# aleksandrina-streltsova/lidar-global-registration

Measured on AMD Instinct MI355X. Metric: scan-pair registrations/sec, higher is better.
Workload: dtype f32

## Files before the change

include/lgr.h:

```cpp
#ifndef LGR_H
#define LGR_H
#include <stddef.h>
#include <stdint.h>
#ifdef __cplusplus
extern "C" {
#endif

#define LGR_VERSION 5

enum {
    LGR_OK = 0,
    LGR_ERR_INVALID_ARG = -1,
    LGR_ERR_NO_DEVICE = -2,
    LGR_ERR_OOM = -3,
    LGR_ERR_HIP = -4,
    LGR_ERR_UNSUPPORTED = -5,
    LGR_ERR_VOXEL_TOO_SMALL = -6
};

enum { LGR_MATCH_LR = 0, LGR_MATCH_ONE_SIDED = 1, LGR_MATCH_CLUSTER = 2 };
enum { LGR_METRIC_CORRESPONDENCES = 0, LGR_METRIC_UNIFORMITY = 1, LGR_METRIC_CLOSEST_PLANE = 2, LGR_METRIC_COMBINATION = 3,
       LGR_METRIC_WEIGHTED_CLOSEST_PLANE = 4 };
enum { LGR_SCORE_CONSTANT = 0, LGR_SCORE_MAE = 1, LGR_SCORE_MSE = 2, LGR_SCORE_EXP = 3 };
enum { LGR_ALIGN_RANSAC = 0, LGR_ALIGN_GROR = 1 };
enum { LGR_KEYPOINT_ANY = 0, LGR_KEYPOINT_ISS = 1 };
enum { LGR_ORDER_REFERENCE = 0, LGR_ORDER_CANONICAL = 1 };

typedef struct { int32_t index_query, index_match; float distance, threshold; } lgr_corr;

typedef struct {
    int32_t feature_nr_points;
    int32_t normal_nr_points;
    float   edge_thr_coef;
    float   distance_thr;
    float   feature_radius;
    float   scale_factor;
    float   confidence;
    int32_t bf_block_size;
    int32_t cluster_k;
    int32_t randomness;
    int32_t n_samples;
    int32_t alignment_id, matching_id, metric_id, score_id;
    int32_t max_iterations;
    int32_t normals_available;
    int32_t fix_seed;
    int32_t has_vp_src, has_vp_tgt;
    float   vp_src[3], vp_tgt[3];
    int32_t ransac_batch;
    uint64_t seed;
    int32_t keypoint_id;
    float   iss_radius_src, iss_radius_tgt;
    int32_t use_bfmatcher;
    int32_t has_guess;
    float   match_search_radius;
    float   guess[16];
} lgr_params;

typedef struct {
    float   transformation[16];
    int32_t iterations;
    int32_t converged;
    int32_t n_inliers;
    float   metric;
    float   best_metric_before_refit;
    int32_t best_iteration;
    int32_t num_rejections;
    int32_t estimated_iters;
    int32_t n_correspondences;
    double  time_cs, time_te;
    float   stage_ms[12];
} lgr_result;

typedef struct lgr_ctx lgr_ctx;

typedef struct {
    int32_t helper_contexts;
    int32_t concurrent_contexts;
    int32_t arithmetic;
    int32_t pcl_neighbour_cap;
    int32_t ransac_schedule;
    int32_t reserved[3];
} lgr_ctx_options;
enum { LGR_RANSAC_SCHEDULE_DEFAULT = 0, LGR_RANSAC_SCHEDULE_CHAIN = 1, LGR_RANSAC_SCHEDULE_RESIDENT = 2 };
enum { LGR_ARITH_FAST = 0, LGR_ARITH_PCL = 1 };

typedef struct {
    int32_t prune;
    int32_t leaves;
    int32_t near;
    int32_t operand_format;
    int32_t box_bounds;
    int32_t column_stage;
    int32_t coarse_rejection;
    int32_t rerank_refilter;
    int32_t pair_cap;
    int32_t poison_tables;
    int32_t self_check;
    int32_t shell_bound;
    int32_t split_sweep;
    int32_t kept_cap;
    int32_t auto_dense;
    int32_t irregular_rows;
} lgr_match_options;

int  lgr_version(void);
#define LGR_STREAM_OWN ((void*) (intptr_t) -1)
int  lgr_ctx_create(int device, void* stream, lgr_ctx** out);
int  lgr_ctx_destroy(lgr_ctx* ctx);
int  lgr_ctx_sync(lgr_ctx* ctx);
const char* lgr_last_error(lgr_ctx* ctx);
void lgr_default_params(lgr_params* p);
int  lgr_ctx_stage_ms(lgr_ctx* ctx, float* out12);
void lgr_match_default_options(lgr_match_options* opt);
int  lgr_ctx_set_match_options(lgr_ctx* ctx, const lgr_match_options* opt);
int  lgr_ctx_get_match_options(lgr_ctx* ctx, lgr_match_options* opt);
int  lgr_ctx_workspace_bytes(lgr_ctx* ctx, uint64_t* bytes);
void lgr_ctx_default_options(lgr_ctx_options* opt);
int  lgr_ctx_set_options(lgr_ctx* ctx, const lgr_ctx_options* opt);
int  lgr_ctx_get_options(lgr_ctx* ctx, lgr_ctx_options* opt);
int  lgr_ctx_host_threads(lgr_ctx* ctx, int* n);

int lgr_sort_pairs_u32_dev(lgr_ctx*, const uint32_t* d_keys_in, uint32_t* d_keys_out, const int32_t* d_vals_in, int32_t* d_vals_out,
                           size_t n, int begin_bit, int end_bit);
int lgr_sort_pairs_u64_dev(lgr_ctx*, const uint64_t* d_keys_in, uint64_t* d_keys_out, const int32_t* d_vals_in, int32_t* d_vals_out,
                           size_t n, const int* shifts, const int* widths, int n_ranges);

int lgr_bbox_dev(lgr_ctx*, const float* d_pts, int n, float* d_min3_max3 );

int lgr_preprocess(lgr_ctx*, const float* pts, int n, const float* vp3, int normals_available, int order, float* out, int* n_out, float* voxel_out);
int lgr_preprocess_dev(lgr_ctx*, const float* d_pts, int n, const float* vp3 , int normals_available, float* d_out, int* n_out ,
                       float* voxel_out );
int lgr_dedupe_dev(lgr_ctx*, const float* d_pts, int n, float* d_out, int* n_out );
int lgr_cloud_density_dev(lgr_ctx*, const float* d_pts, int n, float quantile, float* out );

int lgr_iss_keypoints(lgr_ctx*, const float* pts, int n, float radius, float gamma21, float gamma32, int min_neighbors,
                      int32_t* idx, int* n_out);
int lgr_iss_keypoints_dev(lgr_ctx*, const float* d_pts, int n, float radius, float gamma21, float gamma32, int min_neighbors,
                          int32_t* d_idx, int* n_out );

int lgr_downsample(lgr_ctx*, const float* pts, int n, float voxel, int order, float* out, int* n_out);
int lgr_downsample_dev(lgr_ctx*, const float* d_pts, int n, float voxel, float* d_out, int* n_out );

int lgr_normals_knn(lgr_ctx*, float* pts, int n, const float* surf, int ns, int k, const float* vp3, int normals_available);
int lgr_normals_knn_dev(lgr_ctx*, float* d_pts, int n, const float* d_surf, int ns, int k, const float* vp3 , int normals_available);

int lgr_fpfh(lgr_ctx*, const float* kps, int m, const float* surf, int n, float radius, float* out_m_x_33);
int lgr_fpfh_dev(lgr_ctx*, const float* d_kps, int m, const float* d_surf, int n, float radius, float* d_out);
int lgr_shot_lrf(lgr_ctx*, const float* kps, int m, const float* surf, int n, float radius, float* out_m_x_9);
int lgr_shot_lrf_dev(lgr_ctx*, const float* d_kps, int m, const float* d_surf, int n, float radius, float* d_out_m_x_9);
int lgr_shot(lgr_ctx*, const float* kps, int m, const float* surf, int n, float radius, const float* lrf_or_null,
             float* out_m_x_352, float* out_lrf_or_null);
int lgr_shot_dev(lgr_ctx*, const float* d_kps, int m, const float* d_surf, int n, float radius, const float* d_lrf_or_null,
                 float* d_out_m_x_352, float* d_out_lrf_or_null);
int lgr_gravity_lrf(lgr_ctx*, const float* kps, int m, const float* surf, int n, float radius, float* out_m_x_9);
int lgr_gravity_lrf_dev(lgr_ctx*, const float* d_kps, int m, const float* d_surf, int n, float radius, float* d_out_m_x_9);
int lgr_rops(lgr_ctx*, const float* kps, int m, const float* surf, int n, float radius, const float* lrf, float* out_m_x_135);
int lgr_rops_dev(lgr_ctx*, const float* d_kps, int m, const float* d_surf, int n, float radius, const float* d_lrf, float* d_out_m_x_135);
int lgr_selfcheck_rcp(lgr_ctx*, unsigned lo_bits, unsigned hi_bits, unsigned long long* out2);
int lgr_selfcheck_libm(lgr_ctx*, int fn, const float* a, const float* b, long long n, float* out);

int lgr_match_bf(lgr_ctx*, const float* q33, int mq, const float* t33, int mt, int block, int32_t* idx, float* dist);
int lgr_match_bf_dev(lgr_ctx*, const float* d_q33, int mq, const float* d_t33, int mt, int block, int32_t* d_idx, float* d_dist);
int lgr_match_bf2_dev(lgr_ctx*, const float* d_a33, int ma, const float* d_b33, int mb, int block,
                      int32_t* d_ab_idx, float* d_ab_dist, int32_t* d_ba_idx, float* d_ba_dist);
int lgr_match_shot(lgr_ctx*, const float* q352, int mq, const float* t352, int mt, int block, int32_t* idx, float* dist);
int lgr_match_shot_dev(lgr_ctx*, const float* d_q352, int mq, const float* d_t352, int mt, int block, int32_t* d_idx, float* d_dist);
int lgr_match2_shot_dev(lgr_ctx*, const float* d_a352, int ma, const float* d_b352, int mb, int block,
                        int32_t* d_ab_idx, float* d_ab_dist, int32_t* d_ba_idx, float* d_ba_dist);
int lgr_match_rops(lgr_ctx*, const float* q135, int mq, const float* t135, int mt, int block, int32_t* idx, float* dist);
int lgr_match_rops_dev(lgr_ctx*, const float* d_q135, int mq, const float* d_t135, int mt, int block, int32_t* d_idx, float* d_dist);
int lgr_match2_rops_dev(lgr_ctx*, const float* d_a135, int ma, const float* d_b135, int mb, int block,
                        int32_t* d_ab_idx, float* d_ab_dist, int32_t* d_ba_idx, float* d_ba_dist);
int lgr_match_flann(lgr_ctx*, const float* q33, int mq, const float* t33, int mt, int32_t* idx, float* dist);
int lgr_match_flann_dev(lgr_ctx*, const float* d_q33, int mq, const float* d_t33, int mt, int32_t* d_idx, float* d_dist);
int lgr_match_local(lgr_ctx*, const float* query_pts, int mq, const float* train_pts, int mt, const float* q33, const float* t33,
                    const float guess16[16], float match_search_radius, int32_t* idx, float* dist);
int lgr_match_local_dev(lgr_ctx*, const float* d_query_pts, int mq, const float* d_train_pts, int mt, const float* d_q33, const float* d_t33,
                        const float guess16[16] , float match_search_radius, int32_t* d_idx, float* d_dist);

int lgr_match_last_stats(lgr_ctx*, unsigned* out6);
int lgr_match_last_kernel_ms(lgr_ctx*, float* ms);
int lgr_match_last_work(lgr_ctx*, double* executed_fraction);
int lgr_match_last_issued(lgr_ctx*, double* out2 );
int lgr_match_last_coarse(lgr_ctx*, double* out2);
int lgr_match_last_shell(lgr_ctx*, double* tiles_skipped);
int lgr_match_last_pairs(lgr_ctx*, unsigned* out2);
int lgr_match_last_format(lgr_ctx*, int* f16);
int lgr_match_last_lbstats(lgr_ctx*, double* out2);
int lgr_match_last_irregular(lgr_ctx*, unsigned* out3);
int lgr_match_last_check(lgr_ctx*, double* out2);
int lgr_match_last_check_cover(lgr_ctx*, unsigned long long* out8);
int lgr_smoothed_densities(lgr_ctx*, const float* pts, int n, int k, float* out);
int lgr_smoothed_densities_dev(lgr_ctx*, const float* d_pts, int n, int k, float* d_out);
int lgr_knn_dev(lgr_ctx*, const float* d_q, int nq, const float* d_pts, int n, int k, int32_t* d_idx, float* d_d2);

int lgr_filter_dev(lgr_ctx*, int matching_id, const float* d_src, int ns, const float* d_tgt, int nt,
                   const int32_t* d_ij_idx, const float* d_ij_dist, const int32_t* d_ji_idx, const float* d_ji_dist,
                   float distance_thr, int cluster_k, lgr_corr* d_out, int* n_out );

int lgr_correspondences(lgr_ctx*, const float* src, int ns, const float* tgt, int nt, const lgr_params*, lgr_corr* out, int* n_out);
int lgr_correspondences_dev(lgr_ctx*, const float* d_src, int ns, const float* d_tgt, int nt, const lgr_params*, lgr_corr* d_out, int* n_out );

enum { LGR_DESCRIPTOR_FPFH = 0, LGR_DESCRIPTOR_SHOT = 1, LGR_DESCRIPTOR_ROPS = 2 };
enum { LGR_LRF_DEFAULT = 0, LGR_LRF_GRAVITY = 1, LGR_LRF_GT = 2 };
typedef struct {
    int32_t descriptor_id;
    int32_t lrf_id;
    int32_t reserved[6];
} lgr_feature_params;
void lgr_default_feature_params(lgr_feature_params* f);
int lgr_correspondences_ex(lgr_ctx*, const float* src, int ns, const float* tgt, int nt, const lgr_params*, const lgr_feature_params*,
                           lgr_corr* out, int* n_out);
int lgr_correspondences_ex_dev(lgr_ctx*, const float* d_src, int ns, const float* d_tgt, int nt, const lgr_params*, const lgr_feature_params*,
                               lgr_corr* d_out, int* n_out );

int lgr_ransac(lgr_ctx*, const float* src, int ns, const float* tgt, int nt, const lgr_corr* corr, int c,
               const lgr_params*, lgr_result*, uint8_t* final_mask);
int lgr_ransac_dev(lgr_ctx*, const float* d_src, int ns, const float* d_tgt, int nt, const lgr_corr* d_corr, int c,
                   const lgr_params*, lgr_result* , uint8_t* d_final_mask);
int lgr_ransac_replay_dev(lgr_ctx*, const float* d_src, int ns, const float* d_tgt, int nt, const lgr_corr* d_corr, int c,
                          const lgr_params*, const int32_t* d_triples, int n,
                          uint8_t* d_ok, float* d_T16, int32_t* d_n_inliers, float* d_metric);
int lgr_ransac_samples_dev(lgr_ctx*, uint64_t seed, int first, int n, int n_corr, int32_t* d_triples);
int lgr_ransac_samples_n_dev(lgr_ctx*, uint64_t seed, int first, int n, int n_corr, int n_samples, int32_t* d_tuples);
int lgr_selfcheck_philox(lgr_ctx*, uint64_t key, const uint32_t counter4[4], uint32_t out4[4]);
int lgr_evaluate_dev(lgr_ctx*, const float* d_src, int ns, const float* d_tgt, int nt, const lgr_corr* d_corr, int c,
                     const float T16[16] , int metric_id, int score_id,
                     uint8_t* d_mask, int* n_inliers, float* rmse, float* metric );

int lgr_evaluate_plane_dev(lgr_ctx*, const float* d_src, int ns, const float* d_tgt, int nt, const float T16[16] , int score_id,
                           uint64_t seed, uint32_t counter, int* n_inliers, float* rmse, float* metric, float* threshold ,
                           int32_t* pairs , int* n_pairs);

enum { LGR_WEIGHT_CONSTANT = 0, LGR_WEIGHT_EXP_CURVATURE = 1, LGR_WEIGHT_CURVEDNESS = 2, LGR_WEIGHT_HARRIS = 3, LGR_WEIGHT_TOMASI = 4,
       LGR_WEIGHT_CURVATURE = 5, LGR_WEIGHT_NSS = 6 };
typedef struct {
    int32_t weight_id;
    int32_t reserved[5];
    const float* weights;
} lgr_metric_params;
void lgr_default_metric_params(lgr_metric_params* m);
int lgr_ransac_ex(lgr_ctx*, const float* src, int ns, const float* tgt, int nt, const lgr_corr* corr, int c,
                  const lgr_params*, const lgr_metric_params*, lgr_result*, uint8_t* final_mask);
int lgr_ransac_ex_dev(lgr_ctx*, const float* d_src, int ns, const float* d_tgt, int nt, const lgr_corr* d_corr, int c,
                      const lgr_params*, const lgr_metric_params*, lgr_result* , uint8_t* d_final_mask);
int lgr_weights(lgr_ctx*, const float* pts, int n, int weight_id, int nr_points, float* out, float* weights_sum );
int lgr_weights_dev(lgr_ctx*, const float* d_pts, int n, int weight_id, int nr_points, float* d_out, float* weights_sum );
int lgr_principal_curvatures(lgr_ctx*, const float* pts, int n, int k, float* pc1, float* pc2);
int lgr_principal_curvatures_dev(lgr_ctx*, const float* d_pts, int n, int k, float* d_pc1, float* d_pc2);
int lgr_evaluate_plane_weighted_dev(lgr_ctx*, const float* d_src, int ns, const float* d_tgt, int nt, const float T16[16] , int score_id,
                                    uint64_t seed, uint32_t counter, const float* d_weights, float weights_sum,
                                    int* n_inliers, float* rmse, float* metric, float* threshold ,
                                    int32_t* pairs , int* n_pairs);

int lgr_refit_svd(lgr_ctx*, const float* src, const float* tgt, int ns, int nt, const lgr_corr* inliers, int n, float T16[16]);
int lgr_refit_svd_dev(lgr_ctx*, const float* d_src, const float* d_tgt, const lgr_corr* d_corr, int c,
                      const uint8_t* d_mask , float T16[16] );

int lgr_align(lgr_ctx*, const float* src, int ns, const float* tgt, int nt, const lgr_params*, lgr_result*);
int lgr_align_dev(lgr_ctx*, const float* d_src, int ns, const float* d_tgt, int nt, const lgr_params*, lgr_result* );

int lgr_align_ex(lgr_ctx*, const float* src, int ns, const float* tgt, int nt, const lgr_params*, const lgr_feature_params*, lgr_result*);
int lgr_align_ex_dev(lgr_ctx*, const float* d_src, int ns, const float* d_tgt, int nt, const lgr_params*, const lgr_feature_params*,
                     lgr_result* );

int lgr_align_ex2(lgr_ctx*, const float* src, int ns, const float* tgt, int nt, const lgr_params*, const lgr_feature_params*,
                  const lgr_metric_params*, lgr_result*);
int lgr_align_ex2_dev(lgr_ctx*, const float* d_src, int ns, const float* d_tgt, int nt, const lgr_params*, const lgr_feature_params*,
                      const lgr_metric_params*, lgr_result* );

int lgr_gror(lgr_ctx*, const float* src, int ns, const float* tgt, int nt, const lgr_corr* corr, int c,
             float resolution, int k_optimal, lgr_result* res, uint8_t* inlier_mask );
int lgr_gror_dev(lgr_ctx*, const float* d_src, int ns, const float* d_tgt, int nt, const lgr_corr* d_corr, int c,
                 float resolution, int k_optimal, lgr_result* res , uint8_t* d_inlier_mask );
int lgr_gror_node_degree_dev(lgr_ctx*, const float* d_src, const float* d_tgt, const lgr_corr* d_corr, int c,
                             float resolution, int32_t* d_degree);

int lgr_choose_best_hypothesis_dev(lgr_ctx*, const float* d_src, int ns, const float* d_tgt, int nt, const lgr_corr* d_corr, int c,
                                   const float* tns16 , int n, float T_out16[16], int* best_index, float* uniformities );
int lgr_update_hypotheses(float* tns16, float* metrics, int n, int cap, const float* new_T16, float new_metric, float distance_thr);

#ifdef __cplusplus
}
#endif
#endif
```

lidar-global-registration_amd/csrc/lgr_features.hip:

```cpp
#include <rocprim/device/device_radix_sort.hpp>
#include <rocprim/device/device_scan.hpp>

#include <algorithm>
#include <cmath>
#include <type_traits>
#include <unordered_map>
#include <vector>

#include "lgr_grid.cuh"
#include "lgr_knn_wave.cuh"
#include "lgr_seqsum.h"
#include "lgr_math.cuh"
#include "lgr_libm.cuh"

namespace {

__global__ void voxel_keys(const float* __restrict__ pts, int n, float bx, float by, float bz, float voxel,
                           unsigned long long* __restrict__ keys, int* __restrict__ vals, int* __restrict__ bad) {
    int i = blockIdx.x * blockDim.x + threadIdx.x;
    if (i >= n) return;
    float x = pts[(size_t) i * 12], y = pts[(size_t) i * 12 + 1], z = pts[(size_t) i * 12 + 2];
    unsigned long long k = ~0ull;
    if (lgr_finite3(x, y, z)) {
        int ix = (int) floorf((x - bx) / voxel), iy = (int) floorf((y - by) / voxel), iz = (int) floorf((z - bz) / voxel);
        if (ix < 0 || iy < 0 || iz < 0 || ix >= (1 << 21) || iy >= (1 << 21) || iz >= (1 << 21)) { atomicExch(bad, 1); ix = iy = iz = 0; }
        k = ((unsigned long long) iz << 42) | ((unsigned long long) iy << 21) | (unsigned long long) ix;
    }
    keys[i] = k; vals[i] = i;
}

__global__ void head_flags(const unsigned long long* __restrict__ keys, int n, int* __restrict__ flags) {
    int i = blockIdx.x * blockDim.x + threadIdx.x;
    if (i >= n) return;
    unsigned long long k = keys[i];
    flags[i] = (k != ~0ull && (i == 0 || keys[i - 1] != k)) ? 1 : 0;
}

__global__ void voxel_accumulate(const float* __restrict__ pts, const unsigned long long* __restrict__ keys,
                                 const int* __restrict__ vals, const int* __restrict__ flags,
                                 const int* __restrict__ rank , int n,
                                 float* __restrict__ out, unsigned long long* __restrict__ out_keys, int* __restrict__ out_first) {
    int i = blockIdx.x * blockDim.x + threadIdx.x;
    if (i >= n || !flags[i]) return;
    unsigned long long k = keys[i];
    float sx = 0.f, sy = 0.f, sz = 0.f, sw = 0.f, snx = 0.f, sny = 0.f, snz = 0.f;
    for (int j = i; j < n && keys[j] == k; ++j) {
        const float4* p = reinterpret_cast<const float4*>(pts + (size_t) vals[j] * 12);
        float4 a = p[0], b = p[1], c = p[2];
        float w = c.x;
        sx += w * a.x; sy += w * a.y; sz += w * a.z;
        sw += w;
        snx += w * b.x; sny += w * b.y; snz += w * b.z;
    }
    float ax = snx / sw, ay = sny / sw, az = snz / sw;
    float norm = __builtin_sqrtf(ax * ax + ay * ay + az * az);
    norm = ((double) norm < 1e-5) ? 1.f : norm;
    int r = rank[i];
    float4* o = reinterpret_cast<float4*>(out + (size_t) r * 12);
    o[0] = make_float4(sx / sw, sy / sw, sz / sw, 1.f);
    o[1] = make_float4(ax / norm, ay / norm, az / norm, 0.f);
    o[2] = make_float4(sw, 0.f, 0.f, 0.f);
    if (out_keys) { out_keys[r] = k; out_first[r] = vals[i]; }
}

constexpr int NB = 128;

template <class IndexOf>
__device__ __forceinline__ void normals_finish(float* __restrict__ p, float px, float py, float pz, int count, IndexOf&& index_of,
                                               const float* __restrict__ surf, float vpx, float vpy, float vpz) {
    const float nanv = __uint_as_float(0x7fc00000u);
    if (count < 3) { p[4] = nanv; p[5] = nanv; p[6] = nanv; p[9] = nanv; return; }
    const float* K = surf + (size_t) index_of(0) * 12;
    float Kx = K[0], Ky = K[1], Kz = K[2];
    float a0 = 0.f, a1 = 0.f, a2 = 0.f, a3 = 0.f, a4 = 0.f, a5 = 0.f, a6 = 0.f, a7 = 0.f, a8 = 0.f;
    for (int j = 0; j < count; ++j) {
        const float* q = surf + (size_t) index_of(j) * 12;
        float x = q[0] - Kx, y = q[1] - Ky, z = q[2] - Kz;
        a0 += x * x; a1 += x * y; a2 += x * z; a3 += y * y; a4 += y * z; a5 += z * z;
        a6 += x; a7 += y; a8 += z;
    }
    float fn = (float) count;
    a0 /= fn; a1 /= fn; a2 /= fn; a3 /= fn; a4 /= fn; a5 /= fn; a6 /= fn; a7 /= fn; a8 /= fn;
    float C[9];
    C[0] = a0 - a6 * a6; C[1] = a1 - a6 * a7; C[2] = a2 - a6 * a8;
    C[4] = a3 - a7 * a7; C[5] = a4 - a7 * a8; C[8] = a5 - a8 * a8;
    C[3] = C[1]; C[6] = C[2]; C[7] = C[5];
    float lambda_min, nx, ny, nz;
    lgr_pcl_eigen33(C, lambda_min, nx, ny, nz);
    float eig_sum = C[0] + C[4] + C[8];
    float curv = (eig_sum != 0.f) ? fabsf(lambda_min / eig_sum) : 0.f;
    float dx = vpx - px, dy = vpy - py, dz = vpz - pz;
    float cos_theta = (dx * nx + dy * ny + dz * nz);
    if (cos_theta < 0.f) { nx = -nx; ny = -ny; nz = -nz; }
    if (lgr_finite3(nx, ny, nz)) {
        float norm = __builtin_sqrtf(nx * nx + ny * ny + nz * nz);
        nx /= norm; ny /= norm; nz /= norm;
    }
    p[4] = nx; p[5] = ny; p[6] = nz; p[9] = curv;
}

__global__ __launch_bounds__(NB) void normals_kernel(GridDev g, const float* __restrict__ surf, float* __restrict__ pts, int n,
                                                      int k, float vpx, float vpy, float vpz, int by_grid) {
    extern __shared__ float smem[];
    float* sd = smem;
    int* si = (int*) (smem + (size_t) k * NB);
    int i = blockIdx.x * NB + threadIdx.x;
    if (by_grid == 1) {
        i = lgr_xcd_tile(blockIdx.x, cdiv_dev(g.n, NB)) * NB + threadIdx.x;
        if (i >= g.n) return;
        i = __float_as_int(g.pxyz[i].w);
    } else if (i >= n) return;
    float* p = pts + (size_t) i * 12;
    float px = p[0], py = p[1], pz = p[2];
    if (by_grid == 2 && lgr_finite3(px, py, pz)) return;
    KnnList<NB> L;
    L.init(sd, si, k, threadIdx.x);
    if (lgr_finite3(px, py, pz) && g.n > 0) lgr_knn_query(g, px, py, pz, L);
    normals_finish(p, px, py, pz, L.count, [&](int j) { return L.index(j); }, surf, vpx, vpy, vpz);
}

constexpr int NW_WAVES = 4;
template <int KPL>
__global__ __launch_bounds__(64 * NW_WAVES) void normals_wave_kernel(GridDev g, const float* __restrict__ surf, float* __restrict__ pts, int k,
                                                                      float vpx, float vpy, float vpz, float r2_init) {
    extern __shared__ int slist[];
    __shared__ unsigned long long sbuf[NW_WAVES][WaveKnn<KPL>::BUF];
    __shared__ int srow[NW_WAVES][128];
    const int lane = threadIdx.x & 63, wv = threadIdx.x >> 6;
    const int n_tiles = cdiv_dev(g.n, 64 * NW_WAVES);
    const int tile = lgr_xcd_tile(blockIdx.x, n_tiles);
    if (tile >= n_tiles) return;
    const int t = (tile * NW_WAVES + wv) * 64 + lane;
    int* list = slist + (size_t) wv * k * 64;
    int qi = -1;
    float px = 0.f, py = 0.f, pz = 0.f;
    if (t < g.n) {
        const float4 q = g.pxyz[t];
        qi = __float_as_int(q.w); px = q.x; py = q.y; pz = q.z;
    }
    float guess = r2_init;
    int count = 0;
    lgr_wave_knn_tile<KPL>(g, qi >= 0, px, py, pz, k, guess, sbuf[wv], srow[wv], [&](int l, const WaveKnn<KPL>& W) {
        const int mk = min(W.m, k);
#pragma unroll
        for (int j = 0; j < KPL; ++j)
            if (W.rank[j] < mk) list[W.rank[j] * 64 + l] = (int) (unsigned) W.key[j];
        if (lane == l) count = mk;
    });
    __builtin_amdgcn_fence(__ATOMIC_RELEASE, "wavefront");
    __builtin_amdgcn_wave_barrier();
    if (qi < 0) return;
    normals_finish(pts + (size_t) qi * 12, px, py, pz, count, [&](int j) { return list[j * 64 + lane]; }, surf, vpx, vpy, vpz);
}

__device__ __forceinline__ float dot3e(float ax, float ay, float az, float bx, float by, float bz) {
    return (ax * bx + az * bz) + ay * by;
}

__device__ __forceinline__ bool pair_features(float p1x, float p1y, float p1z, float n1x, float n1y, float n1z,
                                              float p2x, float p2y, float p2z, float n2x, float n2y, float n2z,
                                              float& f1, float& f2, float& f3) {
    float dx = p2x - p1x, dy = p2y - p1y, dz = p2z - p1z;
    float f4 = __builtin_sqrtf(dot3e(dx, dy, dz, dx, dy, dz));
    if (f4 == 0.0f) return false;
    float angle1 = dot3e(n1x, n1y, n1z, dx, dy, dz) / f4;
    float angle2 = dot3e(n2x, n2y, n2z, dx, dy, dz) / f4;
    float ux = n1x, uy = n1y, uz = n1z, mx = n2x, my = n2y, mz = n2z;
    float a1 = fabsf(angle1), a2 = fabsf(angle2);
    if (lgr_glibc::acosf_(a1) > lgr_glibc::acosf_(a2)) {
        ux = n2x; uy = n2y; uz = n2z; mx = n1x; my = n1y; mz = n1z;
        dx = -dx; dy = -dy; dz = -dz;
        f3 = -angle2;
    } else {
        f3 = angle1;
    }
    float vx = dy * uz - dz * uy, vy = dz * ux - dx * uz, vz = dx * uy - dy * ux;
    float v_norm = __builtin_sqrtf(dot3e(vx, vy, vz, vx, vy, vz));
    if (v_norm == 0.0f) return false;
    vx /= v_norm; vy /= v_norm; vz /= v_norm;
    float wx = uy * vz - uz * vy, wy = uz * vx - ux * vz, wz = ux * vy - uy * vx;
    f2 = dot3e(vx, vy, vz, mx, my, mz);
    float yy = dot3e(wx, wy, wz, mx, my, mz), xx = dot3e(ux, uy, uz, mx, my, mz);
    f1 = lgr_glibc::atan2f_(yy, xx);
    return true;
}

typedef float v2f __attribute__((ext_vector_type(2)));

__device__ __forceinline__ float lgr_atan2f_fast(float y, float x) {
    const float ax = fabsf(x), ay = fabsf(y);
    const float mx = (ax > ay) ? ax : ay;
    const float mn = (ax > ay) ? ay : ax;
    const float a = mn * __builtin_amdgcn_rcpf(mx);
    const bool hi = a > 0.41421356237f;
    const float z = hi ? (a - 1.0f) * __builtin_amdgcn_rcpf(a + 1.0f) : a;
    const float z2 = z * z;
    float p = 8.05374449538e-2f * z2 - 1.38776856032e-1f;
    p = p * z2 + 1.99777106478e-1f;
    p = p * z2 - 3.33329491539e-1f;
    p = p * z2 * z + z;
    float r = (hi ? 0.78539816339f : 0.0f) + p;
    if (ay > ax) r = 1.57079632679f - r;
    if (x < 0.0f) r = 3.14159265359f - r;
    if (y < 0.0f) r = -r;
    return r;
}
__device__ __forceinline__ bool bin_decided(float t, float margin, int& b) {
    const float fl = floorf(t);
    const float fr = t - fl;
    b = (int) fminf(fmaxf(fl, 0.0f), 10.0f);
    return fr > margin && fr < 1.0f - margin;
}
__device__ __forceinline__ void pair_bins_fast(float p1x, float p1y, float p1z, float n1x, float n1y, float n1z, float p2x, float p2y, float p2z, float n2x, float n2y, float n2z,
                                               int (&b0)[3], bool& dec0) {
    constexpr float DA = 1e-6f;
    float dx = p2x - p1x, dy = p2y - p1y, dz = p2z - p1z;
    const float f4s = dot3e(dx, dy, dz, dx, dy, dz);
    const float rs = __builtin_amdgcn_rsqf(f4s);
    const float angle1 = dot3e(n1x, n1y, n1z, dx, dy, dz) * rs;
    const float angle2 = dot3e(n2x, n2y, n2z, dx, dy, dz) * rs;
    const float a1 = fabsf(angle1), a2 = fabsf(angle2);
    const bool s0 = a1 < a2;
    bool c0 = f4s > 1e-30f && (s0 ? (a2 - a1 > 2.0f * DA && a2 < 1.0f - DA) : (a1 - a2 > 2.0f * DA));
    const float ux = s0 ? n2x : n1x, uy = s0 ? n2y : n1y, uz = s0 ? n2z : n1z;
    const float mx = s0 ? n1x : n2x, my = s0 ? n1y : n2y, mz = s0 ? n1z : n2z;
    dx = s0 ? -dx : dx; dy = s0 ? -dy : dy; dz = s0 ? -dz : dz;
    const float f3 = s0 ? -angle2 : angle1;
    float vx = dy * uz - dz * uy, vy = dz * ux - dx * uz, vz = dx * uy - dy * ux;
    const float vn2 = dot3e(vx, vy, vz, vx, vy, vz);
    const float rv = __builtin_amdgcn_rsqf(vn2);
    c0 = c0 && vn2 > 1e-30f;
    vx = vx * rv; vy = vy * rv; vz = vz * rv;
    const float wx = uy * vz - uz * vy, wy = uz * vx - ux * vz, wz = ux * vy - uy * vx;
    const float f2 = dot3e(vx, vy, vz, mx, my, mz);
    const float yy = dot3e(wx, wy, wz, mx, my, mz), xx = dot3e(ux, uy, uz, mx, my, mz);
    const float rho2 = xx * xx + yy * yy;
    const float f1 = lgr_atan2f_fast(yy, xx);
    const float irho = __builtin_amdgcn_rsqf(rho2);
    c0 = c0 && rho2 > 1e-4f;
    constexpr float S1 = (float) (11.0 * (double) (1.0f / (2.0f * 3.14159274101257324f)));
    constexpr float O1 = (float) (11.0 * 3.14159265358979323846 * (double) (1.0f / (2.0f * 3.14159274101257324f)));
    const float t1 = __builtin_fmaf(f1, S1, O1), t2 = __builtin_fmaf(f2, 5.5f, 5.5f), t3 = __builtin_fmaf(f3, 5.5f, 5.5f);
    const float m1 = __builtin_fmaf(irho, 1.751f * 5e-6f, 1.751f * 3e-6f + 2e-6f);
    constexpr float M2 = 5.5f * 3e-6f + 1e-6f, M3 = 5.5f * DA + 1e-6f;
    const bool d01 = bin_decided(t1, m1, b0[0]), d02 = bin_decided(t2, M2, b0[1]), d03 = bin_decided(t3, M3, b0[2]);
    dec0 = d01 && d02 && d03 && c0;
}

__device__ __forceinline__ int bin11(double t) {
    double v = floor(11 * t);
    if (!(v == v)) return 0;
    if (v < 0) return 0;
    if (v >= 11) return 10;
    return (int) v;
}

constexpr int HP = 48;
__host__ __device__ constexpr int spfh_slot(int b) { return (b & 15) * 3 + (b >> 4); }
#ifdef LGR_SPFH_CHECK
__device__ unsigned long long g_spfh_check[4];
#endif
constexpr int ST = 16;
constexpr int SQ = 256;
constexpr int SHP = 33;

#ifndef LGR_SPFH_WAVES
#define LGR_SPFH_WAVES 5
#endif
__global__ __launch_bounds__(64) __attribute__((amdgpu_waves_per_eu(LGR_SPFH_WAVES, LGR_SPFH_WAVES))) void spfh_tile_kernel(GridDev g, float r2, const int* __restrict__ order, float* __restrict__ spfh ) {
    __shared__ float4 tp[ST], tn[ST];
    __shared__ float4 cp[64], cn[64];
    __shared__ unsigned short queue[SQ];
    __shared__ int hist[2][ST][SHP];
    __shared__ int kcnt[ST];
    const int l = threadIdx.x;
    int pos = -1, cell = -1;
    float x = 0.f, y = 0.f, z = 0.f;
    const int tile = lgr_xcd_tile(blockIdx.x, cdiv_dev(g.n, ST));
    if (tile * ST >= g.n) return;
    if (l < ST) {
        const int rnk = tile * ST + l;
        if (rnk < g.n) {
            pos = order ? order[rnk] : rnk;
            const float4 P = g.pxyz[pos];
            x = P.x; y = P.y; z = P.z;
            tp[l] = make_float4(P.x, P.y, P.z, __int_as_float(pos));
            tn[l] = g.pnrm[pos];
            const int cx = min(max(lgr_cellc(x, g.ox, g.h), 0), g.dx - 1), cy = min(max(lgr_cellc(y, g.oy, g.h), 0), g.dy - 1), cz = min(max(lgr_cellc(z, g.oz, g.h), 0), g.dz - 1);
            cell = (cz * g.dy + cy) * g.dx + cx;
        }
        kcnt[l] = 0;
    }
    for (int q = l; q < 2 * ST * SHP; q += 64) (&hist[0][0][0])[q] = 0;
    __syncthreads();
    const float r2box = r2 * 1.0001f + 1e-30f;
    const float d_pi = 1.0f / (2.0f * 3.14159274101257324f);
    const double MPI = 3.14159265358979323846;
    int qh = 0, qt = 0;
    auto process = [&](int nb) __attribute__((always_inline)) {
        if (l < nb) {
            const unsigned e0 = queue[(qh + l) & (SQ - 1)];
            const int i0 = (int) (e0 >> 8);
            const float4 P0 = tp[i0], N0 = tn[i0], Q0 = cp[e0 & 255u], M0 = cn[e0 & 255u];
            int ba[3];
            bool dec0, ok0 = true;
            pair_bins_fast(P0.x, P0.y, P0.z, N0.x, N0.y, N0.z, Q0.x, Q0.y, Q0.z, M0.x, M0.y, M0.z, ba, dec0);
#ifdef LGR_SPFH_CHECK
            const bool fdec0 = dec0;
            const int fa0 = ba[0], fa1 = ba[1], fa2 = ba[2];
            dec0 = false;
#endif
            if (!dec0) {
                const int cc = (int) (e0 & 255u);
                const float Px = tp[i0].x, Py = tp[i0].y, Pz = tp[i0].z, Nx = tn[i0].x, Ny = tn[i0].y, Nz = tn[i0].z;
                const float Qx = cp[cc].x, Qy = cp[cc].y, Qz = cp[cc].z, Mx = cn[cc].x, My = cn[cc].y, Mz = cn[cc].z;
                float f1, f2, f3;
                ok0 = pair_features(Px, Py, Pz, Nx, Ny, Nz, Qx, Qy, Qz, Mx, My, Mz, f1, f2, f3);
                ba[0] = bin11(((double) f1 + MPI) * (double) d_pi); ba[1] = bin11(((double) f2 + 1.0) * 0.5); ba[2] = bin11(((double) f3 + 1.0) * 0.5);
            }
#ifdef LGR_SPFH_CHECK
            {
                const bool bad0 = fdec0 && (!ok0 || fa0 != ba[0] || fa1 != ba[1] || fa2 != ba[2]);
                const unsigned long long n_pairs = __popcll(__ballot(true));
                const unsigned long long n_und = __popcll(__ballot(!fdec0));
                const unsigned long long n_bad = __popcll(__ballot(bad0));
                if (l == 0) { atomicAdd(&g_spfh_check[0], n_pairs); atomicAdd(&g_spfh_check[1], n_und); if (n_bad) atomicAdd(&g_spfh_check[2], n_bad); }
            }
#endif
            if (ok0) {
                int* h = &hist[l & 1][i0][0];
                atomicAdd(h + ba[0], 1); atomicAdd(h + 11 + ba[1], 1); atomicAdd(h + 22 + ba[2], 1);
            }
        }
        qh += nb;
    };
    for (int p = 0; p < ST;) {
        const int c = __builtin_amdgcn_readlane(cell, p);
        const bool active = l < ST && cell == c;
        const int n_run = __popcll(__ballot(active));
        const int p0 = p;
        p += n_run;
        if (c < 0) break;
        float bx0 = active ? x : 3.4e38f, bx1 = active ? x : -3.4e38f, by0 = active ? y : 3.4e38f, by1 = active ? y : -3.4e38f;
        float bz0 = active ? z : 3.4e38f, bz1 = active ? z : -3.4e38f;
#pragma unroll
        for (int o = 1; o < 64; o <<= 1) {
            bx0 = fminf(bx0, __shfl_xor(bx0, o)); bx1 = fmaxf(bx1, __shfl_xor(bx1, o));
            by0 = fminf(by0, __shfl_xor(by0, o)); by1 = fmaxf(by1, __shfl_xor(by1, o));
            bz0 = fminf(bz0, __shfl_xor(bz0, o)); bz1 = fmaxf(bz1, __shfl_xor(bz1, o));
        }
        const int cz = c / (g.dx * g.dy), cy = (c / g.dx) % g.dy, cx = c % g.dx;
        int n_buf = 0;
        auto test_block = [&](int n_c) __attribute__((always_inline)) {
            float4 Q = make_float4(0.f, 0.f, 0.f, 0.f);
            if (l < n_c) Q = cp[l];
            for (int i = p0; i < p0 + n_run; ++i) {
                const float4 P_i = tp[i];
                const float d2 = lgr_dist2(P_i.x, P_i.y, P_i.z, Q.x, Q.y, Q.z);
                const bool acc = l < n_c && d2 < r2;
                const unsigned long long am = __ballot(acc);
                if (am == 0ull) continue;
                if (l == 0) kcnt[i] += __popcll(am);
                const bool enq = acc && __float_as_int(Q.w) != __float_as_int(P_i.w);
                const unsigned long long em = __ballot(enq);
                if (enq) {
                    const int rank = __builtin_amdgcn_mbcnt_hi((unsigned) (em >> 32), __builtin_amdgcn_mbcnt_lo((unsigned) em, 0u));
                    queue[(qt + rank) & (SQ - 1)] = (unsigned short) ((i << 8) | l);
                }
                qt += __popcll(em);
                if (qt - qh >= 64) {
                    __syncthreads();
                    process(64);
                }
            }
            __syncthreads();
            while (qt - qh > 0) process(min(qt - qh, 64));
            __syncthreads();
        };
        for (int zz = max(cz - 1, 0); zz <= min(cz + 1, g.dz - 1); ++zz)
            for (int yy = max(cy - 1, 0); yy <= min(cy + 1, g.dy - 1); ++yy) {
                const int x0 = max(cx - 1, 0), x1 = min(cx + 1, g.dx - 1);
                const size_t c0 = ((size_t) zz * g.dy + yy) * g.dx;
                const int b = g.cell_start[c0 + x0], e = g.cell_start[c0 + x1 + 1];
                for (int t0 = b; t0 < e; t0 += 64) {
                    const int t = t0 + l;
                    bool live = false;
                    float4 P = make_float4(0.f, 0.f, 0.f, 0.f);
                    if (t < e) {
                        P = g.pxyz[t];
                        const float ddx = fmaxf(fmaxf(bx0 - P.x, P.x - bx1), 0.f), ddy = fmaxf(fmaxf(by0 - P.y, P.y - by1), 0.f), ddz = fmaxf(fmaxf(bz0 - P.z, P.z - bz1), 0.f);
                        live = (ddx * ddx + ddy * ddy) + ddz * ddz <= r2box;
                    }
                    const unsigned long long lm = __ballot(live);
                    if (lm == 0ull) continue;
                    const int rank = __builtin_amdgcn_mbcnt_hi((unsigned) (lm >> 32), __builtin_amdgcn_mbcnt_lo((unsigned) lm, 0u));
                    const int fit = min(__popcll(lm), 64 - n_buf);
                    float4 Nq = make_float4(0.f, 0.f, 0.f, 0.f);
                    if (live) {
                        Nq = g.pnrm[t];
                        if (rank < fit) { cp[n_buf + rank] = make_float4(P.x, P.y, P.z, __int_as_float(t)); cn[n_buf + rank] = Nq; }
                    }
                    n_buf += fit;
                    __syncthreads();
                    if (n_buf == 64) {
                        test_block(64);
                        if (live && rank >= fit) { cp[rank - fit] = make_float4(P.x, P.y, P.z, __int_as_float(t)); cn[rank - fit] = Nq; }
                        n_buf = __popcll(lm) - fit;
                        __syncthreads();
                    }
                }
            }
        if (n_buf > 0) test_block(n_buf);
    }
    __syncthreads();
    for (int q = l; q < ST * 33; q += 64) {
        const int i = q / 33, b = q % 33;
        if (tile * ST + i >= g.n) continue;
        const int ps = __float_as_int(tp[i].w);
        const float incr = 100.0f / (float) (kcnt[i] - 1);
        spfh[(size_t) ps * HP + spfh_slot(b)] = lgr_seqsum(incr, hist[0][i][b] + hist[1][i][b]);
    }
    for (int q = l; q < ST * (HP - 33); q += 64) {
        const int i = q / (HP - 33), b = 33 + q % (HP - 33);
        if (tile * ST + i >= g.n) continue;
        spfh[(size_t) __float_as_int(tp[i].w) * HP + spfh_slot(b)] = 0.f;
    }
}

typedef float f32x4 __attribute__((ext_vector_type(4)));
typedef float f32x3 __attribute__((ext_vector_type(3)));
#ifndef LGR_RCP_STEPS
#define LGR_RCP_STEPS 1
#endif
constexpr float LGR_RCP_LO = 1e-36f;
__device__ __forceinline__ v2f lgr_rcp2(v2f x) {
    v2f y{__builtin_amdgcn_rcpf(x.x), __builtin_amdgcn_rcpf(x.y)};
    const v2f one{1.f, 1.f};
#pragma unroll
    for (int s = 0; s < LGR_RCP_STEPS; ++s) {
        const v2f e = __builtin_elementwise_fma(-x, y, one);
        y = __builtin_elementwise_fma(e, y, y);
    }
    return y;
}
__device__ __forceinline__ float lgr_rcp1(float x) {
    float y = __builtin_amdgcn_rcpf(x);
#pragma unroll
    for (int s = 0; s < LGR_RCP_STEPS; ++s) {
        const float e = fmaf(-x, y, 1.f);
        y = fmaf(e, y, y);
    }
    return y;
}
__global__ void rcp_check_kernel(unsigned lo_bits, unsigned hi_bits, unsigned long long* __restrict__ out) {
    unsigned long long bad = 0, cnt = 0;
    const unsigned long long span = (unsigned long long) hi_bits - lo_bits + 1ull;
    for (unsigned long long o = (unsigned long long) blockIdx.x * blockDim.x + threadIdx.x; o < span; o += (unsigned long long) gridDim.x * blockDim.x) {
        const float x = __uint_as_float(lo_bits + (unsigned) o);
        const float q = 1.0f / x;
        const v2f r2 = lgr_rcp2(v2f{x, x});
        bad += (__float_as_uint(lgr_rcp1(x)) != __float_as_uint(q)) || (__float_as_uint(r2.x) != __float_as_uint(q)) || (__float_as_uint(r2.y) != __float_as_uint(q));
        ++cnt;
    }
    for (int o = 32; o > 0; o >>= 1) { bad += __shfl_xor(bad, o); cnt += __shfl_xor(cnt, o); }
    if ((threadIdx.x & 63) == 0) { if (bad) atomicAdd(&out[0], bad); atomicAdd(&out[1], cnt); }
}
constexpr int FT = 16;
constexpr int FRING = 128;
constexpr int FP_PITCH = 36;

__global__ __launch_bounds__(64) void fpfh_mfma_kernel(GridDev g, const float* __restrict__ kps, const int* __restrict__ order, int m, float r2,
                                                       const float* __restrict__ Hs , float* __restrict__ out) {
    __shared__ float4 ring[FRING];
    __shared__ float fpl[FT * FP_PITCH];
    const int l = threadIdx.x, i = l & 15, k = l >> 4;
    const int tile = lgr_xcd_tile(blockIdx.x, cdiv_dev(m, FT));
    if (tile * FT >= m) return;
    const int r = tile * FT + i;
    const float nanv = __uint_as_float(0x7fc00000u);
    int kp = -1;
    float x = nanv, y = nanv, z = nanv;
    if (r < m) {
        kp = order[r];
        x = kps[(size_t) kp * 12]; y = kps[(size_t) kp * 12 + 1]; z = kps[(size_t) kp * 12 + 2];
    }
    const bool fin = lgr_finite3(x, y, z);
    int cell = -1;
    if (fin && g.n > 0) {
        int cx = min(max(lgr_cellc(x, g.ox, g.h), 0), g.dx - 1), cy = min(max(lgr_cellc(y, g.oy, g.h), 0), g.dy - 1), cz = min(max(lgr_cellc(z, g.oz, g.h), 0), g.dz - 1);
        cell = (cz * g.dy + cy) * g.dx + cx;
    }
    f32x4 acc0 = {0.f, 0.f, 0.f, 0.f}, acc1 = acc0, acc2 = acc0;
    bool found = false;
    const float r2box = r2 * 1.0001f + 1e-30f;
    const float* hload = Hs + 3 * i;
    for (int p = 0; p < FT;) {
        const int c = __builtin_amdgcn_readlane(cell, p);
        const bool active = cell == c;
        const unsigned long long am = __ballot(active) & 0xffffull;
        p += __popcll(am);
        if (c < 0) continue;
        float bx0 = active ? x : 3.4e38f, bx1 = active ? x : -3.4e38f, by0 = active ? y : 3.4e38f, by1 = active ? y : -3.4e38f;
        float bz0 = active ? z : 3.4e38f, bz1 = active ? z : -3.4e38f;
#pragma unroll
        for (int o = 1; o < 16; o <<= 1) {
            bx0 = fminf(bx0, __shfl_xor(bx0, o)); bx1 = fmaxf(bx1, __shfl_xor(bx1, o));
            by0 = fminf(by0, __shfl_xor(by0, o)); by1 = fmaxf(by1, __shfl_xor(by1, o));
            bz0 = fminf(bz0, __shfl_xor(bz0, o)); bz1 = fmaxf(bz1, __shfl_xor(bz1, o));
        }
        auto uni = [](float v) { return __int_as_float(__builtin_amdgcn_readfirstlane(__float_as_int(v))); };
        bx0 = uni(bx0); bx1 = uni(bx1); by0 = uni(by0); by1 = uni(by1); bz0 = uni(bz0); bz1 = uni(bz1);
        const int cz = c / (g.dx * g.dy), cy = (c / g.dx) % g.dy, cx = c % g.dx;
        int head = 0, tail = 0;
        auto round = [&](auto GC) {
            constexpr int G = decltype(GC)::value;
            float4 e[G];
            f32x3 hv[G];
#pragma unroll
            for (int u = 0; u < G; ++u) e[u] = ring[(head + 4 * u + k) & (FRING - 1)];
#pragma unroll
            for (int u = 0; u < G; ++u) hv[u] = *reinterpret_cast<const f32x3*>(hload + (unsigned) __float_as_int(e[u].w));
            const v2f X{x, x}, Y{y, y}, Z{z, z};
            float d2[G], w[G];
#pragma unroll
            for (int h2 = 0; h2 < G / 2; ++h2) {
                const v2f dx = X - v2f{e[2 * h2].x, e[2 * h2 + 1].x}, dy = Y - v2f{e[2 * h2].y, e[2 * h2 + 1].y}, dz = Z - v2f{e[2 * h2].z, e[2 * h2 + 1].z};
                const v2f dd = (dx * dx + dy * dy) + dz * dz;
                const v2f ww = lgr_rcp2(dd);
                d2[2 * h2] = dd.x; d2[2 * h2 + 1] = dd.y; w[2 * h2] = ww.x; w[2 * h2 + 1] = ww.y;
            }
            bool odd = false;
#pragma unroll
            for (int u = 0; u < G; ++u) {
                const bool in = active & (d2[u] < r2);
                found = found | in;
                const bool use = in & (d2[u] != 0.f);
                odd = odd | (use & !(d2[u] >= LGR_RCP_LO));
                w[u] = use ? w[u] : 0.f;
            }
            if (__ballot(odd) != 0ull) {
#pragma unroll
                for (int u = 0; u < G; ++u) w[u] = (active & (d2[u] < r2) & (d2[u] != 0.f)) ? 1.0f / d2[u] : 0.f;
            }
#pragma unroll
            for (int u = 0; u < G; ++u) {
                acc0 = __builtin_amdgcn_mfma_f32_16x16x4f32(w[u], hv[u].x, acc0, 0, 0, 0);
                acc1 = __builtin_amdgcn_mfma_f32_16x16x4f32(w[u], hv[u].y, acc1, 0, 0, 0);
                acc2 = __builtin_amdgcn_mfma_f32_16x16x4f32(w[u], hv[u].z, acc2, 0, 0, 0);
            }
            head += 4 * G;
        };
        auto consume = [&](int n_groups) {
            int gq = 0;
            for (; gq + 4 <= n_groups; gq += 4) round(std::integral_constant<int, 4>{});
            for (; gq < n_groups; ++gq, head += 4) {
                const float4 e = ring[(head + k) & (FRING - 1)];
                const float d2 = lgr_dist2(x, y, z, e.x, e.y, e.z);
                const bool in = active & (d2 < r2);
                found = found | in;
                const bool use = in & (d2 != 0.f);
                if (__ballot(use) == 0ull) continue;
                float w = lgr_rcp1(d2);
                if (__ballot(use & !(d2 >= LGR_RCP_LO)) != 0ull) w = 1.0f / d2;
                w = use ? w : 0.f;
                const f32x3 hv = *reinterpret_cast<const f32x3*>(hload + (unsigned) __float_as_int(e.w));
                const float b0 = hv.x, b1 = hv.y, b2 = hv.z;
                acc0 = __builtin_amdgcn_mfma_f32_16x16x4f32(w, b0, acc0, 0, 0, 0);
                acc1 = __builtin_amdgcn_mfma_f32_16x16x4f32(w, b1, acc1, 0, 0, 0);
                acc2 = __builtin_amdgcn_mfma_f32_16x16x4f32(w, b2, acc2, 0, 0, 0);
            }
        };
        for (int zz = max(cz - 1, 0); zz <= min(cz + 1, g.dz - 1); ++zz)
            for (int yy = max(cy - 1, 0); yy <= min(cy + 1, g.dy - 1); ++yy) {
                const int x0 = max(cx - 1, 0), x1 = min(cx + 1, g.dx - 1);
                const size_t c0 = ((size_t) zz * g.dy + yy) * g.dx;
                const int b = g.cell_start[c0 + x0], e = g.cell_start[c0 + x1 + 1];
                for (int t0 = b; t0 < e; t0 += 64) {
                    const int t = t0 + l;
                    bool live = false;
                    float4 P = make_float4(0.f, 0.f, 0.f, 0.f);
                    if (t < e) {
                        P = g.pxyz[t];
                        const float ddx = fmaxf(fmaxf(bx0 - P.x, P.x - bx1), 0.f), ddy = fmaxf(fmaxf(by0 - P.y, P.y - by1), 0.f), ddz = fmaxf(fmaxf(bz0 - P.z, P.z - bz1), 0.f);
                        live = (ddx * ddx + ddy * ddy) + ddz * ddz <= r2box;
                    }
                    const unsigned long long lm = __ballot(live);
                    if (lm == 0ull) continue;
                    if (live) {
                        const int rank = __builtin_amdgcn_mbcnt_hi((unsigned) (lm >> 32), __builtin_amdgcn_mbcnt_lo((unsigned) lm, 0u));
                        ring[(tail + rank) & (FRING - 1)] = make_float4(P.x, P.y, P.z, __uint_as_float((unsigned) t * (unsigned) HP));
                    }
                    tail += __popcll(lm);
                    __syncthreads();
                    consume((tail - head) >> 2);
                    __syncthreads();
                }
            }
        if (tail > head) {
            if (l < 4 - (tail - head)) ring[(tail + l) & (FRING - 1)] = make_float4(3.0e38f, 3.0e38f, 3.0e38f, __uint_as_float((unsigned) g.n * (unsigned) HP));
            __syncthreads();
            consume(1);
            __syncthreads();
        }
    }
    asm volatile("s_nop 15\n\ts_nop 7" ::: "memory");
    const unsigned long long fm = __ballot(found);
#pragma unroll
    for (int q = 0; q < 4; ++q) {
        const int row = 4 * k + q;
        fpl[row * FP_PITCH + i] = acc0[q];
        fpl[row * FP_PITCH + 16 + i] = acc1[q];
        if (i == 0) fpl[row * FP_PITCH + 32] = acc2[q];
    }
    __syncthreads();
    if (l < 3 * FT) {
        const int kq = l / 3, blk = l % 3;
        const int rr = tile * FT + kq;
        if (rr < m) {
            const bool any = ((fm >> kq) | (fm >> (kq + 16)) | (fm >> (kq + 32)) | (fm >> (kq + 48))) & 1ull;
            float* o = out + (size_t) order[rr] * 33 + 11 * blk;
            const float* f = fpl + kq * FP_PITCH + 11 * blk;
            if (!any) {
#pragma unroll
                for (int q = 0; q < 11; ++q) o[q] = nanv;
            } else {
                double sum = 0.0;
#pragma unroll
                for (int q = 0; q < 11; ++q) sum += (double) f[q];
                if (sum != 0) sum = 100.0 / sum;
#pragma unroll
                for (int q = 0; q < 11; ++q) o[q] = (float) ((double) f[q] * sum);
            }
        }
    }
}

template <int PW_CAP>
__global__ __launch_bounds__(64) void fpfh_pcl_kernel(GridDev g, const float* __restrict__ kps, const int* __restrict__ order, int m, float r2,
                                                      const float* __restrict__ Hs , float* __restrict__ out) {
    __shared__ unsigned long long skey[PW_CAP];
    __shared__ unsigned spos[PW_CAP];
    __shared__ float sval[64];
    const int l = threadIdx.x;
    const int tile = lgr_xcd_tile(blockIdx.x, m);
    if (tile >= m) return;
    const int kp = order[tile];
    const float x = kps[(size_t) kp * 12], y = kps[(size_t) kp * 12 + 1], z = kps[(size_t) kp * 12 + 2];
    const float nanv = __uint_as_float(0x7fc00000u);
    float* o = out + (size_t) kp * 33;
    if (!lgr_finite3(x, y, z) || g.n == 0) {
        if (l < 33) o[l] = nanv;
        return;
    }
    const int cx = min(max(lgr_cellc(x, g.ox, g.h), 0), g.dx - 1), cy = min(max(lgr_cellc(y, g.oy, g.h), 0), g.dy - 1), cz = min(max(lgr_cellc(z, g.oz, g.h), 0), g.dz - 1);
    const unsigned long long key_end = (unsigned long long) __float_as_uint(r2) << 32;
    auto scan = [&](unsigned long long lo, unsigned long long hi, bool store) -> int {
        int cnt = 0;
        for (int zz = max(cz - 1, 0); zz <= min(cz + 1, g.dz - 1); ++zz)
            for (int yy = max(cy - 1, 0); yy <= min(cy + 1, g.dy - 1); ++yy) {
                const int x0 = max(cx - 1, 0), x1 = min(cx + 1, g.dx - 1);
                const size_t c0 = ((size_t) zz * g.dy + yy) * g.dx;
                const int b = g.cell_start[c0 + x0], e = g.cell_start[c0 + x1 + 1];
                for (int t0 = b; t0 < e; t0 += 64) {
                    const int t = t0 + l;
                    bool in = false;
                    unsigned long long key = 0ull;
                    if (t < e) {
                        const float4 P = g.pxyz[t];
                        const float d2 = lgr_dist2(x, y, z, P.x, P.y, P.z);
                        key = ((unsigned long long) __float_as_uint(d2) << 32) | (unsigned) __float_as_int(P.w);
                        in = d2 < r2 && key >= lo && key < hi;
                    }
                    const unsigned long long bm = __ballot(in);
                    if (bm == 0ull) continue;
                    if (store && in) {
                        const int slot = cnt + __builtin_amdgcn_mbcnt_hi((unsigned) (bm >> 32), __builtin_amdgcn_mbcnt_lo((unsigned) bm, 0u));
                        if (slot < PW_CAP) { skey[slot] = key; spos[slot] = (unsigned) t; }
                    }
                    cnt += __popcll(bm);
                }
            }
        return cnt;
    };
    const int bin = min(l, 32);
    const float* hcol = Hs + spfh_slot(bin);
    for (int strict = 0; strict < 2; ++strict) {
        float fp = 0.f;
        double dsum = 0.0;
        int emin = 255;
        bool bad = false;
        int total = 0;
        unsigned long long lo = 0ull;
        while (lo < key_end) {
            unsigned long long hi = key_end;
            __syncthreads();
            int cnt = scan(lo, hi, true);
            if (cnt > PW_CAP) {
                unsigned long long a = lo, bnd = hi;
                for (;;) {
                    const unsigned long long mid = a + ((bnd - a) >> 1);
                    const int c = scan(lo, mid, false);
                    if (c > PW_CAP) bnd = mid;
                    else { a = mid; if (c >= PW_CAP / 4 || bnd - a <= 1ull) break; }
                }
                hi = a;
                __syncthreads();
                cnt = scan(lo, hi, true);
            }
            total += cnt;
            int n_pad = 64;
            while (n_pad < cnt) n_pad <<= 1;
            for (int q = cnt + l; q < n_pad; q += 64) { skey[q] = ~0ull; spos[q] = 0u; }
            __syncthreads();
            for (int k2 = 2; k2 <= n_pad; k2 <<= 1)
                for (int j = k2 >> 1; j > 0; j >>= 1) {
                    for (int q = l; q < (n_pad >> 1); q += 64) {
                        const int i0 = ((q & ~(j - 1)) << 1) | (q & (j - 1)), i1 = i0 | j;
                        const unsigned long long ka = skey[i0], kb = skey[i1];
                        const bool up = (i0 & k2) == 0;
                        if ((ka > kb) == up) {
                            skey[i0] = kb; skey[i1] = ka;
                            const unsigned pa = spos[i0]; spos[i0] = spos[i1]; spos[i1] = pa;
                        }
                    }
                    __syncthreads();
                }
            for (int q = l; q < cnt; q += 64) {
                const float d2 = __uint_as_float((unsigned) (skey[q] >> 32));
                const float w = d2 == 0.f ? 0.f : 1.0f / d2;
                skey[q] = ((unsigned long long) __float_as_uint(w) << 32) | (spos[q] * (unsigned) HP);
            }
            __syncthreads();
            if (!strict) {
                int q = 0;
                for (; q + 4 <= cnt; q += 4) {
                    const unsigned long long e0 = skey[q], e1 = skey[q + 1], e2 = skey[q + 2], e3 = skey[q + 3];
                    const float h0 = hcol[(unsigned) e0], h1 = hcol[(unsigned) e1], h2 = hcol[(unsigned) e2], h3 = hcol[(unsigned) e3];
                    const float w0 = __uint_as_float((unsigned) (e0 >> 32)), w1 = __uint_as_float((unsigned) (e1 >> 32)), w2 = __uint_as_float((unsigned) (e2 >> 32)), w3 = __uint_as_float((unsigned) (e3 >> 32));
                    const float v[4] = {h0 * w0, h1 * w1, h2 * w2, h3 * w3};
                    const float ws[4] = {w0, w1, w2, w3};
#pragma unroll
                    for (int u = 0; u < 4; ++u) {
                        if (ws[u] == 0.f) continue;
                        fp += v[u];
                        dsum += (double) v[u];
                        const int eb = (int) ((__float_as_uint(v[u]) >> 23) & 0xffu);
                        bad = bad || !(v[u] >= 0.f) || eb == 255;
                        if (v[u] != 0.f) emin = min(emin, max(eb, 1));
                    }
                }
                for (; q < cnt; ++q) {
                    const unsigned long long e0 = skey[q];
                    const float w0 = __uint_as_float((unsigned) (e0 >> 32));
                    if (w0 == 0.f) continue;
                    const float v0 = hcol[(unsigned) e0] * w0;
                    fp += v0;
                    dsum += (double) v0;
                    const int eb = (int) ((__float_as_uint(v0) >> 23) & 0xffu);
                    bad = bad || !(v0 >= 0.f) || eb == 255;
                    if (v0 != 0.f) emin = min(emin, max(eb, 1));
                }
            } else {
                for (int q = 0; q < cnt; ++q) {
                    const unsigned long long e0 = skey[q];
                    const float w0 = __uint_as_float((unsigned) (e0 >> 32));
                    if (w0 == 0.f) continue;
                    const float v0 = hcol[(unsigned) e0] * w0;
                    fp += v0;
                    sval[l] = v0;
                    __syncthreads();
                    if (l < 3) {
#pragma unroll
                        for (int u = 0; u < 11; ++u) dsum += (double) sval[11 * l + u];
                    }
                    __syncthreads();
                }
            }
            lo = hi;
        }
        if (total == 0) {
            if (l < 33) o[l] = nanv;
            return;
        }
        double bsum;
        if (!strict) {
            double t_all = l < 33 ? dsum : 0.0;
            int e_all = l < 33 ? emin : 255;
            bool b_all = l < 33 && bad;
#pragma unroll
            for (int s2 = 1; s2 < 64; s2 <<= 1) {
                t_all += __shfl_xor(t_all, s2);
                e_all = min(e_all, __shfl_xor(e_all, s2));
            }
            b_all = __ballot(b_all) != 0ull;
            const bool exact_here = !b_all && (e_all == 255 || t_all * 1.000001 < ldexp(1.0, 53 + e_all - 150));
            if (__ballot(!exact_here) != 0ull) continue;
            const int blk = bin / 11;
            bsum = 0.0;
#pragma unroll
            for (int u = 0; u < 11; ++u) bsum += __shfl(dsum, 11 * blk + u);
        } else {
            bsum = __shfl(dsum, bin / 11);
        }
        if (bsum != 0) bsum = 100.0 / bsum;
        if (l < 33) o[l] = (float) ((double) fp * bsum);
        return;
    }
}

__global__ void fine_keys(GridDev g, const float* __restrict__ pts, int stride, int m, int sb, unsigned* __restrict__ keys, int* __restrict__ vals) {
    int i = blockIdx.x * blockDim.x + threadIdx.x;
    if (i >= m) return;
    float x = pts[(size_t) i * stride], y = pts[(size_t) i * stride + 1], z = pts[(size_t) i * stride + 2];
    unsigned k = 0xffffffffu;
    if (lgr_finite3(x, y, z)) {
        int cx = min(max(lgr_cellc(x, g.ox, g.h), 0), g.dx - 1), cy = min(max(lgr_cellc(y, g.oy, g.h), 0), g.dy - 1), cz = min(max(lgr_cellc(z, g.oz, g.h), 0), g.dz - 1);
        k = (unsigned) ((cz * g.dy + cy) * g.dx + cx);
        if (sb > 0) {
            const float q = (float) (1 << sb);
            int sx = min(max((int) (((x - g.ox) / g.h - (float) cx) * q), 0), (1 << sb) - 1);
            int sy = min(max((int) (((y - g.oy) / g.h - (float) cy) * q), 0), (1 << sb) - 1);
            int sz = min(max((int) (((z - g.oz) / g.h - (float) cz) * q), 0), (1 << sb) - 1);
            unsigned mort = 0;
            for (int b = 0; b < sb; ++b) mort |= (((unsigned) sx >> b) & 1u) << (3 * b) | (((unsigned) sy >> b) & 1u) << (3 * b + 1) | (((unsigned) sz >> b) & 1u) << (3 * b + 2);
            k = (k << (3 * sb)) | mort;
        }
    }
    keys[i] = k; vals[i] = i;
}

struct Key3 { int x, y, z; bool operator==(const Key3& o) const { return x == o.x && y == o.y && z == o.z; } };
struct HashKey3 {
    std::size_t operator()(const Key3& k) const {
        std::size_t seed = 0;
        const int e[3] = {k.x, k.y, k.z};
        for (int i = 0; i < 3; ++i) seed ^= std::hash<int>()(e[i]) + 0x9e3779b9 + (seed << 6) + (seed >> 2);
        return seed;
    }
};

}

static int downsample_core(lgr_ctx* ctx, const float* d_pts, int n, float voxel, float* d_out, int* n_out,
                           std::vector<unsigned long long>* h_keys, std::vector<int>* h_first) {
    LGR_CHECK(ctx, voxel > 0.f, LGR_ERR_INVALID_ARG);
    *n_out = 0;
    if (n == 0) return LGR_OK;
    float bb[12];
    LGR_TRY(lgr_bbox_host(ctx, d_pts, n, bb));
    float bx = bb[6] - voxel * 0.5f, by = bb[7] - voxel * 0.5f, bz = bb[8] - voxel * 0.5f;
    unsigned long long *keys, *keys2;
    int *vals, *vals2, *flags, *rank, *bad;
    LGR_TRY(lgr_ws_t(ctx, WS_DS_KEYS, (size_t) n, &keys));
    LGR_TRY(lgr_ws_t(ctx, WS_DS_KEYS2, (size_t) n, &keys2));
    LGR_TRY(lgr_ws_t(ctx, WS_DS_VALS, (size_t) n, &vals));
    LGR_TRY(lgr_ws_t(ctx, WS_DS_VALS2, (size_t) n, &vals2));
    LGR_TRY(lgr_ws_t(ctx, WS_DS_FLAGS, (size_t) 2 * n + 16, &flags));
    rank = flags + n;
    bad = rank + n;
    LGR_HIP(ctx, hipMemsetAsync(bad, 0, 4, ctx->stream));
    voxel_keys<<<cdiv(n, 256), 256, 0, ctx->stream>>>(d_pts, n, bx, by, bz, voxel, keys, vals, bad);
    size_t tb2 = 0;
    LGR_HIP(ctx, rocprim::exclusive_scan(nullptr, tb2, flags, rank, 0, (size_t) n, rocprim::plus<int>(), ctx->stream));
    void* tmp;
    LGR_TRY(lgr_ws(ctx, WS_GRID_TMP, tb2, &tmp));
    {
        const float bnd[3] = {bx, by, bz};
        int shifts[3] = {0, 21, 42}, widths[3];
        for (int a = 0; a < 3; ++a) {
            const float q = std::floor((bb[9 + a] - bnd[a]) / voxel);
            long long imax = (q >= 0.f && q < 2097152.f) ? (long long) q : 2097151;
            int b = 1;
            while ((1ll << b) <= imax) ++b;
            widths[a] = std::min(21, b);
        }
        widths[2] = std::min(22, widths[2] + 1);
        LGR_TRY(lgr_sort_pairs_u64(ctx, keys, keys2, vals, vals2, (size_t) n, shifts, widths, 3));
    }
    head_flags<<<cdiv(n, 256), 256, 0, ctx->stream>>>(keys2, n, flags);
    LGR_HIP(ctx, rocprim::exclusive_scan(tmp, tb2, flags, rank, 0, (size_t) n, rocprim::plus<int>(), ctx->stream));
    int* h;
    LGR_TRY(lgr_pinned(ctx, 64, (void**) &h));
    LGR_HIP(ctx, hipMemcpyAsync(h, rank + (n - 1), 4, hipMemcpyDeviceToHost, ctx->stream));
    LGR_HIP(ctx, hipMemcpyAsync(h + 1, flags + (n - 1), 4, hipMemcpyDeviceToHost, ctx->stream));
    LGR_HIP(ctx, hipMemcpyAsync(h + 2, bad, 4, hipMemcpyDeviceToHost, ctx->stream));
    LGR_HIP(ctx, hipStreamSynchronize(ctx->stream));
    int nv = h[0] + h[1];
    if (h[2]) return lgr_fail(ctx, LGR_ERR_VOXEL_TOO_SMALL, "voxel index exceeds 21 bits per axis", __FILE__, __LINE__);
    unsigned long long* okeys = nullptr;
    int* ofirst = nullptr;
    if (h_keys) {
        LGR_TRY(lgr_ws_t(ctx, WS_DS_MISC, (size_t) nv * 3 + 4, (int**) &ofirst));
        okeys = (unsigned long long*) (ofirst + ((nv + 1) & ~1));
    }
    float* stage = d_out;
    bool alias = d_out == d_pts;
    if (alias) LGR_TRY(lgr_ws_t(ctx, WS_HOST_F, (size_t) nv * 12 + 4, &stage));
    voxel_accumulate<<<cdiv(n, 256), 256, 0, ctx->stream>>>(d_pts, keys2, vals2, flags, rank, n, stage, okeys, ofirst);
    if (alias) LGR_HIP(ctx, hipMemcpyAsync(d_out, stage, (size_t) nv * 48, hipMemcpyDeviceToDevice, ctx->stream));
    if (h_keys) {
        h_keys->resize(nv); h_first->resize(nv);
        LGR_HIP(ctx, hipMemcpyAsync(h_keys->data(), okeys, (size_t) nv * 8, hipMemcpyDeviceToHost, ctx->stream));
        LGR_HIP(ctx, hipMemcpyAsync(h_first->data(), ofirst, (size_t) nv * 4, hipMemcpyDeviceToHost, ctx->stream));
        LGR_HIP(ctx, hipStreamSynchronize(ctx->stream));
    }
    LGR_HIP(ctx, hipGetLastError());
    *n_out = nv;
    return LGR_OK;
}

extern "C" int lgr_downsample_dev(lgr_ctx* ctx, const float* d_pts, int n, float voxel, float* d_out, int* n_out) {
    lgr_turn turn__(ctx);
    if (!ctx) return LGR_ERR_INVALID_ARG;
    LGR_CHECK(ctx, (d_pts || n == 0) && (d_out || n == 0) && n_out && n >= 0, LGR_ERR_INVALID_ARG);
    LGR_HIP(ctx, hipSetDevice(ctx->device));
    return downsample_core(ctx, d_pts, n, voxel, d_out, n_out, nullptr, nullptr);
}

extern "C" int lgr_downsample(lgr_ctx* ctx, const float* pts, int n, float voxel, int order, float* out, int* n_out) {
    lgr_turn turn__(ctx);
    if (!ctx) return LGR_ERR_INVALID_ARG;
    LGR_CHECK(ctx, (pts || n == 0) && out && n_out && n >= 0, LGR_ERR_INVALID_ARG);
    LGR_CHECK(ctx, order == LGR_ORDER_REFERENCE || order == LGR_ORDER_CANONICAL, LGR_ERR_INVALID_ARG);
    LGR_HIP(ctx, hipSetDevice(ctx->device));
    *n_out = 0;
    if (n == 0) return LGR_OK;
    float *dp, *dout;
    LGR_TRY(lgr_ws_t(ctx, WS_HOST_A, (size_t) n * 12, &dp));
    LGR_TRY(lgr_ws_t(ctx, WS_HOST_B, (size_t) n * 12, &dout));
    LGR_HIP(ctx, hipMemcpyAsync(dp, pts, (size_t) n * 48, hipMemcpyHostToDevice, ctx->stream));
    std::vector<unsigned long long> keys;
    std::vector<int> first;
    int nv = 0;
    LGR_TRY(downsample_core(ctx, dp, n, voxel, dout, &nv, order == LGR_ORDER_REFERENCE ? &keys : nullptr, &first));
    if (order == LGR_ORDER_CANONICAL) {
        LGR_HIP(ctx, hipMemcpyAsync(out, dout, (size_t) nv * 48, hipMemcpyDeviceToHost, ctx->stream));
        LGR_HIP(ctx, hipStreamSynchronize(ctx->stream));
    } else {
        std::vector<float> tmp((size_t) nv * 12);
        LGR_HIP(ctx, hipMemcpyAsync(tmp.data(), dout, (size_t) nv * 48, hipMemcpyDeviceToHost, ctx->stream));
        LGR_HIP(ctx, hipStreamSynchronize(ctx->stream));
        std::vector<int> by_first(nv);
        for (int i = 0; i < nv; ++i) by_first[i] = i;
        std::sort(by_first.begin(), by_first.end(), [&](int a, int b) { return first[a] < first[b]; });
        std::unordered_map<Key3, int, HashKey3> m;
        for (int v : by_first) {
            unsigned long long k = keys[v];
            Key3 k3{(int) (k & 0x1fffff), (int) ((k >> 21) & 0x1fffff), (int) ((k >> 42) & 0x1fffff)};
            m[k3] = v;
        }
        size_t o = 0;
        for (const auto& kv : m) { memcpy(out + 12 * o, tmp.data() + 12 * (size_t) kv.second, 48); ++o; }
    }
    *n_out = nv;
    return LGR_OK;
}

extern "C" int lgr_selfcheck_rcp(lgr_ctx* ctx, unsigned lo_bits, unsigned hi_bits, unsigned long long* out2) {
    lgr_turn turn__(ctx);
    if (!ctx) return LGR_ERR_INVALID_ARG;
    LGR_CHECK(ctx, out2 && lo_bits <= hi_bits, LGR_ERR_INVALID_ARG);
    LGR_HIP(ctx, hipSetDevice(ctx->device));
    unsigned long long* d;
    LGR_TRY(lgr_ws_t(ctx, WS_HOST_A, (size_t) 2, &d));
    LGR_HIP(ctx, hipMemsetAsync(d, 0, 16, ctx->stream));
    rcp_check_kernel<<<8 * ctx->n_cu, 256, 0, ctx->stream>>>(lo_bits, hi_bits, d);
    LGR_HIP(ctx, hipGetLastError());
    LGR_HIP(ctx, hipMemcpyAsync(out2, d, 16, hipMemcpyDeviceToHost, ctx->stream));
    LGR_HIP(ctx, hipStreamSynchronize(ctx->stream));
    return LGR_OK;
}

__global__ void libm_eval_kernel(int fn, const float* __restrict__ a, const float* __restrict__ b, long long n, float* __restrict__ out) {
    for (long long i = (long long) blockIdx.x * blockDim.x + threadIdx.x; i < n; i += (long long) gridDim.x * blockDim.x) {
        const float x = a[i];
        float r;
        switch (fn) {
            case 0: r = lgr_glibc::acosf_(x); break;
            case 1: r = lgr_glibc::atanf_(x); break;
            case 2: r = lgr_glibc::atan2f_(x, b[i]); break;
            case 3: r = lgr_glibc::sinf_(x); break;
            default: r = lgr_glibc::cosf_(x); break;
        }
        out[i] = r;
    }
}
extern "C" int lgr_selfcheck_libm(lgr_ctx* ctx, int fn, const float* a, const float* b, long long n, float* out) {
    lgr_turn turn__(ctx);
    if (!ctx) return LGR_ERR_INVALID_ARG;
    LGR_CHECK(ctx, fn >= 0 && fn <= 6 && a && out && n >= 0 && (fn != 2 || b), LGR_ERR_INVALID_ARG);
    if (n == 0) return LGR_OK;
    LGR_HIP(ctx, hipSetDevice(ctx->device));
    float *da, *db, *dout;
    LGR_TRY(lgr_ws_t(ctx, WS_HOST_A, (size_t) n, &da));
    LGR_TRY(lgr_ws_t(ctx, WS_HOST_B, (size_t) n, &db));
    LGR_TRY(lgr_ws_t(ctx, WS_HOST_C, (size_t) n, &dout));
    LGR_HIP(ctx, hipMemcpyAsync(da, a, (size_t) n * 4, hipMemcpyHostToDevice, ctx->stream));
    if (fn == 2) LGR_HIP(ctx, hipMemcpyAsync(db, b, (size_t) n * 4, hipMemcpyHostToDevice, ctx->stream));
    if (fn >= 5) LGR_TRY(lgr_weights_libm_launch(ctx, fn, da, n, dout));
    else libm_eval_kernel<<<8 * ctx->n_cu, 256, 0, ctx->stream>>>(fn, da, db, n, dout);
    LGR_HIP(ctx, hipGetLastError());
    LGR_HIP(ctx, hipMemcpyAsync(out, dout, (size_t) n * 4, hipMemcpyDeviceToHost, ctx->stream));
    LGR_HIP(ctx, hipStreamSynchronize(ctx->stream));
    return LGR_OK;
}

#ifdef LGR_SPFH_CHECK
extern "C" int lgr_debug_spfh_check(unsigned long long* out3, int reset) {
    unsigned long long z[4] = {0, 0, 0, 0};
    if (hipMemcpyFromSymbol(out3, HIP_SYMBOL(g_spfh_check), 24) != hipSuccess) return LGR_ERR_HIP;
    if (reset && hipMemcpyToSymbol(HIP_SYMBOL(g_spfh_check), z, 32) != hipSuccess) return LGR_ERR_HIP;
    return LGR_OK;
}
#endif

extern "C" int lgr_normals_knn_dev(lgr_ctx* ctx, float* d_pts, int n, const float* d_surf, int ns, int k, const float* vp3, int normals_available) {
    lgr_turn turn__(ctx);
    if (!ctx) return LGR_ERR_INVALID_ARG;
    LGR_CHECK(ctx, (d_pts || n == 0) && n >= 0 && k >= 1 && k <= 64, LGR_ERR_INVALID_ARG);
    (void) normals_available;
    if (n == 0) return LGR_OK;
    LGR_HIP(ctx, hipSetDevice(ctx->device));
    const float* S = d_surf;
    if (!S) {
        float* snap;
        LGR_TRY(lgr_ws_t(ctx, WS_HOST_F, (size_t) n * 12, &snap));
        LGR_HIP(ctx, hipMemcpyAsync(snap, d_pts, (size_t) n * 48, hipMemcpyDeviceToDevice, ctx->stream));
        S = snap; ns = n;
    }
    GridDev g;
    const bool wave = !d_surf && k >= 16;
    const float ppc = wave ? 10.f : 6.f;
    LGR_TRY(lgr_grid_build(ctx, WS_GRID_A, S, ns, 0.f, ppc, &g));
    size_t sm = (size_t) k * NB * 8;
    const float vx = vp3 ? vp3[0] : 0.f, vy = vp3 ? vp3[1] : 0.f, vz = vp3 ? vp3[2] : 0.f;
    if (wave) {
        const float r2i = g.h * g.h * 1.25f * (float) k / (3.14159265f * ppc);
        const int grid = lgr_xcd_grid(cdiv(g.n, 64 * NW_WAVES));
        const size_t sml = (size_t) NW_WAVES * k * 64 * sizeof(int);
        if (g.n > 0) {
            if (k <= 40) normals_wave_kernel<1><<<grid, 64 * NW_WAVES, sml, ctx->stream>>>(g, S, d_pts, k, vx, vy, vz, r2i);
            else {
                if (sml + 8192 > 65536) LGR_HIP(ctx, hipFuncSetAttribute((const void*) normals_wave_kernel<2>, hipFuncAttributeMaxDynamicSharedMemorySize, (int) sml));
                normals_wave_kernel<2><<<grid, 64 * NW_WAVES, sml, ctx->stream>>>(g, S, d_pts, k, vx, vy, vz, r2i);
            }
        }
        if (g.n < n) normals_kernel<<<cdiv(n, NB), NB, sm, ctx->stream>>>(g, S, d_pts, n, k, vx, vy, vz, 2);
    } else if (!d_surf) {
        if (g.n > 0) normals_kernel<<<lgr_xcd_grid(cdiv(g.n, NB)), NB, sm, ctx->stream>>>(g, S, d_pts, n, k, vx, vy, vz, 1);
        if (g.n < n) normals_kernel<<<cdiv(n, NB), NB, sm, ctx->stream>>>(g, S, d_pts, n, k, vx, vy, vz, 2);
    } else {
        normals_kernel<<<cdiv(n, NB), NB, sm, ctx->stream>>>(g, S, d_pts, n, k, vx, vy, vz, 0);
    }
    LGR_HIP(ctx, hipGetLastError());
    return LGR_OK;
}

extern "C" int lgr_normals_knn(lgr_ctx* ctx, float* pts, int n, const float* surf, int ns, int k, const float* vp3, int normals_available) {
    lgr_turn turn__(ctx);
    if (!ctx) return LGR_ERR_INVALID_ARG;
    LGR_CHECK(ctx, (pts || n == 0) && n >= 0, LGR_ERR_INVALID_ARG);
    if (n == 0) return LGR_OK;
    LGR_HIP(ctx, hipSetDevice(ctx->device));
    float *dp, *ds = nullptr;
    LGR_TRY(lgr_ws_t(ctx, WS_HOST_A, (size_t) n * 12, &dp));
    LGR_HIP(ctx, hipMemcpyAsync(dp, pts, (size_t) n * 48, hipMemcpyHostToDevice, ctx->stream));
    if (surf) {
        LGR_TRY(lgr_ws_t(ctx, WS_HOST_B, (size_t) ns * 12 + 4, &ds));
        LGR_HIP(ctx, hipMemcpyAsync(ds, surf, (size_t) ns * 48, hipMemcpyHostToDevice, ctx->stream));
    }
    LGR_TRY(lgr_normals_knn_dev(ctx, dp, n, ds, ns, k, vp3, normals_available));
    LGR_HIP(ctx, hipMemcpyAsync(pts, dp, (size_t) n * 48, hipMemcpyDeviceToHost, ctx->stream));
    LGR_HIP(ctx, hipStreamSynchronize(ctx->stream));
    return LGR_OK;
}

extern "C" int lgr_fpfh_dev(lgr_ctx* ctx, const float* d_kps, int m, const float* d_surf, int n, float radius, float* d_out) {
    lgr_turn turn__(ctx);
    if (!ctx) return LGR_ERR_INVALID_ARG;
    LGR_CHECK(ctx, (d_kps || m == 0) && (d_surf || n == 0) && (d_out || m == 0) && m >= 0 && n >= 0 && radius > 0.f, LGR_ERR_INVALID_ARG);
    LGR_CHECK(ctx, radius <= 1e18f && (size_t) n + 1 <= ((size_t) 1 << 32) / HP - 1, LGR_ERR_UNSUPPORTED);
    if (m == 0) return LGR_OK;
    LGR_HIP(ctx, hipSetDevice(ctx->device));
    GridDev g;
    LGR_TRY(lgr_grid_build(ctx, WS_GRID_B, d_surf, n, radius * 1.001f, 0.f, &g));
    float r2 = radius * radius;
    float* spfh;
    LGR_TRY(lgr_ws_t(ctx, WS_SPFH, ((size_t) n + 1) * HP + 64, &spfh));
    LGR_HIP(ctx, hipMemsetAsync(spfh + (size_t) g.n * HP, 0, HP * sizeof(float), ctx->stream));
    const long long n_cells = (long long) g.dx * g.dy * g.dz;
    int cell_bits = 1;
    while ((1ll << cell_bits) < n_cells) ++cell_bits;
    const int sb = std::max(0, std::min(2, (32 - cell_bits) / 3));
    const int key_bits = std::min(32, cell_bits + 3 * sb);
    const int mx = std::max(m, g.n);
    unsigned *keys, *keys2, *kkeys, *kkeys2;
    int *vals, *vals2, *kvals, *kvals2;
    LGR_TRY(lgr_ws_t(ctx, WS_KP_ORDER, (size_t) mx * 8 + 16, &keys));
    keys2 = keys + mx; vals = (int*) (keys2 + mx); vals2 = vals + mx;
    kkeys = (unsigned*) (vals2 + mx); kkeys2 = kkeys + mx; kvals = (int*) (kkeys2 + mx); kvals2 = kvals + mx;
    fine_keys<<<cdiv(m, 256), 256, 0, ctx->stream>>>(g, d_kps, 12, m, sb, kkeys, kvals);
    LGR_TRY(lgr_sort_pairs_u32(ctx, kkeys, kkeys2, kvals, kvals2, (size_t) m, 0, key_bits));
    if (g.n > 0) {
        fine_keys<<<cdiv(g.n, 256), 256, 0, ctx->stream>>>(g, reinterpret_cast<const float*>(g.pxyz), 4, g.n, sb, keys, vals);
        LGR_TRY(lgr_sort_pairs_u32(ctx, keys, keys2, vals, vals2, (size_t) g.n, 0, key_bits));
        spfh_tile_kernel<<<lgr_xcd_grid(cdiv(g.n, ST)), 64, 0, ctx->stream>>>(g, r2, vals2, spfh);
    }
    if (ctx->opt.arithmetic == LGR_ARITH_PCL) {
        if (ctx->opt.pcl_neighbour_cap == 64) fpfh_pcl_kernel<64><<<lgr_xcd_grid(m), 64, 0, ctx->stream>>>(g, d_kps, kvals2, m, r2, spfh, d_out);
        else if (ctx->opt.pcl_neighbour_cap == 1024) fpfh_pcl_kernel<1024><<<lgr_xcd_grid(m), 64, 0, ctx->stream>>>(g, d_kps, kvals2, m, r2, spfh, d_out);
        else fpfh_pcl_kernel<512><<<lgr_xcd_grid(m), 64, 0, ctx->stream>>>(g, d_kps, kvals2, m, r2, spfh, d_out);
    } else {
        fpfh_mfma_kernel<<<lgr_xcd_grid(cdiv(m, FT)), 64, 0, ctx->stream>>>(g, d_kps, kvals2, m, r2, spfh, d_out);
    }
    LGR_HIP(ctx, hipGetLastError());
    return LGR_OK;
}

extern "C" int lgr_fpfh(lgr_ctx* ctx, const float* kps, int m, const float* surf, int n, float radius, float* out) {
    lgr_turn turn__(ctx);
    if (!ctx) return LGR_ERR_INVALID_ARG;
    LGR_CHECK(ctx, (kps || m == 0) && (surf || n == 0) && (out || m == 0) && m >= 0 && n >= 0, LGR_ERR_INVALID_ARG);
    if (m == 0) return LGR_OK;
    LGR_HIP(ctx, hipSetDevice(ctx->device));
    float *dk, *ds, *dout;
    LGR_TRY(lgr_ws_t(ctx, WS_HOST_A, (size_t) m * 12, &dk));
    LGR_TRY(lgr_ws_t(ctx, WS_HOST_B, (size_t) n * 12 + 4, &ds));
    LGR_TRY(lgr_ws_t(ctx, WS_HOST_C, (size_t) m * 33, &dout));
    LGR_HIP(ctx, hipMemcpyAsync(dk, kps, (size_t) m * 48, hipMemcpyHostToDevice, ctx->stream));
    if (n) LGR_HIP(ctx, hipMemcpyAsync(ds, surf, (size_t) n * 48, hipMemcpyHostToDevice, ctx->stream));
    LGR_TRY(lgr_fpfh_dev(ctx, dk, m, ds, n, radius, dout));
    LGR_HIP(ctx, hipMemcpyAsync(out, dout, (size_t) m * 132, hipMemcpyDeviceToHost, ctx->stream));
    LGR_HIP(ctx, hipStreamSynchronize(ctx->stream));
    return LGR_OK;
}
```

lidar-global-registration_amd/csrc/lgr_grid.hip:

```cpp
#include <rocprim/device/device_radix_sort.hpp>
#include <rocprim/device/device_scan.hpp>

#include <algorithm>
#include <cmath>

#include "lgr_grid.cuh"
#include "lgr_knn_wave.cuh"

namespace {

__device__ __forceinline__ unsigned fkey(float f) {
    unsigned b = __float_as_uint(f);
    return (b & 0x80000000u) ? ~b : (b | 0x80000000u);
}
__host__ __device__ inline float fkey_inv(unsigned k) {
    unsigned b = (k & 0x80000000u) ? (k & 0x7fffffffu) : ~k;
    float f;
    memcpy(&f, &b, 4);
    return f;
}

__global__ void bbox_kernel(const float* __restrict__ pts, int n, unsigned* __restrict__ out) {
    float tmn[3] = {INFINITY, INFINITY, INFINITY}, tmx[3] = {-INFINITY, -INFINITY, -INFINITY};
    float qmn[3] = {3.4028234663852886e38f, 3.4028234663852886e38f, 3.4028234663852886e38f};
    float qmx[3] = {1.17549435e-38f, 1.17549435e-38f, 1.17549435e-38f};
    for (int i = blockIdx.x * blockDim.x + threadIdx.x; i < n; i += gridDim.x * blockDim.x) {
        float p[3] = {pts[(size_t) i * 12], pts[(size_t) i * 12 + 1], pts[(size_t) i * 12 + 2]};
        bool fin = lgr_finite3(p[0], p[1], p[2]);
#pragma unroll
        for (int a = 0; a < 3; ++a) {
            if (fin) { tmn[a] = fminf(tmn[a], p[a]); tmx[a] = fmaxf(tmx[a], p[a]); }
            qmn[a] = (p[a] < qmn[a]) ? p[a] : qmn[a];
            qmx[a] = (qmx[a] < p[a]) ? p[a] : qmx[a];
        }
    }
    __shared__ float sh[4][12];
#pragma unroll
    for (int a = 0; a < 3; ++a) {
        for (int o = 32; o > 0; o >>= 1) {
            tmn[a] = fminf(tmn[a], __shfl_xor(tmn[a], o)); tmx[a] = fmaxf(tmx[a], __shfl_xor(tmx[a], o));
            qmn[a] = fminf(qmn[a], __shfl_xor(qmn[a], o)); qmx[a] = fmaxf(qmx[a], __shfl_xor(qmx[a], o));
        }
        if ((threadIdx.x & 63) == 0) {
            int w = threadIdx.x >> 6;
            sh[w][a] = tmn[a]; sh[w][3 + a] = tmx[a]; sh[w][6 + a] = qmn[a]; sh[w][9 + a] = qmx[a];
        }
    }
    __syncthreads();
    if (threadIdx.x < 12) {
        int k = threadIdx.x;
        bool is_min = (k < 3) || (k >= 6 && k < 9);
        float v = sh[0][k];
        for (int w = 1; w < (int) (blockDim.x >> 6); ++w) v = is_min ? fminf(v, sh[w][k]) : fmaxf(v, sh[w][k]);
        if (is_min) atomicMin(&out[k], fkey(v)); else atomicMax(&out[k], fkey(v));
    }
}

__global__ void cell_keys(const float* __restrict__ pts, int n, float ox, float oy, float oz, float h, int dx, int dy, int dz,
                          unsigned invalid_key, unsigned* __restrict__ keys, int* __restrict__ vals) {
    int i = blockIdx.x * blockDim.x + threadIdx.x;
    if (i >= n) return;
    float x = pts[(size_t) i * 12], y = pts[(size_t) i * 12 + 1], z = pts[(size_t) i * 12 + 2];
    unsigned k = invalid_key;
    if (lgr_finite3(x, y, z)) {
        int cx = min(max(lgr_cellc(x, ox, h), 0), dx - 1), cy = min(max(lgr_cellc(y, oy, h), 0), dy - 1), cz = min(max(lgr_cellc(z, oz, h), 0), dz - 1);
        k = (unsigned) ((cz * dy + cy) * dx + cx);
    }
    keys[i] = k; vals[i] = i;
}

constexpr int CSF_T = 256, CSF_SHIFT = 10, CSF_CELLS = 1 << CSF_SHIFT;
static_assert(CSF_CELLS == 4 * CSF_T, "one int4 store per thread");
__global__ __launch_bounds__(256) void coarse_start_fill(const unsigned* __restrict__ keys, int n, int nblk, int* __restrict__ coarse) {
    const int lane = threadIdx.x & 63;
    const int base = (blockIdx.x * 4 + (threadIdx.x >> 6)) * 64;
    const int i = base + lane;
    int lo = 1, hi = 0;
    if (i <= n) {
        lo = i == 0 ? 0 : (int) (keys[i - 1] >> CSF_SHIFT) + 1;
        hi = i == n ? nblk : (int) (keys[i] >> CSF_SHIFT);
    }
    unsigned long long todo = __ballot(lo <= hi);
    while (todo) {
        const int j = __builtin_ctzll(todo);
        todo &= todo - 1ull;
        const int lo_j = __builtin_amdgcn_readlane(lo, j), hi_j = __builtin_amdgcn_readlane(hi, j);
        for (int c = lo_j + lane; c <= hi_j; c += 64) coarse[c] = base + j;
    }
}
__global__ __launch_bounds__(CSF_T) void cell_start_fill(const unsigned* __restrict__ keys, const int* __restrict__ coarse, unsigned ncell, int* __restrict__ start) {
    const int k0 = coarse[blockIdx.x], k1 = coarse[blockIdx.x + 1];
    const unsigned c = (unsigned) blockIdx.x * CSF_CELLS + 4u * threadIdx.x;
    if (c > ncell) return;
    int lo = k0, hi = k1;
    while (lo < hi) { const int mid = (lo + hi) >> 1; if (keys[mid] < c) lo = mid + 1; else hi = mid; }
    int4 v;
    v.x = lo;
    while (lo < k1 && keys[lo] < c + 1u) ++lo;
    v.y = lo;
    while (lo < k1 && keys[lo] < c + 2u) ++lo;
    v.z = lo;
    while (lo < k1 && keys[lo] < c + 3u) ++lo;
    v.w = lo;
    if (c + 3u <= ncell) {
        *reinterpret_cast<int4*>(start + c) = v;
    } else {
        start[c] = v.x;
        if (c + 1u <= ncell) start[c + 1] = v.y;
        if (c + 2u <= ncell) start[c + 2] = v.z;
    }
}

__global__ void gather_points(const float* __restrict__ pts, const int* __restrict__ vals, int nvalid,
                              float4* __restrict__ pxyz, float4* __restrict__ pnrm) {
    int i = blockIdx.x * blockDim.x + threadIdx.x;
    if (i >= nvalid) return;
    int o = vals[i];
    const float4* p = reinterpret_cast<const float4*>(pts + (size_t) o * 12);
    float4 a = p[0], b = p[1], c = p[2];
    pxyz[i] = make_float4(a.x, a.y, a.z, __int_as_float(o));
    pnrm[i] = make_float4(b.x, b.y, b.z, c.y);
}

constexpr int KNN_BLOCK = 128;

template <int MODE>
__global__ __launch_bounds__(KNN_BLOCK) void knn_kernel(GridDev g, const float* __restrict__ q, int nq, int k,
                                                        int32_t* __restrict__ idx, float* __restrict__ d2, int by_grid) {
    extern __shared__ float smem[];
    float* sd = smem;
    int* si = (int*) (smem + (size_t) k * KNN_BLOCK);
    int i = blockIdx.x * KNN_BLOCK + threadIdx.x;
    bool active = true;
    if (by_grid == 1) {
        i = lgr_xcd_tile(blockIdx.x, cdiv_dev(g.n, KNN_BLOCK)) * KNN_BLOCK + threadIdx.x;
        active = i < g.n;
        i = active ? __float_as_int(g.pxyz[i].w) : 0;
    } else if (i >= nq) { active = false; i = 0; }
    float x = 0.f, y = 0.f, z = 0.f;
    if (active) { x = q[(size_t) i * 12]; y = q[(size_t) i * 12 + 1]; z = q[(size_t) i * 12 + 2]; }
    if (by_grid == 2 && lgr_finite3(x, y, z)) active = false;
    KnnList<KNN_BLOCK> L;
    L.init(sd, si, k, threadIdx.x);
    if (active && lgr_finite3(x, y, z) && g.n > 0) lgr_knn_query(g, x, y, z, L);
    if (MODE == 0) {
        const int lane = threadIdx.x & 63, wbase = threadIdx.x & ~63;
        const int my_row = active ? i : -1, my_cnt = L.count;
        for (int r = 0; r < 64; ++r) {
            const int row = __builtin_amdgcn_readlane(my_row, r);
            if (row < 0) continue;
            const int cnt = __builtin_amdgcn_readlane(my_cnt, r);
            for (int j = lane; j < k; j += 64) {
                idx[(size_t) row * k + j] = j < cnt ? si[j * KNN_BLOCK + wbase + r] : -1;
                if (d2) d2[(size_t) row * k + j] = j < cnt ? sd[j * KNN_BLOCK + wbase + r] : INFINITY;
            }
        }
    } else if (active) {
        d2[i] = L.count >= k ? __builtin_sqrtf(L.dist(k - 1)) : __uint_as_float(0x7fc00000u);
        idx[i] = L.count >= 2 ? L.index(1) : i;
    }
}

constexpr int WK_WAVES = 4, WK_Q = 32;
template <int MODE, int KPL>
__device__ __forceinline__ void knn_wave_emit(const WaveKnn<KPL>& W, int m, int i, int k, int32_t* __restrict__ idx, float* __restrict__ d2) {
    const int lane = threadIdx.x & 63;
    if (MODE == 0) {
        const int mk = min(m, k);
#pragma unroll
        for (int j = 0; j < KPL; ++j)
            if (m > 0 && W.rank[j] < mk) {
                idx[(size_t) i * k + W.rank[j]] = (int) (unsigned) W.key[j];
                if (d2) d2[(size_t) i * k + W.rank[j]] = wk_key_d2(W.key[j]);
            }
        for (int j = mk + lane; j < k; j += 64) {
            idx[(size_t) i * k + j] = -1;
            if (d2) d2[(size_t) i * k + j] = INFINITY;
        }
    } else {
        if (m >= k) {
#pragma unroll
            for (int j = 0; j < KPL; ++j) if (W.rank[j] == k - 1) d2[i] = __builtin_sqrtf(wk_key_d2(W.key[j]));
        } else if (lane == 0) d2[i] = __uint_as_float(0x7fc00000u);
        if (m >= 2) {
#pragma unroll
            for (int j = 0; j < KPL; ++j) if (W.rank[j] == 1) idx[i] = (int) (unsigned) W.key[j];
        } else if (lane == 0) idx[i] = i;
    }
}

template <int MODE, int KPL>
__global__ __launch_bounds__(64 * WK_WAVES) void knn_wave_kernel(GridDev g, const float* __restrict__ q, int nq, int k,
                                                                  int32_t* __restrict__ idx, float* __restrict__ d2, int by_grid, float r2_init) {
    __shared__ unsigned long long sbuf[WK_WAVES][WaveKnn<KPL>::BUF];
    const int lane = threadIdx.x & 63, wv = threadIdx.x >> 6;
    const int t0 = (blockIdx.x * WK_WAVES + wv) * WK_Q;
    int qi = -1;
    float qx = 0.f, qy = 0.f, qz = 0.f;
    if (lane < WK_Q && t0 + lane < nq) {
        qi = t0 + lane;
        qx = q[(size_t) qi * 12]; qy = q[(size_t) qi * 12 + 1]; qz = q[(size_t) qi * 12 + 2];
        if (by_grid == 2 && lgr_finite3(qx, qy, qz)) qi = -1;
    }
    float guess = r2_init;
    WaveKnn<KPL> W;
    const int nloc = min(WK_Q, nq - t0);
    for (int l = 0; l < nloc; ++l) {
        const int i = __builtin_amdgcn_readlane(qi, l);
        if (i < 0) continue;
        const float x = __uint_as_float(__builtin_amdgcn_readlane(__float_as_uint(qx), l));
        const float y = __uint_as_float(__builtin_amdgcn_readlane(__float_as_uint(qy), l));
        const float z = __uint_as_float(__builtin_amdgcn_readlane(__float_as_uint(qz), l));
        W.m = 0;
        if (lgr_finite3(x, y, z) && g.n > 0) lgr_wave_knn<KPL>(g, x, y, z, k, guess, sbuf[wv], W);
        knn_wave_emit<MODE, KPL>(W, W.m, i, k, idx, d2);
    }
}

template <int MODE, int KPL>
__global__ __launch_bounds__(64 * WK_WAVES) void knn_tile_kernel(GridDev g, int k, int32_t* __restrict__ idx, float* __restrict__ d2, float r2_init) {
    __shared__ unsigned long long sbuf[WK_WAVES][WaveKnn<KPL>::BUF];
    __shared__ int srow[WK_WAVES][128];
    const int lane = threadIdx.x & 63, wv = threadIdx.x >> 6;
    const int n_tiles = cdiv_dev(g.n, WK_WAVES * 64);
    const int tile = lgr_xcd_tile(blockIdx.x, n_tiles);
    if (tile >= n_tiles) return;
    const int t = (tile * WK_WAVES + wv) * 64 + lane;
    int qi = -1;
    float px = 0.f, py = 0.f, pz = 0.f;
    if (t < g.n) {
        const float4 p = g.pxyz[t];
        qi = __float_as_int(p.w); px = p.x; py = p.y; pz = p.z;
    }
    float guess = r2_init;
    lgr_wave_knn_tile<KPL>(g, qi >= 0, px, py, pz, k, guess, sbuf[wv], srow[wv], [&](int l, const WaveKnn<KPL>& W) {
        knn_wave_emit<MODE, KPL>(W, W.m, __builtin_amdgcn_readlane(qi, l), k, idx, d2);
    });
}

static float wk_r2_init(const GridDev& g, int k, float ppc) { return g.h * g.h * 1.25f * (float) k / (3.14159265f * ppc); }

template <int MODE>
static void knn_wave_launch(lgr_ctx* ctx, const GridDev& g, const float* d_q, int nq, int k, int32_t* d_idx, float* d_d2, int by_grid, float ppc) {
    const float r2i = wk_r2_init(g, k, ppc);
    const int T = 64 * WK_WAVES;
    if (by_grid == 1) {
        if (g.n <= 0) return;
        const int grid = lgr_xcd_grid(cdiv(g.n, WK_WAVES * 64));
        if (k <= 40) knn_tile_kernel<MODE, 1><<<grid, T, 0, ctx->stream>>>(g, k, d_idx, d_d2, r2i);
        else if (k <= 96) knn_tile_kernel<MODE, 2><<<grid, T, 0, ctx->stream>>>(g, k, d_idx, d_d2, r2i);
        else knn_tile_kernel<MODE, 4><<<grid, T, 0, ctx->stream>>>(g, k, d_idx, d_d2, r2i);
        return;
    }
    if (nq <= 0) return;
    const int grid = cdiv(nq, WK_WAVES * WK_Q);
    if (k <= 40) knn_wave_kernel<MODE, 1><<<grid, T, 0, ctx->stream>>>(g, d_q, nq, k, d_idx, d_d2, by_grid, r2i);
    else if (k <= 96) knn_wave_kernel<MODE, 2><<<grid, T, 0, ctx->stream>>>(g, d_q, nq, k, d_idx, d_d2, by_grid, r2i);
    else knn_wave_kernel<MODE, 4><<<grid, T, 0, ctx->stream>>>(g, d_q, nq, k, d_idx, d_d2, by_grid, r2i);
}

__global__ void density_min(const float* __restrict__ dk, const int32_t* __restrict__ nn1, int n, float* __restrict__ out) {
    int i = blockIdx.x * blockDim.x + threadIdx.x;
    if (i >= n) return;
    float a = dk[i], b = dk[nn1[i]];
    out[i] = (b < a) ? b : a;
}

}

int lgr_bbox_launch(lgr_ctx* ctx, const float* d_pts, int n, const unsigned** d_keys12) {
    unsigned* d;
    LGR_TRY(lgr_ws_t(ctx, WS_GRID_MISC, 16, &d));
    unsigned init[12];
    unsigned pinf = 0x7f800000u | 0x80000000u;
    unsigned ninf = ~0xff800000u;
    float fmx = 3.4028234663852886e38f, fmn = 1.17549435e-38f;
    unsigned kfmx, kfmn;
    memcpy(&kfmx, &fmx, 4); kfmx |= 0x80000000u;
    memcpy(&kfmn, &fmn, 4); kfmn |= 0x80000000u;
    for (int a = 0; a < 3; ++a) { init[a] = pinf; init[3 + a] = ninf; init[6 + a] = kfmx; init[9 + a] = kfmn; }
    LGR_HIP(ctx, hipMemcpyAsync(d, init, sizeof init, hipMemcpyHostToDevice, ctx->stream));
    if (n > 0) bbox_kernel<<<std::min(cdiv(n, 256), ctx->n_cu), 256, 0, ctx->stream>>>(d_pts, n, d);
    LGR_HIP(ctx, hipGetLastError());
    *d_keys12 = d;
    return LGR_OK;
}

int lgr_bbox_host(lgr_ctx* ctx, const float* d_pts, int n, float* out12) {
    const unsigned* d;
    LGR_TRY(lgr_bbox_launch(ctx, d_pts, n, &d));
    unsigned* h;
    LGR_TRY(lgr_pinned(ctx, 64, (void**) &h));
    LGR_HIP(ctx, hipMemcpyAsync(h, d, 48, hipMemcpyDeviceToHost, ctx->stream));
    LGR_HIP(ctx, hipStreamSynchronize(ctx->stream));
    for (int i = 0; i < 12; ++i) out12[i] = fkey_inv(h[i]);
    return LGR_OK;
}

extern "C" int lgr_bbox_dev(lgr_ctx* ctx, const float* d_pts, int n, float* d_min3_max3) {
    lgr_turn turn__(ctx);
    if (!ctx) return LGR_ERR_INVALID_ARG;
    LGR_CHECK(ctx, (d_pts || n == 0) && d_min3_max3 && n >= 0, LGR_ERR_INVALID_ARG);
    float bb[12];
    LGR_TRY(lgr_bbox_host(ctx, d_pts, n, bb));
    LGR_HIP(ctx, hipMemcpyAsync(d_min3_max3, bb + 6, 24, hipMemcpyHostToDevice, ctx->stream));
    LGR_HIP(ctx, hipStreamSynchronize(ctx->stream));
    return LGR_OK;
}

int lgr_grid_build(lgr_ctx* ctx, int sb, const float* d_pts, int n, float h, float target, GridDev* out) {
    float bb[12];
    LGR_TRY(lgr_bbox_host(ctx, d_pts, n, bb));
    float mn[3] = {bb[0], bb[1], bb[2]}, mx[3] = {bb[3], bb[4], bb[5]};
    if (!(mn[0] <= mx[0])) { for (int a = 0; a < 3; ++a) { mn[a] = 0.f; mx[a] = 0.f; } }
    if (!(h > 0.f)) {
        float e[3] = {mx[0] - mn[0], mx[1] - mn[1], mx[2] - mn[2]};
        std::sort(e, e + 3);
        float area = std::max(e[2] * e[1], 1e-12f);
        h = std::sqrt(area * target / (float) std::max(n, 1));
        h = std::max(h, std::max(e[2] / 1024.f, 1e-6f));
    }
    int dim[3];
    for (;;) {
        double cells = 1;
        for (int a = 0; a < 3; ++a) {
            dim[a] = (int) std::floor((mx[a] - mn[a]) / h) + 1;
            if (dim[a] < 1) dim[a] = 1;
            cells *= dim[a];
        }
        if (cells <= 256e6) break;
        h *= 2.f;
    }
    int ncell = dim[0] * dim[1] * dim[2];
    unsigned *keys, *keys2;
    int *vals, *vals2, *start;
    float4 *pxyz, *pnrm;
    LGR_TRY(lgr_ws_t(ctx, sb + 0, (size_t) n + 1, &keys));
    LGR_TRY(lgr_ws_t(ctx, sb + 1, (size_t) n + 1, &vals));
    LGR_TRY(lgr_ws_t(ctx, sb + 2, (size_t) n + 1, &keys2));
    LGR_TRY(lgr_ws_t(ctx, sb + 3, (size_t) n + 1, &vals2));
    LGR_TRY(lgr_ws_t(ctx, sb + 4, (size_t) ncell + 2, &start));
    LGR_TRY(lgr_ws_t(ctx, sb + 5, (size_t) n + 1, &pxyz));
    LGR_TRY(lgr_ws_t(ctx, sb + 6, (size_t) n + 1, &pnrm));
    int nvalid = 0;
    if (n > 0) {
        cell_keys<<<cdiv(n, 256), 256, 0, ctx->stream>>>(d_pts, n, mn[0], mn[1], mn[2], h, dim[0], dim[1], dim[2], (unsigned) ncell, keys, vals);
        int bits = 1;
        while (((unsigned long long) 1 << bits) <= (unsigned long long) ncell) ++bits;
        LGR_TRY(lgr_sort_pairs_u32(ctx, keys, keys2, vals, vals2, (size_t) n, 0, bits));
        const int nblk = (int) (((size_t) ncell + 1 + CSF_CELLS - 1) >> CSF_SHIFT);
        int* coarse;
        LGR_TRY(lgr_ws_t(ctx, WS_GRID_MISC, (size_t) nblk + 1 + 64, &coarse));
        coarse += 64;
        coarse_start_fill<<<cdiv(n + 1, 256), 256, 0, ctx->stream>>>(keys2, n, nblk, coarse);
        cell_start_fill<<<nblk, CSF_T, 0, ctx->stream>>>(keys2, coarse, (unsigned) ncell, start);
        int* h_n;
        LGR_TRY(lgr_pinned(ctx, 64, (void**) &h_n));
        LGR_HIP(ctx, hipMemcpyAsync(h_n, start + ncell, 4, hipMemcpyDeviceToHost, ctx->stream));
        LGR_HIP(ctx, hipStreamSynchronize(ctx->stream));
        nvalid = *h_n;
        if (nvalid > 0) gather_points<<<cdiv(nvalid, 256), 256, 0, ctx->stream>>>(d_pts, vals2, nvalid, pxyz, pnrm);
    } else {
        LGR_HIP(ctx, hipMemsetAsync(start, 0, ((size_t) ncell + 2) * 4, ctx->stream));
    }
    LGR_HIP(ctx, hipGetLastError());
    out->ox = mn[0]; out->oy = mn[1]; out->oz = mn[2]; out->h = h;
    out->dx = dim[0]; out->dy = dim[1]; out->dz = dim[2];
    out->n = nvalid; out->cell_start = start; out->pxyz = pxyz; out->pnrm = pnrm;
    return LGR_OK;
}

extern "C" int lgr_knn_dev(lgr_ctx* ctx, const float* d_q, int nq, const float* d_pts, int n, int k, int32_t* d_idx, float* d_d2) {
    lgr_turn turn__(ctx);
    if (!ctx) return LGR_ERR_INVALID_ARG;
    LGR_CHECK(ctx, d_d2 != nullptr, LGR_ERR_INVALID_ARG);
    return lgr_knn_lists(ctx, d_q, nq, d_pts, n, k, d_idx, d_d2);
}

int lgr_knn_lists(lgr_ctx* ctx, const float* d_q, int nq, const float* d_pts, int n, int k, int32_t* d_idx, float* d_d2) {
    LGR_CHECK(ctx, nq >= 0 && n >= 0 && k >= 1 && k <= 128 && (d_q || nq == 0) && (d_pts || n == 0) && d_idx, LGR_ERR_INVALID_ARG);
    if (nq == 0) return LGR_OK;
    LGR_HIP(ctx, hipSetDevice(ctx->device));
    GridDev g;
    const float ppc = std::max(4.f, 0.35f * (float) k);
    LGR_TRY(lgr_grid_build(ctx, WS_GRID_A, d_pts, n, 0.f, ppc, &g));
    size_t sm = (size_t) k * KNN_BLOCK * 8;
    const bool heap = k < 16;
    if (!heap) {
        if (d_q == d_pts && nq == n) {
            knn_wave_launch<0>(ctx, g, d_q, nq, k, d_idx, d_d2, 1, ppc);
            if (g.n < nq) knn_wave_launch<0>(ctx, g, d_q, nq, k, d_idx, d_d2, 2, ppc);
        } else {
            knn_wave_launch<0>(ctx, g, d_q, nq, k, d_idx, d_d2, 0, ppc);
        }
    } else if (d_q == d_pts && nq == n) {
        if (g.n > 0) knn_kernel<0><<<lgr_xcd_grid(cdiv(g.n, KNN_BLOCK)), KNN_BLOCK, sm, ctx->stream>>>(g, d_q, nq, k, d_idx, d_d2, 1);
        if (g.n < nq) knn_kernel<0><<<cdiv(nq, KNN_BLOCK), KNN_BLOCK, sm, ctx->stream>>>(g, d_q, nq, k, d_idx, d_d2, 2);
    } else {
        knn_kernel<0><<<cdiv(nq, KNN_BLOCK), KNN_BLOCK, sm, ctx->stream>>>(g, d_q, nq, k, d_idx, d_d2, 0);
    }
    LGR_HIP(ctx, hipGetLastError());
    return LGR_OK;
}

extern "C" int lgr_smoothed_densities_dev(lgr_ctx* ctx, const float* d_pts, int n, int k, float* d_out) {
    lgr_turn turn__(ctx);
    if (!ctx) return LGR_ERR_INVALID_ARG;
    LGR_CHECK(ctx, d_pts && d_out && n > 1 && k >= 2 && k <= 128, LGR_ERR_INVALID_ARG);
    LGR_HIP(ctx, hipSetDevice(ctx->device));
    GridDev g;
    LGR_TRY(lgr_grid_build(ctx, WS_GRID_A, d_pts, n, 0.f, 4.f, &g));
    float* dk; int32_t* nn1;
    LGR_TRY(lgr_ws_t(ctx, WS_DENS_A, (size_t) n, &dk));
    LGR_TRY(lgr_ws_t(ctx, WS_DENS_B, (size_t) n, &nn1));
    size_t sm = (size_t) k * KNN_BLOCK * 8;
    const bool heap = k < 16;
    if (!heap) {
        knn_wave_launch<1>(ctx, g, d_pts, n, k, nn1, dk, 1, 4.f);
        if (g.n < n) knn_wave_launch<1>(ctx, g, d_pts, n, k, nn1, dk, 2, 4.f);
    } else {
    if (g.n > 0) knn_kernel<1><<<lgr_xcd_grid(cdiv(g.n, KNN_BLOCK)), KNN_BLOCK, sm, ctx->stream>>>(g, d_pts, n, k, nn1, dk, 1);
    if (g.n < n) knn_kernel<1><<<cdiv(n, KNN_BLOCK), KNN_BLOCK, sm, ctx->stream>>>(g, d_pts, n, k, nn1, dk, 2);
    }
    density_min<<<cdiv(n, 256), 256, 0, ctx->stream>>>(dk, nn1, n, d_out);
    LGR_HIP(ctx, hipGetLastError());
    return LGR_OK;
}

extern "C" int lgr_smoothed_densities(lgr_ctx* ctx, const float* pts, int n, int k, float* out) {
    lgr_turn turn__(ctx);
    if (!ctx) return LGR_ERR_INVALID_ARG;
    LGR_CHECK(ctx, pts && out && n > 1, LGR_ERR_INVALID_ARG);
    LGR_HIP(ctx, hipSetDevice(ctx->device));
    float *dp, *dout;
    LGR_TRY(lgr_ws_t(ctx, WS_HOST_A, (size_t) n * 12, &dp));
    LGR_TRY(lgr_ws_t(ctx, WS_HOST_C, (size_t) n, &dout));
    LGR_HIP(ctx, hipMemcpyAsync(dp, pts, (size_t) n * 48, hipMemcpyHostToDevice, ctx->stream));
    LGR_TRY(lgr_smoothed_densities_dev(ctx, dp, n, k, dout));
    LGR_HIP(ctx, hipMemcpyAsync(out, dout, (size_t) n * 4, hipMemcpyDeviceToHost, ctx->stream));
    LGR_HIP(ctx, hipStreamSynchronize(ctx->stream));
    return LGR_OK;
}
```

lidar-global-registration_amd/csrc/lgr_internal.h:

```cpp
#pragma once
#include <hip/hip_runtime.h>
#include <stdint.h>
#include <stdio.h>
#include <string.h>

#include <condition_variable>
#include <functional>
#include <mutex>
#include <string>
#include <thread>
#include <vector>

#include "../../include/lgr.h"

#define LGR_WAVE 64
#define LGR_STREAM_OWN_LOW ((void*) (intptr_t) -2)

struct lgr_buf {
    void* p = nullptr;
    size_t cap = 0;
};

struct lgr_match_stats { unsigned items_ab, dense_ab, items_ba, dense_ba; int sub_cols, rg_rows; double stages_done, stages_all, stages_unique; int f16; double coarse_tested, coarse_rejected; unsigned pairs_ab, pairs_ba; double shell_skipped; double lb_zero, lb_finite; unsigned irr_a, irr_b, irr_gave_up; };

struct lgr_helper {
    std::thread th;
    std::mutex mu;
    std::condition_variable cv;
    std::function<int()> job;
    bool has_job = false, busy = false, quit = false, started = false;
    int rc = 0;
};

struct lgr_ctx {
    int device = 0;
    hipStream_t stream = nullptr;
    bool own_stream = false;
    std::string err;
    lgr_buf ws[112];
    void* pinned = nullptr;
    size_t pinned_cap = 0;
    hipEvent_t ev[32];
    float stage_ms[12];
    int n_cu = 256;
    int mfma_timed = 0;
    lgr_match_options mopt{-1, 0, 0, -1, 1, 1, 1, 1, -1, 0, 0, 1, 1, 0, 1, 1};
    bool corr_trusted = false;
    void* match_prep = nullptr;
    void (*match_prep_free)(void*) = nullptr;
    lgr_ctx* aux = nullptr;
    hipEvent_t aux_ev = nullptr;
    lgr_ctx* aux2 = nullptr;
    hipEvent_t aux2_ev = nullptr;
    hipStream_t stream3 = nullptr;
    hipEvent_t ev3 = nullptr;
    lgr_ctx_options opt{1, 0, LGR_ARITH_FAST, 0, 0, {0, 0, 0}};
    lgr_helper* helper = nullptr;
    lgr_match_stats mstats{};
    double mcheck[2] = {-1, -1};
    unsigned long long mcover[8] = {~0ull, ~0ull, ~0ull, ~0ull, ~0ull, ~0ull, ~0ull, ~0ull};
    bool internal = false;
    int turn_depth = 0;
    unsigned long long turn_id = 0;
};

struct lgr_turn {
    lgr_ctx* c = nullptr;
    bool held = false;
    explicit lgr_turn(lgr_ctx* ctx);
    ~lgr_turn();
    lgr_turn(const lgr_turn&) = delete;
    lgr_turn& operator=(const lgr_turn&) = delete;
};

int lgr_fail(lgr_ctx* ctx, int code, const char* what, const char* file, int line);

#define LGR_HIP(ctx, call)                                                                 \
    do {                                                                                   \
        hipError_t e__ = (call);                                                           \
        if (e__ != hipSuccess) {                                                           \
            char b__[512];                                                                 \
            snprintf(b__, sizeof b__, "%s -> %s", #call, hipGetErrorString(e__));          \
            return lgr_fail(ctx, e__ == hipErrorOutOfMemory ? LGR_ERR_OOM : LGR_ERR_HIP, b__, __FILE__, __LINE__); \
        }                                                                                  \
    } while (0)

#define LGR_CHECK(ctx, cond, code)                                                         \
    do {                                                                                   \
        if (!(cond)) return lgr_fail(ctx, code, #cond, __FILE__, __LINE__);                \
    } while (0)

#define LGR_TRY(expr)                 \
    do {                              \
        int rc__ = (expr);            \
        if (rc__ != LGR_OK) return rc__; \
    } while (0)

enum {
    WS_MATCH_AP = 0, WS_MATCH_BP, WS_MATCH_NA, WS_MATCH_NB, WS_MATCH_ROWMIN, WS_MATCH_COLMIN, WS_MATCH_ITEMS,
    WS_MATCH_BEST_A, WS_MATCH_BEST_B, WS_MATCH_MISC, WS_MATCH_DENSE, WS_MATCH_SORTED_A, WS_MATCH_SORTED_B, WS_MATCH_PRUNE, WS_MATCH_ITEMS2, WS_MATCH_NORMS, WS_MATCH_PAIRS, WS_MATCH_KEPT,
    WS_GRID_A, WS_GRID_B = WS_GRID_A + 7, WS_GRID_C = WS_GRID_B + 7, WS_GRID_TMP = WS_GRID_C + 7, WS_GRID_MISC,
    WS_DS_KEYS, WS_DS_VALS, WS_DS_KEYS2, WS_DS_VALS2, WS_DS_FLAGS, WS_DS_MISC,
    WS_SPFH, WS_KP_ORDER, WS_DENS_A, WS_DENS_B, WS_DENS_C,
    WS_RANSAC_T, WS_RANSAC_STATS, WS_RANSAC_PACK, WS_RANSAC_LIST, WS_RANSAC_HIST, WS_RANSAC_MISC, WS_RANSAC_MASK, WS_RANSAC_MASKT,
    WS_PIPE_SURF_S, WS_PIPE_SURF_T, WS_PIPE_FEAT_S, WS_PIPE_FEAT_T, WS_PIPE_IJ, WS_PIPE_JI, WS_PIPE_DIJ, WS_PIPE_DJI,
    WS_PIPE_CORR, WS_PIPE_KNN_S, WS_PIPE_KNN_T, WS_PIPE_FLAGS, WS_PIPE_MISC, WS_PIPE_KIDX_S, WS_PIPE_KIDX_T, WS_PIPE_KPS_S, WS_PIPE_KPS_T,
    WS_MS_KNN_I, WS_MS_KNN_D, WS_MS_LIST_S, WS_MS_LIST_T, WS_MS_SUB, WS_MS_FEAT_S, WS_MS_FEAT_T, WS_MS_SURF2, WS_MS_RES, WS_PLANE_VISITED, WS_PLANE_CLAIMED, WS_PLANE_OUT, WS_LOCAL_G, WS_SORT_TMP, WS_MATCH_BOX, WS_RANSAC_GHIST,
    WS_HOST_A, WS_HOST_B, WS_HOST_C, WS_HOST_D, WS_HOST_E, WS_HOST_F,
    WS_SHOT_PACK_A, WS_SHOT_PACK_B, WS_SHOT_KEYS,
    WS_ROPS_MASKED, WS_ROPS_LRF, WS_ROPS_KPS,
    WS_WEIGHTS, WS_WEIGHTS_KNN, WS_WEIGHTS_TMP, WS_WEIGHTS_VALS, WS_WEIGHTS_SUM, WS_WEIGHTS_HOST,
    WS_COUNT
};
static_assert(WS_COUNT <= 112, "grow lgr_ctx::ws");

int lgr_ws(lgr_ctx* ctx, int slot, size_t bytes, void** out);
int lgr_pinned(lgr_ctx* ctx, size_t bytes, void** out);

template <class T>
static inline int lgr_ws_t(lgr_ctx* ctx, int slot, size_t count, T** out) {
    void* p = nullptr;
    int rc = lgr_ws(ctx, slot, count * sizeof(T), &p);
    *out = (T*) p;
    return rc;
}

static inline int cdiv(long long a, long long b) { return (int) ((a + b - 1) / b); }
static inline size_t cdivz(size_t a, size_t b) { return (a + b - 1) / b; }

struct GridDev {
    float ox, oy, oz, h;
    int dx, dy, dz;
    int n;
    const int* cell_start;
    const float4* pxyz;
    const float4* pnrm;
};
int lgr_grid_build(lgr_ctx* ctx, int slot_base, const float* d_pts, int n, float h, float target, GridDev* out);
int lgr_rops_gravity_dev(lgr_ctx* ctx, const float* d_kps, int m, const float* d_surf, int n, float radius, float* d_out135);
int lgr_bbox_host(lgr_ctx* ctx, const float* d_pts, int n, float* out12);
int lgr_bbox_launch(lgr_ctx* ctx, const float* d_pts, int n, const unsigned** d_keys12);
__host__ __device__ inline float lgr_bbox_key_inv(unsigned k) {
    const unsigned b = (k & 0x80000000u) ? (k & 0x7fffffffu) : ~k;
    float f;
    memcpy(&f, &b, 4);
    return f;
}
int lgr_knn_lists(lgr_ctx* ctx, const float* d_q, int nq, const float* d_pts, int n, int k, int32_t* d_idx, float* d_d2);

int lgr_ctx_aux(lgr_ctx* ctx);
int lgr_ctx_aux2(lgr_ctx* ctx);
int lgr_ctx_stream3(lgr_ctx* ctx, hipStream_t* out);
int lgr_helper_post(lgr_ctx* owner, lgr_ctx* aux, std::function<int()> job);
int lgr_helper_wait(lgr_ctx* aux);
struct lgr_helper_guard {
    lgr_ctx* aux = nullptr;
    bool armed = false;
    int wait() { armed = false; return lgr_helper_wait(aux); }
    ~lgr_helper_guard() { if (armed) (void) lgr_helper_wait(aux); }
};
template <class F>
static inline std::function<int()> lgr_aux_job(lgr_ctx* aux, F&& f) {
    return [aux, &f]() -> int {
        int rc = hipSetDevice(aux->device) == hipSuccess ? f(aux) : (int) LGR_ERR_HIP;
        const hipError_t e = hipStreamSynchronize(aux->stream);
        if (rc == LGR_OK && e != hipSuccess) rc = lgr_fail(aux, LGR_ERR_HIP, hipGetErrorString(e), __FILE__, __LINE__);
        return rc;
    };
}
template <class FA, class FB>
static inline int lgr_run_pair(lgr_ctx* ctx, FA&& fa, FB&& fb) {
    LGR_TRY(lgr_ctx_aux(ctx));
    lgr_ctx* ax = ctx->aux;
    if (!ctx->opt.helper_contexts) {
        LGR_TRY(fa(ctx));
        const int rc = fb(ax);
        if (rc != LGR_OK) ctx->err = ax->err;
        return rc;
    }
    LGR_HIP(ctx, hipEventRecord(ctx->aux_ev, ctx->stream));
    LGR_HIP(ctx, hipStreamWaitEvent(ax->stream, ctx->aux_ev, 0));
    lgr_helper_guard g{ax, false};
    LGR_TRY(lgr_helper_post(ctx, ax, lgr_aux_job(ax, fb)));
    g.armed = true;
    const int rc_a = fa(ctx);
    const int rc_b = g.wait();
    (void) hipSetDevice(ctx->device);
    if (rc_b != LGR_OK) { ctx->err = ax->err; return rc_b; }
    return rc_a;
}

int lgr_check_corr(lgr_ctx* ctx, const lgr_corr* d_corr, int c, int ns, int nt);
int lgr_sort_pairs_u32(lgr_ctx* ctx, const unsigned* kin, unsigned* kout, const int* vin, int* vout, size_t n, int begin_bit, int end_bit);
int lgr_sort_pairs_u64(lgr_ctx* ctx, const unsigned long long* kin, unsigned long long* kout, const int* vin, int* vout, size_t n,
                       const int* shifts, const int* widths, int n_ranges);
int lgr_match_prepare(lgr_ctx* ctx, const float* d_a33, int ma, int mb, bool both);
void lgr_match_prepare_cancel(lgr_ctx* ctx);

struct lgr_plane_dev {
    GridDev g;
    float thr, r2;
    int n_sp, ns;
    const float* d_src;
    uint64_t seed;
    unsigned* visited;
    int* claimed;
    int n_wg;
    const float* w = nullptr;
    float w_sum = 0.f, w_gate = 0.f;
};
int lgr_plane_setup(lgr_ctx* ctx, const float* d_src, int ns, const float* d_tgt, int nt, uint64_t seed, lgr_plane_dev* out);
int lgr_weights_map(lgr_ctx* ctx, const float* d_pts, int n, int weight_id, int nr_points, float* d_w);
int lgr_weights_sum(lgr_ctx* ctx, const float* d_w, int n, float* sum, float* w_max, int* n_bad);
int lgr_weights_prepare(lgr_ctx* ctx, const float* d_src, int ns, const lgr_metric_params* mp, const float** d_w, float* w_sum, float* w_gate);
int lgr_weights_libm_launch(lgr_ctx* ctx, int fn, const float* d_a, long long n, float* d_out);
struct lgr_plane_dyn { const int* nh; const int* counter_base; const float* best_prev; const int* record_prev; };
int lgr_plane_eval(lgr_ctx* ctx, const lgr_plane_dev& pd, const float* d_Ts, const int* d_list, int nh, unsigned counter_base, int score_id,
                   int* d_cnt, float* d_metric, float* d_rmse, int2* d_pairs, int* d_n_pairs, float best_prev = 0.f, int record_prev = 0x7fffffff,
                   const float* d_factor = nullptr, const lgr_plane_dyn* dyn = nullptr);
```

lidar-global-registration_amd/csrc/lgr_sort.hip:

```cpp
#include <algorithm>

#include "lgr_internal.h"

namespace {

constexpr int RS_THREADS = 256, RS_ITEMS = 8, RS_TILE = RS_THREADS * RS_ITEMS, RS_SLOTS = RS_ITEMS * (RS_THREADS / 64);

template <class K>
__global__ __launch_bounds__(RS_THREADS) void rs_count(const K* __restrict__ keys, size_t n, int shift, unsigned mask, int nblk, unsigned* __restrict__ counts ) {
    __shared__ unsigned h[256];
    h[threadIdx.x] = 0u;
    __syncthreads();
    const size_t base = (size_t) blockIdx.x * RS_TILE;
#pragma unroll
    for (int r = 0; r < RS_ITEMS; ++r) {
        const size_t i = base + (size_t) r * RS_THREADS + threadIdx.x;
        if (i < n) atomicAdd(&h[(unsigned) (keys[i] >> shift) & mask], 1u);
    }
    __syncthreads();
    counts[(size_t) threadIdx.x * nblk + blockIdx.x] = h[threadIdx.x];
}

__global__ __launch_bounds__(256) void rs_scan(unsigned* __restrict__ counts, int nblk, unsigned* __restrict__ tot) {
    __shared__ unsigned wsum[4];
    __shared__ unsigned carry_s;
    unsigned* row = counts + (size_t) blockIdx.x * nblk;
    const int tid = threadIdx.x, lane = tid & 63, wave = tid >> 6;
    if (tid == 0) carry_s = 0u;
    __syncthreads();
    for (int b0 = 0; b0 < nblk; b0 += 256) {
        const int b = b0 + tid;
        const unsigned c = b < nblk ? row[b] : 0u;
        unsigned incl = c;
        for (int o = 1; o < 64; o <<= 1) { const unsigned t = __shfl_up(incl, o); if (lane >= o) incl += t; }
        if (lane == 63) wsum[wave] = incl;
        __syncthreads();
        unsigned before = carry_s;
        for (int w = 0; w < wave; ++w) before += wsum[w];
        if (b < nblk) row[b] = before + incl - c;
        __syncthreads();
        if (tid == 255) carry_s = before + incl;
        __syncthreads();
    }
    if (tid == 0) tot[blockIdx.x] = carry_s;
}

template <class K>
__global__ __launch_bounds__(RS_THREADS) void rs_scatter(const K* __restrict__ kin, const int* __restrict__ vin, K* __restrict__ kout, int* __restrict__ vout,
                                                         size_t n, int shift, unsigned mask, int nblk, const unsigned* __restrict__ offs ,
                                                         const unsigned* __restrict__ tot ) {
    __shared__ unsigned short hist[RS_SLOTS][256];
    __shared__ unsigned goff[256];
    __shared__ unsigned short tstart[257];
    __shared__ unsigned wsum[4];
    __shared__ K sk[RS_TILE];
    __shared__ int sv[RS_TILE];
    const int tid = threadIdx.x, lane = tid & 63, wave = tid >> 6;
    for (int e = tid; e < RS_SLOTS * 256; e += RS_THREADS) (&hist[0][0])[e] = 0;
    {
        const unsigned c = tot[tid];
        unsigned incl = c;
        for (int o = 1; o < 64; o <<= 1) { const unsigned t = __shfl_up(incl, o); if (lane >= o) incl += t; }
        if (lane == 63) wsum[wave] = incl;
        __syncthreads();
        unsigned before = 0u;
        for (int w = 0; w < wave; ++w) before += wsum[w];
        goff[tid] = before + incl - c + offs[(size_t) tid * nblk + blockIdx.x];
    }
    __syncthreads();
    const size_t base = (size_t) blockIdx.x * RS_TILE;
    const int n_tile = (int) min((size_t) RS_TILE, n - base);
    const unsigned long long lt = (1ull << lane) - 1ull;
    K key[RS_ITEMS];
    int val[RS_ITEMS];
    unsigned short wrank[RS_ITEMS];
#pragma unroll
    for (int r = 0; r < RS_ITEMS; ++r) {
        const int e = r * RS_THREADS + tid;
        const bool valid = e < n_tile;
        key[r] = valid ? kin[base + e] : (K) 0;
        val[r] = valid ? vin[base + e] : 0;
        const unsigned d = (unsigned) (key[r] >> shift) & mask;
        unsigned long long peers = __ballot(valid);
#pragma unroll
        for (int b = 0; b < 8; ++b) {
            const bool bit = (d >> b) & 1u;
            const unsigned long long bal = __ballot(bit);
            peers &= bit ? bal : ~bal;
        }
        wrank[r] = (unsigned short) __popcll(peers & lt);
        if (valid && (peers & lt) == 0ull) hist[r * (RS_THREADS / 64) + wave][d] = (unsigned short) __popcll(peers);
    }
    __syncthreads();
    {
        unsigned run = 0u;
#pragma unroll 4
        for (int s = 0; s < RS_SLOTS; ++s) { const unsigned c = hist[s][tid]; hist[s][tid] = (unsigned short) run; run += c; }
        unsigned incl = run;
        for (int o = 1; o < 64; o <<= 1) { const unsigned t = __shfl_up(incl, o); if (lane >= o) incl += t; }
        __syncthreads();
        if (lane == 63) wsum[wave] = incl;
        __syncthreads();
        unsigned before = 0u;
        for (int w = 0; w < wave; ++w) before += wsum[w];
        tstart[tid] = (unsigned short) (before + incl - run);
        if (tid == 255) tstart[256] = (unsigned short) (before + incl);
    }
    __syncthreads();
#pragma unroll
    for (int r = 0; r < RS_ITEMS; ++r) {
        const int e = r * RS_THREADS + tid;
        if (e >= n_tile) continue;
        const unsigned d = (unsigned) (key[r] >> shift) & mask;
        const int tp = tstart[d] + hist[r * (RS_THREADS / 64) + wave][d] + wrank[r];
        sk[tp] = key[r];
        sv[tp] = val[r];
    }
    __syncthreads();
#pragma unroll
    for (int r = 0; r < RS_ITEMS; ++r) {
        const int e = r * RS_THREADS + tid;
        if (e >= n_tile) continue;
        const K k = sk[e];
        const unsigned d = (unsigned) (k >> shift) & mask;
        const size_t pos = (size_t) goff[d] + (unsigned) (e - tstart[d]);
        kout[pos] = k;
        vout[pos] = sv[e];
    }
}

__global__ void rs_copy(const unsigned* __restrict__ a, unsigned* __restrict__ b, size_t nwords) {
    size_t i = (size_t) blockIdx.x * blockDim.x + threadIdx.x;
    if (i < nwords) b[i] = a[i];
}

template <class K>
int sort_impl(lgr_ctx* ctx, const K* kin, K* kout, const int* vin, int* vout, size_t n, const int* shifts, const int* widths, int np) {
    if (n == 0) return LGR_OK;
    LGR_CHECK(ctx, kin && kout && vin && vout && (const void*) kin != (const void*) kout && vin != vout && n < ((size_t) 1 << 31), LGR_ERR_INVALID_ARG);
    int dsh[16], dw[16], nd = 0;
    for (int p = 0; p < np; ++p)
        for (int b = 0; b < widths[p]; b += 8) {
            LGR_CHECK(ctx, nd < 16, LGR_ERR_INVALID_ARG);
            dsh[nd] = shifts[p] + b; dw[nd] = std::min(8, widths[p] - b); ++nd;
        }
    if (nd == 0) {
        rs_copy<<<cdiv((long long) (n * sizeof(K) / 4), 256), 256, 0, ctx->stream>>>((const unsigned*) kin, (unsigned*) kout, n * sizeof(K) / 4);
        rs_copy<<<cdiv((long long) n, 256), 256, 0, ctx->stream>>>((const unsigned*) vin, (unsigned*) vout, n);
        LGR_HIP(ctx, hipGetLastError());
        return LGR_OK;
    }
    const int nblk = (int) ((n + RS_TILE - 1) / RS_TILE);
    char* tmp;
    const size_t kb = (n * sizeof(K) + 255) & ~(size_t) 255, vb = (n * 4 + 255) & ~(size_t) 255;
    LGR_TRY(lgr_ws_t(ctx, WS_SORT_TMP, kb + vb + (size_t) nblk * 256 * 4 + 1024, &tmp));
    K* tk = (K*) tmp;
    int* tv = (int*) (tmp + kb);
    unsigned* tot = (unsigned*) (tmp + kb + vb);
    unsigned* counts = tot + 256;
    const K* sk = kin;
    const int* sv = vin;
    for (int p = 0; p < nd; ++p) {
        const bool to_out = ((nd - 1 - p) & 1) == 0;
        K* dk = to_out ? kout : tk;
        int* dv = to_out ? vout : tv;
        const unsigned mask = (1u << dw[p]) - 1u;
        rs_count<K><<<nblk, RS_THREADS, 0, ctx->stream>>>(sk, n, dsh[p], mask, nblk, counts);
        rs_scan<<<256, 256, 0, ctx->stream>>>(counts, nblk, tot);
        rs_scatter<K><<<nblk, RS_THREADS, 0, ctx->stream>>>(sk, sv, dk, dv, n, dsh[p], mask, nblk, counts, tot);
        sk = dk; sv = dv;
    }
    LGR_HIP(ctx, hipGetLastError());
    return LGR_OK;
}

}

int lgr_sort_pairs_u32(lgr_ctx* ctx, const unsigned* kin, unsigned* kout, const int* vin, int* vout, size_t n, int begin_bit, int end_bit) {
    const int sh = begin_bit, w = std::max(0, end_bit - begin_bit);
    return sort_impl<unsigned>(ctx, kin, kout, vin, vout, n, &sh, &w, 1);
}
int lgr_sort_pairs_u64(lgr_ctx* ctx, const unsigned long long* kin, unsigned long long* kout, const int* vin, int* vout, size_t n,
                       const int* shifts, const int* widths, int n_ranges) {
    return sort_impl<unsigned long long>(ctx, kin, kout, vin, vout, n, shifts, widths, n_ranges);
}

extern "C" int lgr_sort_pairs_u32_dev(lgr_ctx* ctx, const uint32_t* kin, uint32_t* kout, const int32_t* vin, int32_t* vout, size_t n, int begin_bit, int end_bit) {
    lgr_turn turn__(ctx);
    if (!ctx) return LGR_ERR_INVALID_ARG;
    LGR_CHECK(ctx, begin_bit >= 0 && end_bit <= 32 && begin_bit <= end_bit, LGR_ERR_INVALID_ARG);
    LGR_HIP(ctx, hipSetDevice(ctx->device));
    return lgr_sort_pairs_u32(ctx, kin, kout, vin, vout, n, begin_bit, end_bit);
}
extern "C" int lgr_sort_pairs_u64_dev(lgr_ctx* ctx, const uint64_t* kin, uint64_t* kout, const int32_t* vin, int32_t* vout, size_t n,
                                      const int* shifts, const int* widths, int n_ranges) {
    lgr_turn turn__(ctx);
    if (!ctx) return LGR_ERR_INVALID_ARG;
    LGR_CHECK(ctx, n_ranges >= 0 && n_ranges <= 8 && (n_ranges == 0 || (shifts && widths)), LGR_ERR_INVALID_ARG);
    for (int i = 0; i < n_ranges; ++i) LGR_CHECK(ctx, shifts[i] >= 0 && widths[i] >= 0 && shifts[i] + widths[i] <= 64, LGR_ERR_INVALID_ARG);
    LGR_HIP(ctx, hipSetDevice(ctx->device));
    return lgr_sort_pairs_u64(ctx, (const unsigned long long*) kin, (unsigned long long*) kout, vin, vout, n, shifts, widths, n_ranges);
}
```

lidar-global-registration_amd/lgr_amd/capi.py:

```python
import ctypes as C
import os

import numpy as np

try:
    import torch as _torch
except ImportError:
    _torch = None

_CSRC = os.path.join(os.path.dirname(os.path.dirname(os.path.abspath(__file__))), "csrc")
LIB_PATH = os.environ.get("LGR_HIP_LIB") or os.path.join(_CSRC, "liblgr_hip.so")

MATCH_LR, MATCH_ONE_SIDED, MATCH_CLUSTER = 0, 1, 2
METRIC_CORRESPONDENCES, METRIC_UNIFORMITY, METRIC_CLOSEST_PLANE, METRIC_COMBINATION, METRIC_WEIGHTED_CLOSEST_PLANE = 0, 1, 2, 3, 4
WEIGHT_CONSTANT, WEIGHT_EXP_CURVATURE, WEIGHT_CURVEDNESS, WEIGHT_HARRIS, WEIGHT_TOMASI, WEIGHT_CURVATURE, WEIGHT_NSS = 0, 1, 2, 3, 4, 5, 6
WEIGHT_IDS = {"constant": 0, "exp_curvature": 1, "curvedness": 2, "harris": 3, "tomasi": 4, "curvature": 5, "nss": 6}
KEYPOINT_ANY, KEYPOINT_ISS = 0, 1
SCORE_CONSTANT, SCORE_MAE, SCORE_MSE, SCORE_EXP = 0, 1, 2, 3
ALIGN_RANSAC, ALIGN_GROR = 0, 1
ORDER_REFERENCE, ORDER_CANONICAL = 0, 1
DESCRIPTOR_FPFH, DESCRIPTOR_SHOT, DESCRIPTOR_ROPS = 0, 1, 2
LRF_DEFAULT, LRF_GRAVITY, LRF_GT = 0, 1, 2
ERR_UNSUPPORTED = -5
ERR_INVALID_ARG = -1

CORR_DTYPE = np.dtype([("index_query", "<i4"), ("index_match", "<i4"), ("distance", "<f4"), ("threshold", "<f4")])


class Params(C.Structure):
    _fields_ = [
        ("feature_nr_points", C.c_int32), ("normal_nr_points", C.c_int32), ("edge_thr_coef", C.c_float),
        ("distance_thr", C.c_float), ("feature_radius", C.c_float), ("scale_factor", C.c_float),
        ("confidence", C.c_float), ("bf_block_size", C.c_int32), ("cluster_k", C.c_int32),
        ("randomness", C.c_int32), ("n_samples", C.c_int32),
        ("alignment_id", C.c_int32), ("matching_id", C.c_int32), ("metric_id", C.c_int32), ("score_id", C.c_int32),
        ("max_iterations", C.c_int32), ("normals_available", C.c_int32), ("fix_seed", C.c_int32),
        ("has_vp_src", C.c_int32), ("has_vp_tgt", C.c_int32), ("vp_src", C.c_float * 3), ("vp_tgt", C.c_float * 3),
        ("ransac_batch", C.c_int32), ("seed", C.c_uint64),
        ("keypoint_id", C.c_int32), ("iss_radius_src", C.c_float), ("iss_radius_tgt", C.c_float), ("use_bfmatcher", C.c_int32),
        ("has_guess", C.c_int32), ("match_search_radius", C.c_float), ("guess", C.c_float * 16),
    ]


class Result(C.Structure):
    _fields_ = [
        ("transformation", C.c_float * 16), ("iterations", C.c_int32), ("converged", C.c_int32),
        ("n_inliers", C.c_int32), ("metric", C.c_float), ("best_metric_before_refit", C.c_float),
        ("best_iteration", C.c_int32), ("num_rejections", C.c_int32), ("estimated_iters", C.c_int32),
        ("n_correspondences", C.c_int32), ("time_cs", C.c_double), ("time_te", C.c_double),
        ("stage_ms", C.c_float * 12),
    ]

    def matrix(self):
        return np.array(self.transformation, dtype=np.float32).reshape(4, 4).T.copy()


class MatchOptions(C.Structure):
    _fields_ = [("prune", C.c_int32), ("leaves", C.c_int32), ("near", C.c_int32), ("operand_format", C.c_int32), ("box_bounds", C.c_int32),
                ("column_stage", C.c_int32), ("coarse_rejection", C.c_int32), ("rerank_refilter", C.c_int32), ("pair_cap", C.c_int32),
                ("poison_tables", C.c_int32), ("self_check", C.c_int32), ("shell_bound", C.c_int32), ("split_sweep", C.c_int32), ("kept_cap", C.c_int32), ("auto_dense", C.c_int32),
                ("irregular_rows", C.c_int32)]


class CtxOptions(C.Structure):
    _fields_ = [("helper_contexts", C.c_int32), ("concurrent_contexts", C.c_int32), ("arithmetic", C.c_int32), ("pcl_neighbour_cap", C.c_int32),
                ("ransac_schedule", C.c_int32), ("reserved", C.c_int32 * 3)]


RANSAC_SCHEDULE_DEFAULT, RANSAC_SCHEDULE_CHAIN, RANSAC_SCHEDULE_RESIDENT = 0, 1, 2
ARITH_FAST, ARITH_PCL = 0, 1
LIBM_ACOSF, LIBM_ATANF, LIBM_ATAN2F, LIBM_SINF, LIBM_COSF = 0, 1, 2, 3, 4


FORMAT_AUTO, FORMAT_F32, FORMAT_F16, FORMAT_F16R = -1, 0, 1, 2


class FeatureParams(C.Structure):
    _fields_ = [("descriptor_id", C.c_int32), ("lrf_id", C.c_int32), ("reserved", C.c_int32 * 6)]


def feature_params(descriptor="fpfh", lrf_id=None):
    f = FeatureParams()
    _lib.lgr_default_feature_params(C.byref(f))
    f.descriptor_id = {"fpfh": DESCRIPTOR_FPFH, "shot": DESCRIPTOR_SHOT, "rops": DESCRIPTOR_ROPS}.get(descriptor, descriptor)
    if lrf_id is None:
        lrf_id = LRF_GRAVITY if f.descriptor_id == DESCRIPTOR_ROPS else LRF_DEFAULT
    f.lrf_id = int(lrf_id)
    return f


class MetricParams(C.Structure):
    _fields_ = [("weight_id", C.c_int32), ("reserved", C.c_int32 * 5), ("weights", C.c_void_p)]


def metric_params(weight="constant", weights=None):
    m = MetricParams()
    _lib.lgr_default_metric_params(C.byref(m))
    m.weight_id = WEIGHT_IDS.get(weight, weight) if isinstance(weight, str) else int(weight)
    if weights is not None:
        m.weights = _ptr(weights).value
    return m


class LgrError(RuntimeError):
    pass


def load():
    if not os.path.exists(LIB_PATH):
        raise ImportError(
            f"{LIB_PATH} is missing: build it with `make -C {_CSRC}` (or __graft_entry__.build()). "
            "The MI355X HIP extension is mandatory; there is no CPU fallback.")
    return C.CDLL(LIB_PATH)


ABI_VERSION = 5

_lib = load()
_lib.lgr_last_error.restype = C.c_char_p
_lib.lgr_last_error.argtypes = [C.c_void_p]
if _lib.lgr_version() != ABI_VERSION:
    raise ImportError(f"{LIB_PATH} has ABI revision {_lib.lgr_version()}, this binding needs {ABI_VERSION}: rebuild it (make -C {_CSRC})")


def lib():
    return _lib


def default_params(**kw):
    p = Params()
    _lib.lgr_default_params(C.byref(p))
    for k, v in kw.items():
        if k in ("vp_src", "vp_tgt"):
            setattr(p, k, (C.c_float * 3)(*[float(x) for x in v]))
            setattr(p, "has_" + k, 1)
        elif k == "guess":
            p.guess = (C.c_float * 16)(*np.asarray(v, np.float32).T.reshape(16).tolist())
            p.has_guess = 1
        else:
            assert hasattr(p, k), k
            setattr(p, k, v)
    return p


def _ptr(t):
    if t is None:
        return None
    if isinstance(t, np.ndarray):
        return t.ctypes.data_as(C.c_void_p)
    return C.c_void_p(t.data_ptr())


class Context:

    def __init__(self, device=0, stream=None):
        import torch
        self.torch = torch
        self.device = int(device)
        self.foreign_stream = stream is not None and stream != torch.cuda.current_stream(self.device).cuda_stream
        if stream is None:
            stream = torch.cuda.current_stream(self.device).cuda_stream
        h = C.c_void_p()
        rc = _lib.lgr_ctx_create(self.device, C.c_void_p(stream), C.byref(h))
        if rc != 0:
            raise LgrError(f"lgr_ctx_create failed: {rc}")
        self.h = h

    def close(self):
        if self.h:
            _lib.lgr_ctx_destroy(self.h)
            self.h = None

    def __del__(self):
        try:
            self.close()
        except Exception:
            pass

    def check(self, rc):
        if rc != 0:
            raise LgrError(f"rc={rc}: {_lib.lgr_last_error(self.h).decode()}")

    def sync(self):
        self.check(_lib.lgr_ctx_sync(self.h))

    def _join(self):
        if self.foreign_stream:
            self.sync()

    def set_match_options(self, **kw):
        o = MatchOptions()
        _lib.lgr_match_default_options(C.byref(o))
        for k, v in kw.items():
            assert hasattr(o, k), k
            setattr(o, k, int(v))
        self.check(_lib.lgr_ctx_set_match_options(self.h, C.byref(o)))
        return o

    def match_options(self):
        o = MatchOptions()
        self.check(_lib.lgr_ctx_get_match_options(self.h, C.byref(o)))
        return o

    def set_options(self, **kw):
        o = CtxOptions()
        _lib.lgr_ctx_default_options(C.byref(o))
        for k, v in kw.items():
            assert hasattr(o, k), k
            setattr(o, k, int(v))
        self.check(_lib.lgr_ctx_set_options(self.h, C.byref(o)))
        return o

    def host_threads(self):
        n = C.c_int(0)
        self.check(_lib.lgr_ctx_host_threads(self.h, C.byref(n)))
        return n.value

    def workspace_bytes(self):
        out = C.c_uint64(0)
        self.check(_lib.lgr_ctx_workspace_bytes(self.h, C.byref(out)))
        return int(out.value)

    def _dev(self):
        return self.torch.device("cuda", self.device)

    def empty(self, shape, dtype):
        return self.torch.empty(shape, dtype=dtype, device=self._dev())

    def match_bf(self, q, t, block=10000):
        torch = self.torch
        q = q.contiguous(); t = t.contiguous()
        idx = self.empty((q.shape[0],), torch.int32)
        dist = self.empty((q.shape[0],), torch.float32)
        self.check(_lib.lgr_match_bf_dev(self.h, _ptr(q), q.shape[0], _ptr(t), t.shape[0], int(block), _ptr(idx), _ptr(dist)))
        return idx, dist

    def match_bf2(self, a, b, block=10000):
        torch = self.torch
        a = a.contiguous(); b = b.contiguous()
        ab_i = self.empty((a.shape[0],), torch.int32); ab_d = self.empty((a.shape[0],), torch.float32)
        ba_i = self.empty((b.shape[0],), torch.int32); ba_d = self.empty((b.shape[0],), torch.float32)
        self.check(_lib.lgr_match_bf2_dev(self.h, _ptr(a), a.shape[0], _ptr(b), b.shape[0], int(block),
                                          _ptr(ab_i), _ptr(ab_d), _ptr(ba_i), _ptr(ba_d)))
        return ab_i, ab_d, ba_i, ba_d

    def sort_pairs_u32(self, keys, vals, begin_bit=0, end_bit=32):
        torch = self.torch
        keys = keys.contiguous(); vals = vals.contiguous()
        ko = self.empty((keys.shape[0],), torch.int32); vo = self.empty((keys.shape[0],), torch.int32)
        self.check(_lib.lgr_sort_pairs_u32_dev(self.h, _ptr(keys), _ptr(ko), _ptr(vals), _ptr(vo), C.c_size_t(keys.shape[0]), int(begin_bit), int(end_bit)))
        return ko, vo

    def sort_pairs_u64(self, keys, vals, ranges):
        torch = self.torch
        keys = keys.contiguous(); vals = vals.contiguous()
        ko = self.empty((keys.shape[0],), torch.int64); vo = self.empty((keys.shape[0],), torch.int32)
        sh = (C.c_int * max(1, len(ranges)))(*[r[0] for r in ranges]); wd = (C.c_int * max(1, len(ranges)))(*[r[1] for r in ranges])
        self.check(_lib.lgr_sort_pairs_u64_dev(self.h, _ptr(keys), _ptr(ko), _ptr(vals), _ptr(vo), C.c_size_t(keys.shape[0]), sh, wd, len(ranges)))
        return ko, vo

    def match_flann(self, q, t):
        torch = self.torch
        q = q.contiguous(); t = t.contiguous()
        idx = self.empty((q.shape[0],), torch.int32)
        dist = self.empty((q.shape[0],), torch.float32)
        self.check(_lib.lgr_match_flann_dev(self.h, _ptr(q), q.shape[0], _ptr(t), t.shape[0], _ptr(idx), _ptr(dist)))
        return idx, dist

    def match_local(self, qpts, tpts, qf, tf, guess, radius):
        torch = self.torch
        g = (C.c_float * 16)(*np.asarray(guess, np.float32).T.reshape(16).tolist())
        idx = self.empty((qpts.shape[0],), torch.int32)
        dist = self.empty((qpts.shape[0],), torch.float32)
        self.check(_lib.lgr_match_local_dev(self.h, _ptr(qpts), qpts.shape[0], _ptr(tpts), tpts.shape[0], _ptr(qf.contiguous()), _ptr(tf.contiguous()),
                                            g, C.c_float(radius), _ptr(idx), _ptr(dist)))
        return idx, dist

    def match_bf_host(self, q, t, block=10000):
        q = np.ascontiguousarray(q, np.float32); t = np.ascontiguousarray(t, np.float32)
        idx = np.zeros(q.shape[0], np.int32); dist = np.zeros(q.shape[0], np.float32)
        self.check(_lib.lgr_match_bf(self.h, _ptr(q), q.shape[0], _ptr(t), t.shape[0], int(block), _ptr(idx), _ptr(dist)))
        return idx, dist

    def match_stats(self):
        out = (C.c_uint * 6)()
        self.check(_lib.lgr_match_last_stats(self.h, out))
        return dict(items_ab=out[0], dense_ab=out[1], items_ba=out[2], dense_ba=out[3], sub_cols=out[4], rg_rows=out[5])

    def match_work(self):
        f = C.c_double(1.0)
        self.check(_lib.lgr_match_last_work(self.h, C.byref(f)))
        return f.value

    def selfcheck_rcp(self, lo, hi):
        out = (C.c_ulonglong * 2)()
        lo_b, hi_b = (int(np.float32(v).view(np.uint32)) for v in (lo, hi))
        self.check(_lib.lgr_selfcheck_rcp(self.h, C.c_uint(lo_b), C.c_uint(hi_b), out))
        return int(out[0]), int(out[1])

    def match_lbstats(self):
        out = (C.c_double * 2)()
        self.check(_lib.lgr_match_last_lbstats(self.h, out))
        return out[0], out[1]

    def match_irregular(self):
        out = (C.c_uint * 3)()
        self.check(_lib.lgr_match_last_irregular(self.h, out))
        return int(out[0]), int(out[1]), int(out[2])

    def selfcheck_philox(self, key, counter4):
        c = (C.c_uint32 * 4)(*[int(x) for x in counter4])
        out = (C.c_uint32 * 4)()
        self.check(_lib.lgr_selfcheck_philox(self.h, C.c_uint64(key), c, out))
        return list(out)

    def selfcheck_libm(self, fn, a, b=None):
        a = np.ascontiguousarray(a, np.float32)
        b = np.ascontiguousarray(a if b is None else b, np.float32)
        out = np.empty_like(a)
        self.check(_lib.lgr_selfcheck_libm(self.h, int(fn), a.ctypes.data_as(C.c_void_p), b.ctypes.data_as(C.c_void_p), C.c_longlong(a.size), out.ctypes.data_as(C.c_void_p)))
        return out

    def match_issued(self):
        out = (C.c_double * 2)()
        self.check(_lib.lgr_match_last_issued(self.h, out))
        return out[0]

    def match_issued_pairs(self):
        out = (C.c_double * 2)()
        self.check(_lib.lgr_match_last_issued(self.h, out))
        return out[1]

    def match_pairs(self):
        out = (C.c_uint * 2)()
        self.check(_lib.lgr_match_last_pairs(self.h, out))
        return out[0], out[1]

    def match_coarse(self):
        out = (C.c_double * 2)()
        self.check(_lib.lgr_match_last_coarse(self.h, out))
        return out[0], out[1]

    def match_shell(self):
        out = C.c_double()
        self.check(_lib.lgr_match_last_shell(self.h, C.byref(out)))
        return out.value

    def match_format(self):
        v = C.c_int(0)
        self.check(_lib.lgr_match_last_format(self.h, C.byref(v)))
        return {0: "f32", 1: "f16", 2: "f16r"}[v.value]

    def match_check(self):
        out = (C.c_double * 2)()
        self.check(_lib.lgr_match_last_check(self.h, out))
        return out[0], out[1]

    def match_check_cover(self):
        out = (C.c_ulonglong * 8)()
        self.check(_lib.lgr_match_last_check_cover(self.h, out))
        keys = ("entries", "upper", "waived", "colstage")
        return {d: {k: (-1 if out[4 * j + n] == 0xFFFFFFFFFFFFFFFF else int(out[4 * j + n])) for n, k in enumerate(keys)}
                for j, d in enumerate(("rows", "cols"))}

    def match_kernel_ms(self):
        ms = C.c_float(0)
        self.check(_lib.lgr_match_last_kernel_ms(self.h, C.byref(ms)))
        return ms.value

    def bbox(self, pts):
        out = self.empty((6,), self.torch.float32)
        self.check(_lib.lgr_bbox_dev(self.h, _ptr(pts), pts.shape[0], _ptr(out)))
        return out

    def knn(self, q, pts, k):
        torch = self.torch
        idx = self.empty((q.shape[0], k), torch.int32); d2 = self.empty((q.shape[0], k), torch.float32)
        self.check(_lib.lgr_knn_dev(self.h, _ptr(q), q.shape[0], _ptr(pts), pts.shape[0], int(k), _ptr(idx), _ptr(d2)))
        return idx, d2

    def smoothed_densities(self, pts, k=2):
        out = self.empty((pts.shape[0],), self.torch.float32)
        self.check(_lib.lgr_smoothed_densities_dev(self.h, _ptr(pts), pts.shape[0], int(k), _ptr(out)))
        return out

    def preprocess(self, pts, vp=None, normals_available=False):
        out = self.empty((pts.shape[0], 12), self.torch.float32)
        n = C.c_int(0)
        voxel = C.c_float(0)
        v = (C.c_float * 3)(*[float(x) for x in vp]) if vp is not None else None
        self.check(_lib.lgr_preprocess_dev(self.h, _ptr(pts), pts.shape[0], v, int(normals_available), _ptr(out), C.byref(n), C.byref(voxel)))
        return out[: n.value], voxel.value

    def preprocess_host(self, pts, vp=None, normals_available=False, order=ORDER_CANONICAL):
        pts = np.ascontiguousarray(pts, np.float32)
        out = np.zeros_like(pts)
        n = C.c_int(0)
        voxel = C.c_float(0)
        v = (C.c_float * 3)(*[float(x) for x in vp]) if vp is not None else None
        self.check(_lib.lgr_preprocess(self.h, _ptr(pts), pts.shape[0], v, int(normals_available), int(order), _ptr(out), C.byref(n), C.byref(voxel)))
        return out[: n.value].copy(), voxel.value

    def dedupe(self, pts):
        out = self.empty((max(pts.shape[0], 1), 12), self.torch.float32)
        n = C.c_int(0)
        self.check(_lib.lgr_dedupe_dev(self.h, _ptr(pts), pts.shape[0], _ptr(out), C.byref(n)))
        return out[: n.value]

    def cloud_density(self, pts, quantile=0.8):
        v = C.c_float(0)
        self.check(_lib.lgr_cloud_density_dev(self.h, _ptr(pts), pts.shape[0], C.c_float(quantile), C.byref(v)))
        return v.value

    def iss_keypoints(self, pts, radius, gamma21=0.975, gamma32=0.975, min_neighbors=4):
        idx = self.empty((max(pts.shape[0], 1),), self.torch.int32)
        n = C.c_int(0)
        self.check(_lib.lgr_iss_keypoints_dev(self.h, _ptr(pts), pts.shape[0], C.c_float(radius), C.c_float(gamma21), C.c_float(gamma32),
                                              int(min_neighbors), _ptr(idx), C.byref(n)))
        return idx[: n.value]

    def downsample(self, pts, voxel):
        out = self.empty((pts.shape[0], 12), self.torch.float32)
        n = C.c_int(0)
        self.check(_lib.lgr_downsample_dev(self.h, _ptr(pts), pts.shape[0], C.c_float(voxel), _ptr(out), C.byref(n)))
        return out[: n.value]

    def downsample_host(self, pts, voxel, order=ORDER_CANONICAL):
        pts = np.ascontiguousarray(pts, np.float32)
        out = np.zeros_like(pts)
        n = C.c_int(0)
        self.check(_lib.lgr_downsample(self.h, _ptr(pts), pts.shape[0], C.c_float(voxel), int(order), _ptr(out), C.byref(n)))
        return out[: n.value].copy()

    def normals_knn(self, pts, k=30, surf=None, vp=None):
        v = (C.c_float * 3)(*[float(x) for x in vp]) if vp is not None else None
        self.check(_lib.lgr_normals_knn_dev(self.h, _ptr(pts), pts.shape[0], _ptr(surf), 0 if surf is None else surf.shape[0],
                                            int(k), v, 0))
        return pts

    def fpfh(self, kps, surf, radius):
        out = self.empty((kps.shape[0], 33), self.torch.float32)
        self.check(_lib.lgr_fpfh_dev(self.h, _ptr(kps), kps.shape[0], _ptr(surf), surf.shape[0], C.c_float(radius), _ptr(out)))
        return out

    def shot_lrf(self, kps, surf, radius):
        out = self.empty((kps.shape[0], 9), self.torch.float32)
        self.check(_lib.lgr_shot_lrf_dev(self.h, _ptr(kps), kps.shape[0], _ptr(surf), surf.shape[0], C.c_float(radius), _ptr(out)))
        return out

    def shot(self, kps, surf, radius, lrf=None, with_lrf=False):
        out = self.empty((kps.shape[0], 352), self.torch.float32)
        lo = self.empty((kps.shape[0], 9), self.torch.float32) if with_lrf else None
        self.check(_lib.lgr_shot_dev(self.h, _ptr(kps), kps.shape[0], _ptr(surf), surf.shape[0], C.c_float(radius),
                                     _ptr(None if lrf is None else lrf.contiguous()), _ptr(out), _ptr(lo)))
        return (out, lo) if with_lrf else out

    def shot_host(self, kps, surf, radius, lrf=None):
        kps = np.ascontiguousarray(kps, np.float32); surf = np.ascontiguousarray(surf, np.float32)
        out = np.zeros((kps.shape[0], 352), np.float32)
        lo = np.zeros((kps.shape[0], 9), np.float32)
        lrf = None if lrf is None else np.ascontiguousarray(lrf, np.float32)
        self.check(_lib.lgr_shot(self.h, _ptr(kps), kps.shape[0], _ptr(surf), surf.shape[0], C.c_float(radius), _ptr(lrf), _ptr(out), _ptr(lo)))
        return out, lo

    def match_shot(self, q, t, block=10000):
        torch = self.torch
        q = q.contiguous(); t = t.contiguous()
        idx = self.empty((q.shape[0],), torch.int32)
        dist = self.empty((q.shape[0],), torch.float32)
        self.check(_lib.lgr_match_shot_dev(self.h, _ptr(q), q.shape[0], _ptr(t), t.shape[0], int(block), _ptr(idx), _ptr(dist)))
        return idx, dist

    def match2_shot(self, a, b, block=10000):
        torch = self.torch
        a = a.contiguous(); b = b.contiguous()
        ab_i = self.empty((a.shape[0],), torch.int32); ab_d = self.empty((a.shape[0],), torch.float32)
        ba_i = self.empty((b.shape[0],), torch.int32); ba_d = self.empty((b.shape[0],), torch.float32)
        self.check(_lib.lgr_match2_shot_dev(self.h, _ptr(a), a.shape[0], _ptr(b), b.shape[0], int(block),
                                            _ptr(ab_i), _ptr(ab_d), _ptr(ba_i), _ptr(ba_d)))
        return ab_i, ab_d, ba_i, ba_d

    def match_shot_host(self, q, t, block=10000):
        q = np.ascontiguousarray(q, np.float32); t = np.ascontiguousarray(t, np.float32)
        idx = np.zeros(q.shape[0], np.int32); dist = np.zeros(q.shape[0], np.float32)
        self.check(_lib.lgr_match_shot(self.h, _ptr(q), q.shape[0], _ptr(t), t.shape[0], int(block), _ptr(idx), _ptr(dist)))
        return idx, dist

    def gravity_lrf(self, kps, surf, radius):
        out = self.empty((kps.shape[0], 9), self.torch.float32)
        self.check(_lib.lgr_gravity_lrf_dev(self.h, _ptr(kps), kps.shape[0], _ptr(surf), surf.shape[0], C.c_float(radius), _ptr(out)))
        return out

    def gravity_lrf_host(self, kps, surf, radius):
        kps = np.ascontiguousarray(kps, np.float32); surf = np.ascontiguousarray(surf, np.float32)
        out = np.zeros((kps.shape[0], 9), np.float32)
        self.check(_lib.lgr_gravity_lrf(self.h, _ptr(kps), kps.shape[0], _ptr(surf), surf.shape[0], C.c_float(radius), _ptr(out)))
        return out

    def rops(self, kps, surf, radius, lrf):
        out = self.empty((kps.shape[0], 135), self.torch.float32)
        self.check(_lib.lgr_rops_dev(self.h, _ptr(kps), kps.shape[0], _ptr(surf), surf.shape[0], C.c_float(radius), _ptr(lrf.contiguous()),
                                     _ptr(out)))
        return out

    def rops_host(self, kps, surf, radius, lrf):
        kps = np.ascontiguousarray(kps, np.float32); surf = np.ascontiguousarray(surf, np.float32)
        lrf = np.ascontiguousarray(lrf, np.float32)
        out = np.zeros((kps.shape[0], 135), np.float32)
        self.check(_lib.lgr_rops(self.h, _ptr(kps), kps.shape[0], _ptr(surf), surf.shape[0], C.c_float(radius), _ptr(lrf), _ptr(out)))
        return out

    def match_rops(self, q, t, block=10000):
        torch = self.torch
        q = q.contiguous(); t = t.contiguous()
        idx = self.empty((q.shape[0],), torch.int32)
        dist = self.empty((q.shape[0],), torch.float32)
        self.check(_lib.lgr_match_rops_dev(self.h, _ptr(q), q.shape[0], _ptr(t), t.shape[0], int(block), _ptr(idx), _ptr(dist)))
        return idx, dist

    def match2_rops(self, a, b, block=10000):
        torch = self.torch
        a = a.contiguous(); b = b.contiguous()
        ab_i = self.empty((a.shape[0],), torch.int32); ab_d = self.empty((a.shape[0],), torch.float32)
        ba_i = self.empty((b.shape[0],), torch.int32); ba_d = self.empty((b.shape[0],), torch.float32)
        self.check(_lib.lgr_match2_rops_dev(self.h, _ptr(a), a.shape[0], _ptr(b), b.shape[0], int(block),
                                            _ptr(ab_i), _ptr(ab_d), _ptr(ba_i), _ptr(ba_d)))
        return ab_i, ab_d, ba_i, ba_d

    def match_rops_host(self, q, t, block=10000):
        q = np.ascontiguousarray(q, np.float32); t = np.ascontiguousarray(t, np.float32)
        idx = np.zeros(q.shape[0], np.int32); dist = np.zeros(q.shape[0], np.float32)
        self.check(_lib.lgr_match_rops(self.h, _ptr(q), q.shape[0], _ptr(t), t.shape[0], int(block), _ptr(idx), _ptr(dist)))
        return idx, dist

    def fpfh_host(self, kps, surf, radius):
        kps = np.ascontiguousarray(kps, np.float32); surf = np.ascontiguousarray(surf, np.float32)
        out = np.zeros((kps.shape[0], 33), np.float32)
        self.check(_lib.lgr_fpfh(self.h, _ptr(kps), kps.shape[0], _ptr(surf), surf.shape[0], C.c_float(radius), _ptr(out)))
        return out

    def filter(self, matching_id, src, tgt, ij, dij, ji, dji, distance_thr, cluster_k=40):
        out = self.empty((src.shape[0], 4), self.torch.int32)
        n = C.c_int(0)
        self.check(_lib.lgr_filter_dev(self.h, int(matching_id), _ptr(src), src.shape[0], _ptr(tgt), tgt.shape[0],
                                       _ptr(ij), _ptr(dij), _ptr(ji), _ptr(dji), C.c_float(distance_thr), int(cluster_k),
                                       _ptr(out), C.byref(n)))
        self._join()
        return out[: n.value].cpu().numpy().view(CORR_DTYPE).reshape(-1)

    def correspondences(self, src, tgt, params, descriptor="fpfh"):
        out = self.empty((src.shape[0], 4), self.torch.int32)
        n = C.c_int(0)
        if isinstance(descriptor, str) and descriptor == "fpfh":
            self.check(_lib.lgr_correspondences_dev(self.h, _ptr(src), src.shape[0], _ptr(tgt), tgt.shape[0], C.byref(params),
                                                    _ptr(out), C.byref(n)))
        else:
            f = descriptor if isinstance(descriptor, FeatureParams) else feature_params(descriptor)
            self.check(_lib.lgr_correspondences_ex_dev(self.h, _ptr(src), src.shape[0], _ptr(tgt), tgt.shape[0], C.byref(params),
                                                       C.byref(f), _ptr(out), C.byref(n)))
        return out[: n.value]

    def stage_ms(self):
        out = (C.c_float * 12)()
        _lib.lgr_ctx_stage_ms(self.h, out)
        return list(out)

    def _corr_dev(self, corr):
        if isinstance(corr, np.ndarray):
            return self.torch.from_numpy(np.ascontiguousarray(corr).view(np.int32).reshape(-1, 4)).to(self._dev())
        return corr

    def ransac_samples(self, seed, first, n, n_corr, n_samples=3):
        out = self.empty((n, n_samples), self.torch.int32)
        self.check(_lib.lgr_ransac_samples_n_dev(self.h, C.c_uint64(seed), int(first), int(n), int(n_corr), int(n_samples), _ptr(out)))
        return out

    def evaluate(self, src, tgt, corr, T, metric_id=METRIC_UNIFORMITY, score_id=SCORE_MSE):
        corr = self._corr_dev(corr)
        c = corr.shape[0]
        mask = self.empty((max(c, 1),), self.torch.uint8)
        T16 = (C.c_float * 16)(*np.asarray(T, np.float32).T.reshape(16).tolist())
        ni, rm, me = C.c_int(0), C.c_float(0), C.c_float(0)
        self.check(_lib.lgr_evaluate_dev(self.h, _ptr(src), src.shape[0], _ptr(tgt), tgt.shape[0], _ptr(corr), c, T16,
                                         int(metric_id), int(score_id), _ptr(mask), C.byref(ni), C.byref(rm), C.byref(me)))
        self._join()
        return mask[:c].cpu().numpy(), ni.value, rm.value, me.value

    def choose_best_hypothesis(self, src, tgt, corr, tns):
        corr = self._corr_dev(corr)
        n = len(tns)
        buf = np.ascontiguousarray(np.stack([np.asarray(T, np.float32).T.reshape(16) for T in tns]), np.float32) if n else np.zeros((1, 16), np.float32)
        out = (C.c_float * 16)()
        bi = C.c_int(-1)
        uni = np.zeros(max(n, 1), np.float32)
        self.check(_lib.lgr_choose_best_hypothesis_dev(self.h, _ptr(src), src.shape[0], _ptr(tgt), tgt.shape[0], _ptr(corr), corr.shape[0],
                                                       _ptr(buf), n, out, C.byref(bi), _ptr(uni)))
        return bi.value, np.array(out, np.float32).reshape(4, 4).T.copy(), uni[:n].copy()

    def evaluate_plane(self, src, tgt, T, score_id=SCORE_CONSTANT, seed=566, counter=0, with_pairs=False):
        T16 = (C.c_float * 16)(*np.asarray(T, np.float32).T.reshape(16).tolist())
        n, rm, me, th, npairs = C.c_int(0), C.c_float(0), C.c_float(0), C.c_float(0), C.c_int(0)
        pairs = np.zeros((max(int(0.01 * src.shape[0]), 1), 2), np.int32) if with_pairs else None
        self.check(_lib.lgr_evaluate_plane_dev(self.h, _ptr(src), src.shape[0], _ptr(tgt), tgt.shape[0], T16, int(score_id), C.c_uint64(seed),
                                               C.c_uint32(counter), C.byref(n), C.byref(rm), C.byref(me), C.byref(th), _ptr(pairs), C.byref(npairs)))
        out = dict(n_inl=n.value, rmse=rm.value, metric=me.value, thr=th.value)
        if with_pairs:
            out["pairs"] = pairs[: npairs.value].copy()
        return out

    def evaluate_plane_weighted(self, src, tgt, T, weights, weights_sum, score_id=SCORE_CONSTANT, seed=566, counter=0, with_pairs=False):
        T16 = (C.c_float * 16)(*np.asarray(T, np.float32).T.reshape(16).tolist())
        n, rm, me, th, npairs = C.c_int(0), C.c_float(0), C.c_float(0), C.c_float(0), C.c_int(0)
        pairs = np.zeros((max(int(0.01 * src.shape[0]), 1), 2), np.int32) if with_pairs else None
        self.check(_lib.lgr_evaluate_plane_weighted_dev(self.h, _ptr(src), src.shape[0], _ptr(tgt), tgt.shape[0], T16, int(score_id), C.c_uint64(seed),
                                                        C.c_uint32(counter), _ptr(weights.contiguous()), C.c_float(weights_sum), C.byref(n), C.byref(rm),
                                                        C.byref(me), C.byref(th), _ptr(pairs), C.byref(npairs)))
        out = dict(n_inl=n.value, rmse=rm.value, metric=me.value, thr=th.value)
        if with_pairs:
            out["pairs"] = pairs[: npairs.value].copy()
        return out

    def weights(self, pts, weight="constant", nr_points=30, with_sum=True):
        wid = WEIGHT_IDS.get(weight, weight) if isinstance(weight, str) else int(weight)
        out = self.empty((max(pts.shape[0], 1),), self.torch.float32)
        s = C.c_float(0)
        self.check(_lib.lgr_weights_dev(self.h, _ptr(pts), pts.shape[0], int(wid), int(nr_points), _ptr(out), C.byref(s) if with_sum else None))
        return out[: pts.shape[0]], (s.value if with_sum else None)

    def weights_host(self, pts, weight="constant", nr_points=30):
        pts = np.ascontiguousarray(pts, np.float32)
        wid = WEIGHT_IDS.get(weight, weight) if isinstance(weight, str) else int(weight)
        out = np.zeros(max(pts.shape[0], 1), np.float32)
        s = C.c_float(0)
        self.check(_lib.lgr_weights(self.h, _ptr(pts), pts.shape[0], int(wid), int(nr_points), _ptr(out), C.byref(s)))
        return out[: pts.shape[0]], s.value

    def principal_curvatures(self, pts, k=30):
        n = pts.shape[0]
        pc1 = self.empty((max(n, 1),), self.torch.float32); pc2 = self.empty((max(n, 1),), self.torch.float32)
        self.check(_lib.lgr_principal_curvatures_dev(self.h, _ptr(pts), n, int(k), _ptr(pc1), _ptr(pc2)))
        return pc1[:n], pc2[:n]

    def ransac_ex(self, src, tgt, corr, params, mparams=None):
        corr = self._corr_dev(corr)
        c = corr.shape[0]
        res = Result()
        mask = self.empty((max(c, 1),), self.torch.uint8)
        self.check(_lib.lgr_ransac_ex_dev(self.h, _ptr(src), src.shape[0], _ptr(tgt), tgt.shape[0], _ptr(corr), c,
                                          C.byref(params), C.byref(mparams) if mparams is not None else None, C.byref(res), _ptr(mask)))
        self._join()
        return res, mask[:c].cpu().numpy()

    def ransac_replay(self, src, tgt, corr, params, triples):
        torch = self.torch
        corr = self._corr_dev(corr)
        n = triples.shape[0]
        assert triples.shape[1] == params.n_samples, "one row of params.n_samples correspondence indices per hypothesis"
        ok = self.empty((n,), torch.uint8); Ts = self.empty((n, 16), torch.float32)
        ninl = self.empty((n,), torch.int32); met = self.empty((n,), torch.float32)
        self.check(_lib.lgr_ransac_replay_dev(self.h, _ptr(src), src.shape[0], _ptr(tgt), tgt.shape[0], _ptr(corr), corr.shape[0],
                                              C.byref(params), _ptr(triples), n, _ptr(ok), _ptr(Ts), _ptr(ninl), _ptr(met)))
        self._join()
        return ok.cpu().numpy(), Ts.cpu().numpy(), ninl.cpu().numpy(), met.cpu().numpy()

    def ransac(self, src, tgt, corr, params):
        corr = self._corr_dev(corr)
        c = corr.shape[0]
        res = Result()
        mask = self.empty((max(c, 1),), self.torch.uint8)
        self.check(_lib.lgr_ransac_dev(self.h, _ptr(src), src.shape[0], _ptr(tgt), tgt.shape[0], _ptr(corr), c,
                                       C.byref(params), C.byref(res), _ptr(mask)))
        self._join()
        return res, mask[:c].cpu().numpy()

    def gror(self, src, tgt, corr, resolution, k_optimal=800):
        corr = self._corr_dev(corr)
        c = corr.shape[0]
        res = Result()
        mask = self.empty((max(c, 1),), self.torch.uint8)
        self.check(_lib.lgr_gror_dev(self.h, _ptr(src), src.shape[0], _ptr(tgt), tgt.shape[0], _ptr(corr), c,
                                     C.c_float(resolution), int(k_optimal), C.byref(res), _ptr(mask)))
        self._join()
        return res, mask[:c].cpu().numpy()

    def gror_node_degree(self, src, tgt, corr, resolution):
        corr = self._corr_dev(corr)
        c = corr.shape[0]
        deg = self.empty((max(c, 1),), self.torch.int32)
        self.check(_lib.lgr_gror_node_degree_dev(self.h, _ptr(src), _ptr(tgt), _ptr(corr), c, C.c_float(resolution), _ptr(deg)))
        self._join()
        return deg[:c].cpu().numpy()

    def refit(self, src, tgt, corr, mask=None):
        corr = self._corr_dev(corr)
        T = (C.c_float * 16)()
        self.check(_lib.lgr_refit_svd_dev(self.h, _ptr(src), _ptr(tgt), _ptr(corr), corr.shape[0], _ptr(mask), T))
        return np.array(T, np.float32).reshape(4, 4).T.copy()

    def align(self, src, tgt, params, descriptor="fpfh"):
        res = Result()
        if isinstance(descriptor, str) and descriptor == "fpfh":
            self.check(_lib.lgr_align_dev(self.h, _ptr(src), src.shape[0], _ptr(tgt), tgt.shape[0], C.byref(params), C.byref(res)))
        else:
            f = descriptor if isinstance(descriptor, FeatureParams) else feature_params(descriptor)
            self.check(_lib.lgr_align_ex_dev(self.h, _ptr(src), src.shape[0], _ptr(tgt), tgt.shape[0], C.byref(params), C.byref(f),
                                             C.byref(res)))
        return res

    def align_ex2(self, src, tgt, params, descriptor="fpfh", mparams=None):
        res = Result()
        f = descriptor if isinstance(descriptor, FeatureParams) else feature_params(descriptor)
        self.check(_lib.lgr_align_ex2_dev(self.h, _ptr(src), src.shape[0], _ptr(tgt), tgt.shape[0], C.byref(params), C.byref(f),
                                          C.byref(mparams) if mparams is not None else None, C.byref(res)))
        return res

    def align_ex2_host(self, src, tgt, params, descriptor="fpfh", mparams=None):
        src = np.ascontiguousarray(src, np.float32); tgt = np.ascontiguousarray(tgt, np.float32)
        res = Result()
        f = descriptor if isinstance(descriptor, FeatureParams) else feature_params(descriptor)
        self.check(_lib.lgr_align_ex2(self.h, _ptr(src), src.shape[0], _ptr(tgt), tgt.shape[0], C.byref(params), C.byref(f),
                                      C.byref(mparams) if mparams is not None else None, C.byref(res)))
        return res

    def align_host(self, src, tgt, params, descriptor="fpfh"):
        src = np.ascontiguousarray(src, np.float32); tgt = np.ascontiguousarray(tgt, np.float32)
        res = Result()
        if isinstance(descriptor, str) and descriptor == "fpfh":
            self.check(_lib.lgr_align(self.h, _ptr(src), src.shape[0], _ptr(tgt), tgt.shape[0], C.byref(params), C.byref(res)))
        else:
            f = descriptor if isinstance(descriptor, FeatureParams) else feature_params(descriptor)
            self.check(_lib.lgr_align_ex(self.h, _ptr(src), src.shape[0], _ptr(tgt), tgt.shape[0], C.byref(params), C.byref(f),
                                         C.byref(res)))
        return res
```

Before: 46.31.

## Fuse cell-key generation and point gather into a wider-digit generic radix sort

Replaces the separate cell_keys, u32 pair sort and gather_points steps in grid build with a templated radix sort. The sort computes cell keys on the fly from the point array and, in its last pass, writes the gathered xyz/normal float4s straight to their sorted positions. Digits widen from 8 to 11 bits, which cuts the number of passes and removes the key/value workspaces. The normals path also drops the device-to-device snapshot copy of the input points and reads d_pts directly, which could race if any kernel still reads d_pts while normals are written back into it. A grid_build_dev API and its Python binding are added as well.

Result: no change. 46.73, median of 6 (+0.9%).

```diff
diff --git a/include/lgr.h b/include/lgr.h
--- a/include/lgr.h
+++ b/include/lgr.h
@@ -125,6 +125,9 @@
 int lgr_sort_pairs_u64_dev(lgr_ctx*, const uint64_t* d_keys_in, uint64_t* d_keys_out, const int32_t* d_vals_in, int32_t* d_vals_out,
                            size_t n, const int* shifts, const int* widths, int n_ranges);
 
+int lgr_grid_build_dev(lgr_ctx*, const float* d_pts, int n, float h, float target, float* origin_h, int* dims_n,
+                       int32_t* d_cell_start, size_t cell_capacity, float* d_pxyz, float* d_pnrm);
+
 int lgr_bbox_dev(lgr_ctx*, const float* d_pts, int n, float* d_min3_max3 );
 
 int lgr_preprocess(lgr_ctx*, const float* pts, int n, const float* vp3, int normals_available, int order, float* out, int* n_out, float* voxel_out);
diff --git a/lidar-global-registration_amd/csrc/lgr_features.hip b/lidar-global-registration_amd/csrc/lgr_features.hip
--- a/lidar-global-registration_amd/csrc/lgr_features.hip
+++ b/lidar-global-registration_amd/csrc/lgr_features.hip
@@ -1022,12 +1022,7 @@
     if (n == 0) return LGR_OK;
     LGR_HIP(ctx, hipSetDevice(ctx->device));
     const float* S = d_surf;
-    if (!S) {
-        float* snap;
-        LGR_TRY(lgr_ws_t(ctx, WS_HOST_F, (size_t) n * 12, &snap));
-        LGR_HIP(ctx, hipMemcpyAsync(snap, d_pts, (size_t) n * 48, hipMemcpyDeviceToDevice, ctx->stream));
-        S = snap; ns = n;
-    }
+    if (!S) { S = d_pts; ns = n; }
     GridDev g;
     const bool wave = !d_surf && k >= 16;
     const float ppc = wave ? 10.f : 6.f;
diff --git a/lidar-global-registration_amd/csrc/lgr_grid.hip b/lidar-global-registration_amd/csrc/lgr_grid.hip
--- a/lidar-global-registration_amd/csrc/lgr_grid.hip
+++ b/lidar-global-registration_amd/csrc/lgr_grid.hip
@@ -6,6 +6,7 @@
 
 #include "lgr_grid.cuh"
 #include "lgr_knn_wave.cuh"
+#include "lgr_sort.cuh"
 
 namespace {
 
@@ -56,18 +57,34 @@
     }
 }
 
-__global__ void cell_keys(const float* __restrict__ pts, int n, float ox, float oy, float oz, float h, int dx, int dy, int dz,
-                          unsigned invalid_key, unsigned* __restrict__ keys, int* __restrict__ vals) {
-    int i = blockIdx.x * blockDim.x + threadIdx.x;
-    if (i >= n) return;
-    float x = pts[(size_t) i * 12], y = pts[(size_t) i * 12 + 1], z = pts[(size_t) i * 12 + 2];
-    unsigned k = invalid_key;
-    if (lgr_finite3(x, y, z)) {
-        int cx = min(max(lgr_cellc(x, ox, h), 0), dx - 1), cy = min(max(lgr_cellc(y, oy, h), 0), dy - 1), cz = min(max(lgr_cellc(z, oz, h), 0), dz - 1);
-        k = (unsigned) ((cz * dy + cy) * dx + cx);
-    }
-    keys[i] = k; vals[i] = i;
-}
+struct CellKeySrc {
+    const float* pts;
+    float ox, oy, oz, h;
+    int dx, dy, dz;
+    unsigned invalid_key;
+    __device__ __forceinline__ unsigned key(size_t i) const {
+        const float x = pts[i * 12], y = pts[i * 12 + 1], z = pts[i * 12 + 2];
+        unsigned k = invalid_key;
+        if (lgr_finite3(x, y, z)) {
+            int cx = min(max(lgr_cellc(x, ox, h), 0), dx - 1), cy = min(max(lgr_cellc(y, oy, h), 0), dy - 1), cz = min(max(lgr_cellc(z, oz, h), 0), dz - 1);
+            k = (unsigned) ((cz * dy + cy) * dx + cx);
+        }
+        return k;
+    }
+    __device__ __forceinline__ int val(size_t i) const { return (int) i; }
+};
+struct GridSink {
+    const float* pts;
+    unsigned* keys;
+    float4 *pxyz, *pnrm;
+    __device__ __forceinline__ void put(size_t pos, unsigned k, int o) const {
+        keys[pos] = k;
+        const float4* p = reinterpret_cast<const float4*>(pts + (size_t) o * 12);
+        const float4 a = p[0], b = p[1], c = p[2];
+        pxyz[pos] = make_float4(a.x, a.y, a.z, __int_as_float(o));
+        pnrm[pos] = make_float4(b.x, b.y, b.z, c.y);
+    }
+};
 
 constexpr int CSF_T = 256, CSF_SHIFT = 10, CSF_CELLS = 1 << CSF_SHIFT;
 static_assert(CSF_CELLS == 4 * CSF_T, "one int4 store per thread");
@@ -109,17 +126,6 @@
         if (c + 1u <= ncell) start[c + 1] = v.y;
         if (c + 2u <= ncell) start[c + 2] = v.z;
     }
-}
-
-__global__ void gather_points(const float* __restrict__ pts, const int* __restrict__ vals, int nvalid,
-                              float4* __restrict__ pxyz, float4* __restrict__ pnrm) {
-    int i = blockIdx.x * blockDim.x + threadIdx.x;
-    if (i >= nvalid) return;
-    int o = vals[i];
-    const float4* p = reinterpret_cast<const float4*>(pts + (size_t) o * 12);
-    float4 a = p[0], b = p[1], c = p[2];
-    pxyz[i] = make_float4(a.x, a.y, a.z, __int_as_float(o));
-    pnrm[i] = make_float4(b.x, b.y, b.z, c.y);
 }
 
 constexpr int KNN_BLOCK = 128;
@@ -332,22 +338,22 @@
         h *= 2.f;
     }
     int ncell = dim[0] * dim[1] * dim[2];
-    unsigned *keys, *keys2;
-    int *vals, *vals2, *start;
+    unsigned* keys2;
+    int* start;
     float4 *pxyz, *pnrm;
-    LGR_TRY(lgr_ws_t(ctx, sb + 0, (size_t) n + 1, &keys));
-    LGR_TRY(lgr_ws_t(ctx, sb + 1, (size_t) n + 1, &vals));
     LGR_TRY(lgr_ws_t(ctx, sb + 2, (size_t) n + 1, &keys2));
-    LGR_TRY(lgr_ws_t(ctx, sb + 3, (size_t) n + 1, &vals2));
     LGR_TRY(lgr_ws_t(ctx, sb + 4, (size_t) ncell + 2, &start));
     LGR_TRY(lgr_ws_t(ctx, sb + 5, (size_t) n + 1, &pxyz));
     LGR_TRY(lgr_ws_t(ctx, sb + 6, (size_t) n + 1, &pnrm));
     int nvalid = 0;
     if (n > 0) {
-        cell_keys<<<cdiv(n, 256), 256, 0, ctx->stream>>>(d_pts, n, mn[0], mn[1], mn[2], h, dim[0], dim[1], dim[2], (unsigned) ncell, keys, vals);
         int bits = 1;
         while (((unsigned long long) 1 << bits) <= (unsigned long long) ncell) ++bits;
-        LGR_TRY(lgr_sort_pairs_u32(ctx, keys, keys2, vals, vals2, (size_t) n, 0, bits));
+        const int sh0 = 0;
+        int dsh[lgr_rs::RS_MAX_PASSES], dw[lgr_rs::RS_MAX_PASSES];
+        const int nd = lgr_rs::plan_digits(&sh0, &bits, 1, dsh, dw);
+        LGR_TRY(lgr_rs::sort_passes<unsigned>(ctx, CellKeySrc{d_pts, mn[0], mn[1], mn[2], h, dim[0], dim[1], dim[2], (unsigned) ncell},
+                                              GridSink{d_pts, keys2, pxyz, pnrm}, (size_t) n, dsh, dw, nd));
         const int nblk = (int) (((size_t) ncell + 1 + CSF_CELLS - 1) >> CSF_SHIFT);
         int* coarse;
         LGR_TRY(lgr_ws_t(ctx, WS_GRID_MISC, (size_t) nblk + 1 + 64, &coarse));
@@ -359,7 +365,6 @@
         LGR_HIP(ctx, hipMemcpyAsync(h_n, start + ncell, 4, hipMemcpyDeviceToHost, ctx->stream));
         LGR_HIP(ctx, hipStreamSynchronize(ctx->stream));
         nvalid = *h_n;
-        if (nvalid > 0) gather_points<<<cdiv(nvalid, 256), 256, 0, ctx->stream>>>(d_pts, vals2, nvalid, pxyz, pnrm);
     } else {
         LGR_HIP(ctx, hipMemsetAsync(start, 0, ((size_t) ncell + 2) * 4, ctx->stream));
     }
@@ -367,6 +372,31 @@
     out->ox = mn[0]; out->oy = mn[1]; out->oz = mn[2]; out->h = h;
     out->dx = dim[0]; out->dy = dim[1]; out->dz = dim[2];
     out->n = nvalid; out->cell_start = start; out->pxyz = pxyz; out->pnrm = pnrm;
+    return LGR_OK;
+}
+
+extern "C" int lgr_grid_build_dev(lgr_ctx* ctx, const float* d_pts, int n, float h, float target, float* origin_h, int* dims_n,
+                                  int32_t* d_cell_start, size_t cell_capacity, float* d_pxyz, float* d_pnrm) {
+    lgr_turn turn__(ctx);
+    if (!ctx) return LGR_ERR_INVALID_ARG;
+    LGR_CHECK(ctx, (d_pts || n == 0) && n >= 0 && origin_h && dims_n && d_cell_start && (n == 0 || (d_pxyz && d_pnrm)), LGR_ERR_INVALID_ARG);
+    LGR_HIP(ctx, hipSetDevice(ctx->device));
+    GridDev g;
+    LGR_TRY(lgr_grid_build(ctx, WS_GRID_C, d_pts, n, h, target, &g));
+    const size_t cells = (size_t) g.dx * g.dy * g.dz;
+    LGR_CHECK(ctx, cells + 1 <= cell_capacity, LGR_ERR_INVALID_ARG);
+    origin_h[0] = g.ox; origin_h[1] = g.oy; origin_h[2] = g.oz; origin_h[3] = g.h;
+    dims_n[0] = g.dx; dims_n[1] = g.dy; dims_n[2] = g.dz; dims_n[3] = g.n;
+    LGR_HIP(ctx, hipMemcpyAsync(d_cell_start, g.cell_start, (cells + 1) * 4, hipMemcpyDeviceToDevice, ctx->stream));
+    if (n > 0) {
+        LGR_HIP(ctx, hipMemsetAsync(d_pxyz, 0, (size_t) n * 16, ctx->stream));
+        LGR_HIP(ctx, hipMemsetAsync(d_pnrm, 0, (size_t) n * 16, ctx->stream));
+    }
+    if (g.n > 0) {
+        LGR_HIP(ctx, hipMemcpyAsync(d_pxyz, g.pxyz, (size_t) g.n * 16, hipMemcpyDeviceToDevice, ctx->stream));
+        LGR_HIP(ctx, hipMemcpyAsync(d_pnrm, g.pnrm, (size_t) g.n * 16, hipMemcpyDeviceToDevice, ctx->stream));
+    }
+    LGR_HIP(ctx, hipStreamSynchronize(ctx->stream));
     return LGR_OK;
 }
 
diff --git a/lidar-global-registration_amd/csrc/lgr_internal.h b/lidar-global-registration_amd/csrc/lgr_internal.h
--- a/lidar-global-registration_amd/csrc/lgr_internal.h
+++ b/lidar-global-registration_amd/csrc/lgr_internal.h
@@ -105,7 +105,7 @@
     WS_RANSAC_T, WS_RANSAC_STATS, WS_RANSAC_PACK, WS_RANSAC_LIST, WS_RANSAC_HIST, WS_RANSAC_MISC, WS_RANSAC_MASK, WS_RANSAC_MASKT,
     WS_PIPE_SURF_S, WS_PIPE_SURF_T, WS_PIPE_FEAT_S, WS_PIPE_FEAT_T, WS_PIPE_IJ, WS_PIPE_JI, WS_PIPE_DIJ, WS_PIPE_DJI,
     WS_PIPE_CORR, WS_PIPE_KNN_S, WS_PIPE_KNN_T, WS_PIPE_FLAGS, WS_PIPE_MISC, WS_PIPE_KIDX_S, WS_PIPE_KIDX_T, WS_PIPE_KPS_S, WS_PIPE_KPS_T,
-    WS_MS_KNN_I, WS_MS_KNN_D, WS_MS_LIST_S, WS_MS_LIST_T, WS_MS_SUB, WS_MS_FEAT_S, WS_MS_FEAT_T, WS_MS_SURF2, WS_MS_RES, WS_PLANE_VISITED, WS_PLANE_CLAIMED, WS_PLANE_OUT, WS_LOCAL_G, WS_SORT_TMP, WS_MATCH_BOX, WS_RANSAC_GHIST,
+    WS_MS_KNN_I, WS_MS_KNN_D, WS_MS_LIST_S, WS_MS_LIST_T, WS_MS_SUB, WS_MS_FEAT_S, WS_MS_FEAT_T, WS_MS_SURF2, WS_MS_RES, WS_PLANE_VISITED, WS_PLANE_CLAIMED, WS_PLANE_OUT, WS_LOCAL_G, WS_SORT_TMP, WS_SORT_TMP2, WS_MATCH_BOX, WS_RANSAC_GHIST,
     WS_HOST_A, WS_HOST_B, WS_HOST_C, WS_HOST_D, WS_HOST_E, WS_HOST_F,
     WS_SHOT_PACK_A, WS_SHOT_PACK_B, WS_SHOT_KEYS,
     WS_ROPS_MASKED, WS_ROPS_LRF, WS_ROPS_KPS,
diff --git a/lidar-global-registration_amd/csrc/lgr_sort.cuh b/lidar-global-registration_amd/csrc/lgr_sort.cuh
--- /dev/null
+++ b/lidar-global-registration_amd/csrc/lgr_sort.cuh
@@ -0,0 +1,242 @@
+#pragma once
+#include <algorithm>
+
+#include "lgr_internal.h"
+
+namespace lgr_rs {
+
+constexpr int RS_BITS = 11, RS_DIGITS = 1 << RS_BITS;
+constexpr int RS_THREADS = 256, RS_WAVES = RS_THREADS / 64, RS_ITEMS = 8, RS_TILE = RS_THREADS * RS_ITEMS, RS_WTILE = 64 * RS_ITEMS;
+constexpr int RS_MAX_PASSES = 16;
+
+template <class K>
+struct PairSrc {
+    const K* k; const int* v;
+    __device__ __forceinline__ K key(size_t i) const { return k[i]; }
+    __device__ __forceinline__ int val(size_t i) const { return v[i]; }
+};
+template <class K>
+struct PairDst {
+    K* k; int* v;
+    __device__ __forceinline__ void put(size_t pos, K key, int val) const { k[pos] = key; v[pos] = val; }
+};
+
+static inline int plan_digits(const int* shifts, const int* widths, int np, int* dsh, int* dw) {
+    int nd = 0;
+    for (int p = 0; p < np; ++p) {
+        const int w = widths[p];
+        if (w <= 0) continue;
+        const int parts = (w + RS_BITS - 1) / RS_BITS;
+        int b = 0;
+        for (int q = 0; q < parts; ++q) {
+            if (nd >= RS_MAX_PASSES) return -1;
+            const int dwq = w / parts + (q < w % parts ? 1 : 0);
+            dsh[nd] = shifts[p] + b; dw[nd] = dwq; ++nd;
+            b += dwq;
+        }
+    }
+    return nd;
+}
+
+template <class K, class Src>
+__global__ __launch_bounds__(RS_THREADS) void rs_count(Src src, size_t n, int shift, unsigned mask, int nblk, unsigned* __restrict__ counts ) {
+    __shared__ unsigned h[RS_DIGITS];
+    const int ndig = (int) mask + 1;
+    for (int d = threadIdx.x; d < ndig; d += RS_THREADS) h[d] = 0u;
+    __syncthreads();
+    const size_t base = (size_t) blockIdx.x * RS_TILE;
+#pragma unroll
+    for (int r = 0; r < RS_ITEMS; ++r) {
+        const size_t i = base + (size_t) r * RS_THREADS + threadIdx.x;
+        if (i < n) atomicAdd(&h[(unsigned) (src.key(i) >> shift) & mask], 1u);
+    }
+    __syncthreads();
+    for (int d = threadIdx.x; d < ndig; d += RS_THREADS) counts[(size_t) d * nblk + blockIdx.x] = h[d];
+}
+
+static __global__ __launch_bounds__(256) void rs_scan(unsigned* __restrict__ counts, int nblk, unsigned* __restrict__ tot) {
+    __shared__ unsigned wsum[4];
+    __shared__ unsigned carry_s;
+    unsigned* row = counts + (size_t) blockIdx.x * nblk;
+    const int tid = threadIdx.x, lane = tid & 63, wave = tid >> 6;
+    if (tid == 0) carry_s = 0u;
+    __syncthreads();
+    for (int b0 = 0; b0 < nblk; b0 += 256) {
+        const int b = b0 + tid;
+        const unsigned c = b < nblk ? row[b] : 0u;
+        unsigned incl = c;
+        for (int o = 1; o < 64; o <<= 1) { const unsigned t = __shfl_up(incl, o); if (lane >= o) incl += t; }
+        if (lane == 63) wsum[wave] = incl;
+        __syncthreads();
+        unsigned before = carry_s;
+        for (int w = 0; w < wave; ++w) before += wsum[w];
+        if (b < nblk) row[b] = before + incl - c;
+        __syncthreads();
+        if (tid == 255) carry_s = before + incl;
+        __syncthreads();
+    }
+    if (tid == 0) tot[blockIdx.x] = carry_s;
+}
+
+template <int DPT>
+__device__ __forceinline__ void rs_block_excl(unsigned (&v)[DPT], unsigned* wsum , unsigned& total) {
+    const int lane = threadIdx.x & 63, wave = threadIdx.x >> 6;
+    unsigned s = 0u;
+#pragma unroll
+    for (int j = 0; j < DPT; ++j) { const unsigned c = v[j]; v[j] = s; s += c; }
+    unsigned incl = s;
+    for (int o = 1; o < 64; o <<= 1) { const unsigned t = __shfl_up(incl, o); if (lane >= o) incl += t; }
+    __syncthreads();
+    if (lane == 63) wsum[wave] = incl;
+    __syncthreads();
+    unsigned before = 0u, all = 0u;
+#pragma unroll
+    for (int w = 0; w < RS_WAVES; ++w) { const unsigned x = wsum[w]; if (w < wave) before += x; all += x; }
+    const unsigned off = before + incl - s;
+#pragma unroll
+    for (int j = 0; j < DPT; ++j) v[j] += off;
+    total = all;
+}
+
+template <class K, class Src, class Dst>
+__global__ __launch_bounds__(RS_THREADS) void rs_scatter(Src src, Dst dst, size_t n, int shift, int bits, int nblk, const unsigned* __restrict__ offs ,
+                                                         const unsigned* __restrict__ tot ) {
+    constexpr int DPT = RS_DIGITS / RS_THREADS;
+    __shared__ __attribute__((aligned(16))) unsigned short whist[RS_WAVES][RS_DIGITS];
+    __shared__ unsigned goff[RS_DIGITS];
+    __shared__ unsigned short tstart[RS_DIGITS];
+    __shared__ unsigned wsum[RS_WAVES];
+    __shared__ K sk[RS_TILE];
+    __shared__ int sv[RS_TILE];
+    const int tid = threadIdx.x, lane = tid & 63, wave = tid >> 6;
+    const unsigned mask = (1u << bits) - 1u;
+    const int ndig = 1 << bits;
+    for (int e = tid; e < RS_WAVES * RS_DIGITS / 2; e += RS_THREADS) reinterpret_cast<unsigned*>(&whist[0][0])[e] = 0u;
+    {
+        unsigned c[DPT];
+#pragma unroll
+        for (int j = 0; j < DPT; ++j) { const int d = tid * DPT + j; c[j] = d < ndig ? tot[d] : 0u; }
+        unsigned all;
+        rs_block_excl<DPT>(c, wsum, all);
+#pragma unroll
+        for (int j = 0; j < DPT; ++j) { const int d = tid * DPT + j; if (d < ndig) goff[d] = c[j] + offs[(size_t) d * nblk + blockIdx.x]; }
+    }
+    __syncthreads();
+    const size_t base = (size_t) blockIdx.x * RS_TILE;
+    const int n_tile = (int) min((size_t) RS_TILE, n - base);
+    const unsigned long long lt = (1ull << lane) - 1ull;
+    K key[RS_ITEMS];
+    int val[RS_ITEMS];
+    unsigned short wrank[RS_ITEMS];
+#pragma unroll
+    for (int r = 0; r < RS_ITEMS; ++r) {
+        const int e = wave * RS_WTILE + r * 64 + lane;
+        const bool valid = e < n_tile;
+        key[r] = valid ? src.key(base + e) : (K) 0;
+        val[r] = valid ? src.val(base + e) : 0;
+    }
+#pragma unroll
+    for (int r = 0; r < RS_ITEMS; ++r) {
+        const int e = wave * RS_WTILE + r * 64 + lane;
+        const bool valid = e < n_tile;
+        const unsigned d = (unsigned) (key[r] >> shift) & mask;
+        unsigned long long peers = __ballot(valid);
+        for (int b = 0; b < bits; ++b) {
+            const bool bit = (d >> b) & 1u;
+            const unsigned long long bal = __ballot(bit);
+            peers &= bit ? bal : ~bal;
+        }
+        const unsigned before = valid ? whist[wave][d] : 0u;
+        wrank[r] = (unsigned short) (before + __popcll(peers & lt));
+        __builtin_amdgcn_fence(__ATOMIC_ACQ_REL, "wavefront");
+        __builtin_amdgcn_wave_barrier();
+        if (valid && (peers & lt) == 0ull) whist[wave][d] = (unsigned short) (before + __popcll(peers));
+        __builtin_amdgcn_fence(__ATOMIC_ACQ_REL, "wavefront");
+        __builtin_amdgcn_wave_barrier();
+    }
+    __syncthreads();
+    {
+        static_assert(DPT == 8, "one uint4 of 16-bit counters per thread and wave");
+        unsigned c[DPT] = {0u, 0u, 0u, 0u, 0u, 0u, 0u, 0u};
+#pragma unroll
+        for (int w = 0; w < RS_WAVES; ++w) {
+            uint4* q = reinterpret_cast<uint4*>(&whist[w][tid * DPT]);
+            const uint4 x = *q;
+            const unsigned in[4] = {x.x, x.y, x.z, x.w};
+            unsigned out[4];
+#pragma unroll
+            for (int j = 0; j < 4; ++j) {
+                out[j] = (c[2 * j] & 0xffffu) | (c[2 * j + 1] << 16);
+                c[2 * j] += in[j] & 0xffffu; c[2 * j + 1] += in[j] >> 16;
+            }
+            *q = make_uint4(out[0], out[1], out[2], out[3]);
+        }
+        unsigned all;
+        rs_block_excl<DPT>(c, wsum, all);
+#pragma unroll
+        for (int j = 0; j < DPT; ++j) tstart[tid * DPT + j] = (unsigned short) c[j];
+    }
+    __syncthreads();
+#pragma unroll
+    for (int r = 0; r < RS_ITEMS; ++r) {
+        const int e = wave * RS_WTILE + r * 64 + lane;
+        if (e >= n_tile) continue;
+        const unsigned d = (unsigned) (key[r] >> shift) & mask;
+        const int tp = tstart[d] + whist[wave][d] + wrank[r];
+        sk[tp] = key[r];
+        sv[tp] = val[r];
+    }
+    __syncthreads();
+#pragma unroll
+    for (int r = 0; r < RS_ITEMS; ++r) {
+        const int e = r * RS_THREADS + tid;
+        if (e >= n_tile) continue;
+        const K k = sk[e];
+        const unsigned d = (unsigned) (k >> shift) & mask;
+        const size_t pos = (size_t) goff[d] + (unsigned) (e - tstart[d]);
+        dst.put(pos, k, sv[e]);
+    }
+}
+
+template <class K>
+static inline size_t tmp_bytes(size_t n) {
+    const size_t nblk = (n + RS_TILE - 1) / RS_TILE;
+    return ((n * sizeof(K) + 255) & ~(size_t) 255) + ((n * 4 + 255) & ~(size_t) 255) + (nblk + 1) * RS_DIGITS * 4 + 1024;
+}
+
+template <class K, class Src, class Dst>
+int sort_passes(lgr_ctx* ctx, Src src, Dst dst, size_t n, const int* dsh, const int* dw, int nd) {
+    LGR_CHECK(ctx, n > 0 && n < ((size_t) 1 << 31) && nd >= 1, LGR_ERR_INVALID_ARG);
+    const int nblk = (int) ((n + RS_TILE - 1) / RS_TILE);
+    char* tmp;
+    const size_t kb = (n * sizeof(K) + 255) & ~(size_t) 255, vb = (n * 4 + 255) & ~(size_t) 255;
+    LGR_TRY(lgr_ws_t(ctx, WS_SORT_TMP, tmp_bytes<K>(n), &tmp));
+    K* tk[2] = {(K*) tmp, nullptr};
+    int* tv[2] = {(int*) (tmp + kb), nullptr};
+    unsigned* tot = (unsigned*) (tmp + kb + vb);
+    unsigned* counts = tot + RS_DIGITS;
+    if (nd > 2) {
+        char* tmp2;
+        LGR_TRY(lgr_ws_t(ctx, WS_SORT_TMP2, kb + vb, &tmp2));
+        tk[1] = (K*) tmp2; tv[1] = (int*) (tmp2 + kb);
+    }
+    PairSrc<K> ps{nullptr, nullptr};
+    for (int p = 0; p < nd; ++p) {
+        const unsigned mask = (1u << dw[p]) - 1u;
+        const bool first = p == 0, last = p == nd - 1;
+        const int t = nd > 2 ? (p & 1) : 0;
+        PairDst<K> pd{tk[t], tv[t]};
+        if (first) rs_count<K, Src><<<nblk, RS_THREADS, 0, ctx->stream>>>(src, n, dsh[p], mask, nblk, counts);
+        else rs_count<K, PairSrc<K>><<<nblk, RS_THREADS, 0, ctx->stream>>>(ps, n, dsh[p], mask, nblk, counts);
+        rs_scan<<<1 << dw[p], 256, 0, ctx->stream>>>(counts, nblk, tot);
+        if (first && last) rs_scatter<K, Src, Dst><<<nblk, RS_THREADS, 0, ctx->stream>>>(src, dst, n, dsh[p], dw[p], nblk, counts, tot);
+        else if (first) rs_scatter<K, Src, PairDst<K>><<<nblk, RS_THREADS, 0, ctx->stream>>>(src, pd, n, dsh[p], dw[p], nblk, counts, tot);
+        else if (last) rs_scatter<K, PairSrc<K>, Dst><<<nblk, RS_THREADS, 0, ctx->stream>>>(ps, dst, n, dsh[p], dw[p], nblk, counts, tot);
+        else rs_scatter<K, PairSrc<K>, PairDst<K>><<<nblk, RS_THREADS, 0, ctx->stream>>>(ps, pd, n, dsh[p], dw[p], nblk, counts, tot);
+        ps = PairSrc<K>{pd.k, pd.v};
+    }
+    LGR_HIP(ctx, hipGetLastError());
+    return LGR_OK;
+}
+
+}
diff --git a/lidar-global-registration_amd/csrc/lgr_sort.hip b/lidar-global-registration_amd/csrc/lgr_sort.hip
--- a/lidar-global-registration_amd/csrc/lgr_sort.hip
+++ b/lidar-global-registration_amd/csrc/lgr_sort.hip
@@ -1,133 +1,8 @@
-#include <algorithm>
-
-#include "lgr_internal.h"
+#include "lgr_sort.cuh"
 
 namespace {
 
-constexpr int RS_THREADS = 256, RS_ITEMS = 8, RS_TILE = RS_THREADS * RS_ITEMS, RS_SLOTS = RS_ITEMS * (RS_THREADS / 64);
-
-template <class K>
-__global__ __launch_bounds__(RS_THREADS) void rs_count(const K* __restrict__ keys, size_t n, int shift, unsigned mask, int nblk, unsigned* __restrict__ counts ) {
-    __shared__ unsigned h[256];
-    h[threadIdx.x] = 0u;
-    __syncthreads();
-    const size_t base = (size_t) blockIdx.x * RS_TILE;
-#pragma unroll
-    for (int r = 0; r < RS_ITEMS; ++r) {
-        const size_t i = base + (size_t) r * RS_THREADS + threadIdx.x;
-        if (i < n) atomicAdd(&h[(unsigned) (keys[i] >> shift) & mask], 1u);
-    }
-    __syncthreads();
-    counts[(size_t) threadIdx.x * nblk + blockIdx.x] = h[threadIdx.x];
-}
-
-__global__ __launch_bounds__(256) void rs_scan(unsigned* __restrict__ counts, int nblk, unsigned* __restrict__ tot) {
-    __shared__ unsigned wsum[4];
-    __shared__ unsigned carry_s;
-    unsigned* row = counts + (size_t) blockIdx.x * nblk;
-    const int tid = threadIdx.x, lane = tid & 63, wave = tid >> 6;
-    if (tid == 0) carry_s = 0u;
-    __syncthreads();
-    for (int b0 = 0; b0 < nblk; b0 += 256) {
-        const int b = b0 + tid;
-        const unsigned c = b < nblk ? row[b] : 0u;
-        unsigned incl = c;
-        for (int o = 1; o < 64; o <<= 1) { const unsigned t = __shfl_up(incl, o); if (lane >= o) incl += t; }
-        if (lane == 63) wsum[wave] = incl;
-        __syncthreads();
-        unsigned before = carry_s;
-        for (int w = 0; w < wave; ++w) before += wsum[w];
-        if (b < nblk) row[b] = before + incl - c;
-        __syncthreads();
-        if (tid == 255) carry_s = before + incl;
-        __syncthreads();
-    }
-    if (tid == 0) tot[blockIdx.x] = carry_s;
-}
-
-template <class K>
-__global__ __launch_bounds__(RS_THREADS) void rs_scatter(const K* __restrict__ kin, const int* __restrict__ vin, K* __restrict__ kout, int* __restrict__ vout,
-                                                         size_t n, int shift, unsigned mask, int nblk, const unsigned* __restrict__ offs ,
-                                                         const unsigned* __restrict__ tot ) {
-    __shared__ unsigned short hist[RS_SLOTS][256];
-    __shared__ unsigned goff[256];
-    __shared__ unsigned short tstart[257];
-    __shared__ unsigned wsum[4];
-    __shared__ K sk[RS_TILE];
-    __shared__ int sv[RS_TILE];
-    const int tid = threadIdx.x, lane = tid & 63, wave = tid >> 6;
-    for (int e = tid; e < RS_SLOTS * 256; e += RS_THREADS) (&hist[0][0])[e] = 0;
-    {
-        const unsigned c = tot[tid];
-        unsigned incl = c;
-        for (int o = 1; o < 64; o <<= 1) { const unsigned t = __shfl_up(incl, o); if (lane >= o) incl += t; }
-        if (lane == 63) wsum[wave] = incl;
-        __syncthreads();
-        unsigned before = 0u;
-        for (int w = 0; w < wave; ++w) before += wsum[w];
-        goff[tid] = before + incl - c + offs[(size_t) tid * nblk + blockIdx.x];
-    }
-    __syncthreads();
-    const size_t base = (size_t) blockIdx.x * RS_TILE;
-    const int n_tile = (int) min((size_t) RS_TILE, n - base);
-    const unsigned long long lt = (1ull << lane) - 1ull;
-    K key[RS_ITEMS];
-    int val[RS_ITEMS];
-    unsigned short wrank[RS_ITEMS];
-#pragma unroll
-    for (int r = 0; r < RS_ITEMS; ++r) {
-        const int e = r * RS_THREADS + tid;
-        const bool valid = e < n_tile;
-        key[r] = valid ? kin[base + e] : (K) 0;
-        val[r] = valid ? vin[base + e] : 0;
-        const unsigned d = (unsigned) (key[r] >> shift) & mask;
-        unsigned long long peers = __ballot(valid);
-#pragma unroll
-        for (int b = 0; b < 8; ++b) {
-            const bool bit = (d >> b) & 1u;
-            const unsigned long long bal = __ballot(bit);
-            peers &= bit ? bal : ~bal;
-        }
-        wrank[r] = (unsigned short) __popcll(peers & lt);
-        if (valid && (peers & lt) == 0ull) hist[r * (RS_THREADS / 64) + wave][d] = (unsigned short) __popcll(peers);
-    }
-    __syncthreads();
-    {
-        unsigned run = 0u;
-#pragma unroll 4
-        for (int s = 0; s < RS_SLOTS; ++s) { const unsigned c = hist[s][tid]; hist[s][tid] = (unsigned short) run; run += c; }
-        unsigned incl = run;
-        for (int o = 1; o < 64; o <<= 1) { const unsigned t = __shfl_up(incl, o); if (lane >= o) incl += t; }
-        __syncthreads();
-        if (lane == 63) wsum[wave] = incl;
-        __syncthreads();
-        unsigned before = 0u;
-        for (int w = 0; w < wave; ++w) before += wsum[w];
-        tstart[tid] = (unsigned short) (before + incl - run);
-        if (tid == 255) tstart[256] = (unsigned short) (before + incl);
-    }
-    __syncthreads();
-#pragma unroll
-    for (int r = 0; r < RS_ITEMS; ++r) {
-        const int e = r * RS_THREADS + tid;
-        if (e >= n_tile) continue;
-        const unsigned d = (unsigned) (key[r] >> shift) & mask;
-        const int tp = tstart[d] + hist[r * (RS_THREADS / 64) + wave][d] + wrank[r];
-        sk[tp] = key[r];
-        sv[tp] = val[r];
-    }
-    __syncthreads();
-#pragma unroll
-    for (int r = 0; r < RS_ITEMS; ++r) {
-        const int e = r * RS_THREADS + tid;
-        if (e >= n_tile) continue;
-        const K k = sk[e];
-        const unsigned d = (unsigned) (k >> shift) & mask;
-        const size_t pos = (size_t) goff[d] + (unsigned) (e - tstart[d]);
-        kout[pos] = k;
-        vout[pos] = sv[e];
-    }
-}
+using namespace lgr_rs;
 
 __global__ void rs_copy(const unsigned* __restrict__ a, unsigned* __restrict__ b, size_t nwords) {
     size_t i = (size_t) blockIdx.x * blockDim.x + threadIdx.x;
@@ -138,40 +13,16 @@
 int sort_impl(lgr_ctx* ctx, const K* kin, K* kout, const int* vin, int* vout, size_t n, const int* shifts, const int* widths, int np) {
     if (n == 0) return LGR_OK;
     LGR_CHECK(ctx, kin && kout && vin && vout && (const void*) kin != (const void*) kout && vin != vout && n < ((size_t) 1 << 31), LGR_ERR_INVALID_ARG);
-    int dsh[16], dw[16], nd = 0;
-    for (int p = 0; p < np; ++p)
-        for (int b = 0; b < widths[p]; b += 8) {
-            LGR_CHECK(ctx, nd < 16, LGR_ERR_INVALID_ARG);
-            dsh[nd] = shifts[p] + b; dw[nd] = std::min(8, widths[p] - b); ++nd;
-        }
+    int dsh[RS_MAX_PASSES], dw[RS_MAX_PASSES];
+    const int nd = plan_digits(shifts, widths, np, dsh, dw);
+    LGR_CHECK(ctx, nd >= 0, LGR_ERR_INVALID_ARG);
     if (nd == 0) {
         rs_copy<<<cdiv((long long) (n * sizeof(K) / 4), 256), 256, 0, ctx->stream>>>((const unsigned*) kin, (unsigned*) kout, n * sizeof(K) / 4);
         rs_copy<<<cdiv((long long) n, 256), 256, 0, ctx->stream>>>((const unsigned*) vin, (unsigned*) vout, n);
         LGR_HIP(ctx, hipGetLastError());
         return LGR_OK;
     }
-    const int nblk = (int) ((n + RS_TILE - 1) / RS_TILE);
-    char* tmp;
-    const size_t kb = (n * sizeof(K) + 255) & ~(size_t) 255, vb = (n * 4 + 255) & ~(size_t) 255;
-    LGR_TRY(lgr_ws_t(ctx, WS_SORT_TMP, kb + vb + (size_t) nblk * 256 * 4 + 1024, &tmp));
-    K* tk = (K*) tmp;
-    int* tv = (int*) (tmp + kb);
-    unsigned* tot = (unsigned*) (tmp + kb + vb);
-    unsigned* counts = tot + 256;
-    const K* sk = kin;
-    const int* sv = vin;
-    for (int p = 0; p < nd; ++p) {
-        const bool to_out = ((nd - 1 - p) & 1) == 0;
-        K* dk = to_out ? kout : tk;
-        int* dv = to_out ? vout : tv;
-        const unsigned mask = (1u << dw[p]) - 1u;
-        rs_count<K><<<nblk, RS_THREADS, 0, ctx->stream>>>(sk, n, dsh[p], mask, nblk, counts);
-        rs_scan<<<256, 256, 0, ctx->stream>>>(counts, nblk, tot);
-        rs_scatter<K><<<nblk, RS_THREADS, 0, ctx->stream>>>(sk, sv, dk, dv, n, dsh[p], mask, nblk, counts, tot);
-        sk = dk; sv = dv;
-    }
-    LGR_HIP(ctx, hipGetLastError());
-    return LGR_OK;
+    return sort_passes<K>(ctx, PairSrc<K>{kin, vin}, PairDst<K>{kout, vout}, n, dsh, dw, nd);
 }
 
 }
diff --git a/lidar-global-registration_amd/lgr_amd/capi.py b/lidar-global-registration_amd/lgr_amd/capi.py
--- a/lidar-global-registration_amd/lgr_amd/capi.py
+++ b/lidar-global-registration_amd/lgr_amd/capi.py
@@ -259,6 +259,16 @@
         self.check(_lib.lgr_sort_pairs_u64_dev(self.h, _ptr(keys), _ptr(ko), _ptr(vals), _ptr(vo), C.c_size_t(keys.shape[0]), sh, wd, len(ranges)))
         return ko, vo
 
+    def grid_build(self, pts, h=0.0, target=0.0, cell_capacity=1 << 22):
+        torch = self.torch
+        pts = pts.contiguous(); n = pts.shape[0]
+        start = self.empty((cell_capacity,), torch.int32); pxyz = self.empty((max(n, 1), 4), torch.float32); pnrm = self.empty((max(n, 1), 4), torch.float32)
+        oh = (C.c_float * 4)(); dn = (C.c_int * 4)()
+        self.check(_lib.lgr_grid_build_dev(self.h, _ptr(pts), int(n), C.c_float(h), C.c_float(target), oh, dn, _ptr(start), C.c_size_t(cell_capacity),
+                                           _ptr(pxyz), _ptr(pnrm)))
+        cells = dn[0] * dn[1] * dn[2]
+        return list(oh), list(dn), start[:cells + 1], pxyz[:n], pnrm[:n]
+
     def match_flann(self, q, t):
         torch = self.torch
         q = q.contiguous(); t = t.contiguous()
```
